# KohakuBlueleaf/UwUDiff

Hardware: AMD Instinct MI355X
Metric: train images/sec (whole node), DiT-S/2 256^2 latent (higher is better)
Workload: dtype bf16; 1 GPU; DiT-S/2 (L12 D384 h6), 4x32x32 synthetic latents + pooled-text cond 1280, eps-MSE, AdamW lr1e-6 wd0.01 cosine; random-init weights; per_gpu_batch=768, global_batch=768, parallelism=dp1

## Files before the change

include/uwu_hip.h:

```cpp
#ifndef UWU_HIP_H
#define UWU_HIP_H

#include <stddef.h>
#include <stdint.h>

#ifdef __cplusplus
extern "C" {
#endif

#define UWU_F32 0
#define UWU_BF16 1
#define UWU_I64 2

#define UWU_OK 0
#define UWU_EINVAL (-1)
#define UWU_ELAUNCH (-2)
#define UWU_ENOTIMPL (-3)

#define UWU_PT_EPSILON 0
#define UWU_PT_V 1
#define UWU_PT_SAMPLE 2
#define UWU_PT_RF 3

#define UWU_EPI_NONE 0
#define UWU_EPI_BIAS 1
#define UWU_EPI_BIAS_GELU 2
#define UWU_EPI_DGELU 3
#define UWU_EPI_BIAS_SILU 4
#define UWU_EPI_ACCUM 5

const char* uwu_last_error(void);
int uwu_version(void);
int uwu_env_refresh(void);
int uwu_memset_zero(void* p, uint64_t bytes, void* stream);


int uwu_schedule_gather(const int64_t* timesteps, const float* sigmas_desc, const float* all_snr,
                        const float* alphas_cumprod, int n_train, int B, int snr_mode, float gamma,
                        int debias, float* coef, void* stream);

int uwu_rf_time_to_sigma(const float* u01, float sigma_max, const float* log_sigmas_asc, int n_train,
                         int B, float* coef, float* timesteps, void* stream);

int uwu_qsample(const float* x, const float* noise, const float* coef, int B, int64_t n, float* noisy,
                void* noisy_bf16, void* stream);

int uwu_qsample_norm(const float* x, const float* noise, const float* coef, int B, int64_t n, float vae_mean,
                     float vae_std, float* x_norm, float* noisy, void* stream);

int uwu_philox_raw(uint32_t* out, int64_t n_counters, uint64_t seed, uint64_t offset, void* stream);
int uwu_philox_normal(float* out, int64_t n, uint64_t seed, uint64_t offset, void* stream);
int uwu_draw_timesteps(int64_t* timesteps, int n_train, int B, uint64_t seed, uint64_t offset, void* stream);
int uwu_draw_u01(float* u01, int B, uint64_t seed, uint64_t offset, void* stream);
int uwu_qsample_draw(const float* x, const float* coef, int B, int64_t n, int use_norm, float vae_mean, float vae_std,
                     float* x_norm, float* noise, float* noisy, uint64_t seed, uint64_t offset, void* stream);
int uwu_posterior_draw(const float* moments, int ldm, int B, int latent, int64_t HW, float* z, float* mean_out, float* logvar_out,
                       uint64_t seed, uint64_t offset, void* stream);

int uwu_ctx_place(const void* src, int dtype, const int64_t* mask, float* out, int B, int S, int F, int S_total,
                  int F_total, int s_off, int f_off, void* stream);

int uwu_loss_fwd_bwd(const float* x, const float* noise, const float* xt, const void* model_output,
                     int out_dtype, const float* coef, int pred_type, int target_type, int force_convert,
                     int B, int64_t n, float* losses, float* loss_mean, void* grad_out, float* pred,
                     float* target, void* stream);

int uwu_scale_inplace(void* y, int dtype, int64_t n, const float* scale, void* stream);
int uwu_scale_into(const void* x, void* y, int dtype, int64_t n, const float* scale, void* stream);
int uwu_cast_i64_to_f32(const int64_t* x, float* y, int64_t n, void* stream);

int uwu_aggregate_concat(const void* emb, const int* starts, void* out, int B, int max_n, int64_t unit_bytes,
                         int elem_size, uint64_t pad_bits, void* stream);
int uwu_aggregate_split(const void* cat, const int* starts, void* out, int B, int max_n, int64_t unit_bytes,
                        void* stream);
int uwu_aggregate_first(const void* emb, const int* starts, void* out, int B, int64_t unit_bytes, void* stream);

int uwu_sampler_step(const float* x, const float* eps_cond, const float* eps_uncond, const float* noise, float* out,
                     float* denoised, int64_t n, float cfg, float sigma, float sigma_down, float sigma_up,
                     float s_noise, void* stream);
int uwu_sampler_combine(const float* base, const float* eps_cond, const float* eps_uncond, const float* noise,
                        float* out, int64_t n, float cfg, float a, float b, float c, void* stream);
int uwu_scale_copy(const float* x, float* y, int64_t n, float scale, void* stream);

int uwu_cfg_input(const float* x, float* y, int B, int64_t n, float c_in, void* stream);
int uwu_sampler_combine_draw(const float* base, const float* eps_cond, const float* eps_uncond, float* out, int64_t n, float cfg,
                             float a, float b, float c, uint64_t seed, uint64_t offset, void* stream);
// ... 328 lines not shown
```

uwudiff_amd/csrc/api.cpp:

```cpp
#include <hip/hip_runtime.h>
#include <stdarg.h>
#include <stdio.h>

#include <atomic>

#include "../../include/uwu_hip.h"

static thread_local char g_err[512] = "";

void uwu_set_error(const char* fmt, ...) {
  va_list ap;
  va_start(ap, fmt);
  vsnprintf(g_err, sizeof(g_err), fmt, ap);
  va_end(ap);
}

extern "C" const char* uwu_last_error(void) { return g_err; }
extern "C" int uwu_version(void) { return 1; }

static int g_env_gen = 0;
int uwu_env_generation() { return g_env_gen; }
extern "C" int uwu_env_refresh(void) { return ++g_env_gen; }

std::atomic<const char*> g_uwu_gemm_last_kernel{""};
extern "C" const char* uwu_gemm_last_kernel(void) { return g_uwu_gemm_last_kernel.load(std::memory_order_relaxed); }

extern "C" int uwu_memset_zero(void* p, uint64_t bytes, void* stream) {
  if (!p || !bytes) {
    uwu_set_error("memset_zero: bad argument");
    return UWU_EINVAL;
  }
  if (hipMemsetAsync(p, 0, (size_t)bytes, (hipStream_t)stream) != hipSuccess) {
    uwu_set_error("memset_zero: hipMemsetAsync failed");
    return UWU_ELAUNCH;
  }
  return UWU_OK;
}

static const int kMaxDev = 64;
static int g_dev_cus[kMaxDev];
static size_t g_dev_lds[kMaxDev];
static bool g_dev_known[kMaxDev];
static int cur_dev() {
  int dev = 0;
  if (hipGetDevice(&dev) != hipSuccess || dev < 0 || dev >= kMaxDev) dev = 0;
  if (!g_dev_known[dev]) {
    hipDeviceProp_t prop;
    if (hipGetDeviceProperties(&prop, dev) == hipSuccess) {
      g_dev_cus[dev] = prop.multiProcessorCount;
      g_dev_lds[dev] = prop.sharedMemPerBlockOptin ? prop.sharedMemPerBlockOptin : prop.sharedMemPerBlock;
    } else {
      g_dev_cus[dev] = 0;
      g_dev_lds[dev] = 0;
    }
    g_dev_known[dev] = true;
  }
  return dev;
}
int uwu_dev_index() { return cur_dev(); }
int uwu_dev_cus() { return g_dev_cus[cur_dev()]; }
bool uwu_dev_lds_fits(size_t bytes) { return g_dev_lds[cur_dev()] >= bytes; }
bool uwu_func_lds(const void* fn, size_t bytes, unsigned char* done) {
  const int dev = cur_dev();
  if (done[dev] == 1) return true;
  if (done[dev] == 2) return false;
  const bool ok = g_dev_lds[dev] >= bytes && hipFuncSetAttribute(fn, hipFuncAttributeMaxDynamicSharedMemorySize, (int)bytes) == hipSuccess;
  done[dev] = ok ? 1 : 2;
  return ok;
}
```

uwudiff_amd/csrc/attention_p256.hip:

```cpp
#include "common.h"

namespace {

constexpr int P_RING = 3;
template <int DH>
struct PGeom {
  static constexpr bool TAIL = DH > 64;
  static constexpr int SLOT = 16384 + (TAIL ? 2048 + 256 : 0);
  static constexpr int OFF_TT = 16384, OFF_TL = 16384 + 2048;
  static constexpr int OFF_DS = P_RING * SLOT;
  static constexpr int KIMG = 32768 + (TAIL ? 4096 : 0);
  static constexpr int OFF_K = OFF_DS + 32768;
  static constexpr int OFF_LSE = OFF_K + 2 * KIMG;
  static constexpr int OFF_DELTA = OFF_LSE + (TAIL ? 0 : 2 * 1024);
  static constexpr int OFF_ZERO = OFF_DELTA + 2 * 256;
  static constexpr int LDS = OFF_ZERO + (TAIL ? 16 : 0);
};
static_assert(PGeom<64>::LDS == 150016 && PGeom<72>::LDS <= 163840, "LDS budget");
constexpr int P_LDS = PGeom<64>::LDS;

struct PArgs {
  const bf16_t *q, *k, *v, *o, *dO;
  bf16_t *dq, *dk, *dv;
  const float* lse;
  int B, H, ldq, ldk, ldv, ldo, nheads;
  float scale;
};

__device__ __forceinline__ int fsw(int row) {
  return (((row >> 2) ^ (row >> 4)) & 1) | ((((row >> 3) ^ (row >> 4)) & 1) << 1) | (((row >> 1) & 1) << 2);
}
__device__ __forceinline__ int Fsw(int row) {
  return (row & 1) | (((row >> 2) & 1) << 1) | (((row >> 3) & 1) << 2) | (((row >> 1) & 1) << 3);
}

typedef short s16x4 __attribute__((ext_vector_type(4)));
typedef unsigned su32x2 __attribute__((ext_vector_type(2)));

__device__ __forceinline__ void glds16(const void* gsrc, unsigned lds_dst ) {
  unsigned keep;
  asm volatile("s_mov_b32 %0, m0\n\ts_mov_b32 m0, %2\n\ts_nop 0\n\tglobal_load_lds_dwordx4 %1, off\n\ts_mov_b32 m0, %0"
               : "=&s"(keep)
               : "v"(gsrc), "s"(lds_dst)
               : "memory");
}
__device__ __forceinline__ void glds4(const void* gsrc, unsigned lds_dst ) {
  unsigned keep;
  asm volatile("s_mov_b32 %0, m0\n\ts_mov_b32 m0, %2\n\ts_nop 0\n\tglobal_load_lds_dword %1, off\n\ts_mov_b32 m0, %0"
               : "=&s"(keep)
               : "v"(gsrc), "s"(lds_dst)
               : "memory");
}
__device__ __forceinline__ void glds16_s(const void* sbase , unsigned voff, unsigned lds_dst ) {
  unsigned keep;
  asm volatile("s_mov_b32 %0, m0\n\ts_mov_b32 m0, %3\n\ts_nop 0\n\tglobal_load_lds_dwordx4 %1, %2\n\ts_mov_b32 m0, %0"
               : "=&s"(keep)
               : "v"(voff), "s"(sbase), "s"(lds_dst)
               : "memory");
}
__device__ __forceinline__ f32x16 mfma32(const uint4& a, const uint4& b, f32x16 c) {
  return __builtin_amdgcn_mfma_f32_32x32x16_bf16(*reinterpret_cast<const bf16x8*>(&a), *reinterpret_cast<const bf16x8*>(&b), c, 0,
                                                 0, 0);
}
__device__ __forceinline__ f32x4 mfma16(const uint4& a, const uint4& b, f32x4 c) {
  return __builtin_amdgcn_mfma_f32_16x16x32_bf16(*reinterpret_cast<const bf16x8*>(&a), *reinterpret_cast<const bf16x8*>(&b), c, 0,
                                                 0, 0);
}
__device__ __forceinline__ uint4 pack8(const f32x16& x, int s) {
  bf16x8 f;
#pragma unroll
  for (int j = 0; j < 8; ++j) f[j] = (bf16_t)x[8 * s + j];
  return *reinterpret_cast<uint4*>(&f);
}

extern __shared__ __attribute__((aligned(16))) char p_smem[];

__device__ __forceinline__ void lane_halves(float x, float& lo, float& hi) {
  float a = x, b = x;
  asm volatile("v_nop\n\tv_nop\n\tv_permlane32_swap_b32 %0, %1" : "+v"(a), "+v"(b));
  lo = a;
  hi = b;
}

__device__ __forceinline__ uint4 tr_pair(unsigned a0, unsigned a1) {
  const s16x4 lo = __builtin_amdgcn_ds_read_tr16_b64_v4i16(
      (__attribute__((address_space(3))) s16x4*)((__attribute__((address_space(3))) char*)p_smem + a0));
  const s16x4 hi = __builtin_amdgcn_ds_read_tr16_b64_v4i16(
      (__attribute__((address_space(3))) s16x4*)((__attribute__((address_space(3))) char*)p_smem + a1));
  uint4 r;
  r.x = ((unsigned)(unsigned short)lo[0]) | ((unsigned)(unsigned short)lo[1] << 16);
  r.y = ((unsigned)(unsigned short)lo[2]) | ((unsigned)(unsigned short)lo[3] << 16);
  r.z = ((unsigned)(unsigned short)hi[0]) | ((unsigned)(unsigned short)hi[1] << 16);
  r.w = ((unsigned)(unsigned short)hi[2]) | ((unsigned)(unsigned short)hi[3] << 16);
  return r;
}

template <int DH>
__global__ void __launch_bounds__(512, 2) attn_bwd_p256(const PArgs a) {
  using G = PGeom<DH>;
  constexpr bool TAIL = G::TAIL;
  constexpr int T = 256, NKS = TAIL ? 5 : 4, NDT = TAIL ? 3 : 2;
  constexpr int P_SLOT = G::SLOT, P_OFF_DS = G::OFF_DS, P_OFF_K = G::OFF_K, P_OFF_LSE = G::OFF_LSE, P_OFF_DELTA = G::OFF_DELTA;
  constexpr int KIMG = G::KIMG;
  char* const smem = p_smem;
  const int tid = threadIdx.x, lane = tid & 63;
  const int wave = __builtin_amdgcn_readfirstlane(tid >> 6);
  const int r = lane & 31, h = lane >> 5;
  const int fr = lane & 15, fq = lane >> 4;
  const unsigned smem_base = (unsigned)(size_t)((const __attribute__((address_space(3))) char*)p_smem);
  const float c = a.scale * 1.4426950408889634f;
  const float ninv_scale = -1.f / a.scale;
  const int nmy = (a.nheads - (int)blockIdx.x + (int)gridDim.x - 1) / (int)gridDim.x;
  const int total = 4 * nmy;
  const int k0 = wave * 32;

  const int drow = tid >> 3;
  const int dchunk = (tid & 7) ^ fsw(drow);
  unsigned B0, A0, K0, D0, TQ0, TA0, KT0;
  auto phase1_consts = [&](int ln) {
    const int r_ = ln & 31, h_ = ln >> 5;
    B0 = (unsigned)(r_ * 128 + ((h_ ^ fsw(r_)) << 4));
    const int rowL = 4 * h_ + ((ln & 15) >> 2), chunkL = 2 * ((ln >> 4) & 1) + ((ln & 3) >> 1);
    A0 = (unsigned)(rowL * 128 + ((chunkL ^ fsw(rowL)) << 4) + 8 * (ln & 1));
    TQ0 = (unsigned)((r_ >> 3) * 256 + (r_ & 7) * 16);
    TA0 = (unsigned)(rowL * 16 + 8 * (ln & 1));
  };
  auto phase2_consts = [&](int ln) {
    const int fr_ = ln & 15, fq_ = ln >> 4;
    const int rowK = 8 * fq_ + (fr_ >> 2);
    K0 = (unsigned)(rowK * 128 + ((((fr_ & 3) >> 1) ^ fsw(rowK)) << 4) + 8 * (fr_ & 1));
    D0 = (unsigned)(rowK * 128 + (((fr_ & 3) ^ Fsw(rowK)) << 3));
    KT0 = (unsigned)(rowK * 16 + 8 * (fr_ & 1));
  };
  auto opaque_lane = [&]() {
    int ln = lane;
    asm volatile("" : "+v"(ln));
    return ln;
  };
  auto my_tid = [&]() {
    int x = tid;
    if constexpr (TAIL) asm volatile("" : "+v"(x));
    return x;
  };
  if constexpr (!TAIL) {
    phase1_consts(lane);
    phase2_consts(lane);
  }

  auto head_ptrs = [&](int j, int& b, int& hd) {
    const int bh = (int)blockIdx.x + j * (int)gridDim.x;
    b = bh / a.H;
    hd = bh - b * a.H;
  };
  uint4 oreg;
  unsigned otail = 0;
  auto issue_tile = [&](int g) {
    int b, hd;
    head_ptrs(g >> 2, b, hd);
    const int tid = my_tid(), lane = tid & 63, drow = tid >> 3, dchunk = (tid & 7) ^ fsw(drow);
    const int row = 64 * (g & 3) + drow;
    const bf16_t* qs = a.q + ((int64_t)b * T + row) * a.ldq + hd * DH + 8 * dchunk;
    const bf16_t* gs = a.dO + ((int64_t)b * T + row) * a.ldo + hd * DH + 8 * dchunk;
    const unsigned dst = smem_base + (unsigned)((g % P_RING) * P_SLOT + wave * 1024);
    glds16(qs, dst);
    glds16(gs, dst + 8192);
    oreg = *reinterpret_cast<const uint4*>(a.o + ((int64_t)b * T + row) * a.ldo + hd * DH + 8 * dchunk);
    if constexpr (TAIL) {
      const unsigned slot = smem_base + (unsigned)((g % P_RING) * P_SLOT);
      if (lane < 16) {
        const int64_t trow = (int64_t)b * T + 64 * (g & 3) + 8 * wave + (lane & 7);
        const bf16_t* src = lane < 8 ? a.q + trow * a.ldq + hd * DH + 64 : a.dO + trow * a.ldo + hd * DH + 64;
        glds16(src, slot + (unsigned)(G::OFF_TT + wave * 256));
      }
      glds4(a.lse + ((int64_t)b * a.H + hd) * T + 64 * (g & 3) + lane, slot + (unsigned)G::OFF_TL);
      otail = *reinterpret_cast<const unsigned*>(a.o + ((int64_t)b * T + row) * a.ldo + hd * DH + 64 + 2 * (tid & 3));
    }
  };
  auto issue_head = [&](int j) {
    int b, hd;
    head_ptrs(j, b, hd);
    const int tid = my_tid(), lane = tid & 63, drow = tid >> 3, dchunk = (tid & 7) ^ fsw(drow);
    const unsigned dst = smem_base + (unsigned)(P_OFF_K + (j & 1) * KIMG + wave * 1024);
#pragma unroll
    for (int p = 0; p < 4; ++p)
      glds16(a.k + ((int64_t)b * T + 64 * p + drow) * a.ldk + hd * DH + 8 * dchunk, dst + p * 8192);
    if constexpr (TAIL) {
      if (lane < 32)
        glds16(a.k + ((int64_t)b * T + 32 * wave + lane) * a.ldk + hd * DH + 64,
               smem_base + (unsigned)(P_OFF_K + (j & 1) * KIMG + 32768 + wave * 512));
    } else {
      glds4(a.lse + ((int64_t)b * a.H + hd) * T + 64 * (wave & 3) + lane,
            smem_base + (unsigned)(P_OFF_LSE + (j & 1) * 1024 + (wave & 3) * 256));
    }
  };
  uint4 kf[NKS], vf[NKS];
  auto load_kv = [&](int j) {
    int b, hd;
    head_ptrs(j, b, hd);
    const int tid = my_tid(), r = tid & 31, h = (tid >> 5) & 1;
#pragma unroll
    for (int s = 0; s < 4; ++s) {
      kf[s] = *reinterpret_cast<const uint4*>(a.k + ((int64_t)b * T + k0 + r) * a.ldk + hd * DH + 16 * s + 8 * h);
      vf[s] = *reinterpret_cast<const uint4*>(a.v + ((int64_t)b * T + k0 + r) * a.ldv + hd * DH + 16 * s + 8 * h);
// ... 188 lines not shown
      const uint4 fa = tr_pair(Ki + ka + ko, Ki + (ka ^ 0x10u) + 512u + ko);
      const uint4 fb = tr_pair(Ki + kb + ko, Ki + (kb ^ 0x10u) + 512u + ko);
      const uint4 fd = tr_pair(Di + da + ko, Di + (da ^ 0x10u) + 512u + ko);
      acc0 = mfma16(fa, fd, acc0);
      acc1 = mfma16(fb, fd, acc1);
      if constexpr (TAIL) {
        const unsigned kt = Ki + 32768u + KT0 + 512u * kk;
        acc2 = mfma16(tr_pair(kt, kt + 64u), fd, acc2);
      }
    }
    int b, hd;
    head_ptrs(j, b, hd);
    const f32x4 v0 = acc0 * a.scale, v1 = acc1 * a.scale;
    const bf16x4 p0b = {(bf16_t)v0[0], (bf16_t)v0[1], (bf16_t)v0[2], (bf16_t)v0[3]};
    const bf16x4 p1b = {(bf16_t)v1[0], (bf16_t)v1[1], (bf16_t)v1[2], (bf16_t)v1[3]};
    const uint2 p0 = *reinterpret_cast<const uint2*>(&p0b), p1 = *reinterpret_cast<const uint2*>(&p1b);
    const su32x2 sx = __builtin_amdgcn_permlane16_swap(p0.x, p1.x, false, false);
    const su32x2 sy = __builtin_amdgcn_permlane16_swap(p0.y, p1.y, false, false);
    const bool odd = fq & 1;
    const int d = odd ? 16 * (db0 + 1) + 4 * (fq - 1) : 16 * db0 + 4 * fq;
    bf16_t* dst = a.dq + ((int64_t)b * T + 64 * t + 16 * qblk + fr) * a.ldq + hd * DH + d;
    *reinterpret_cast<uint4*>(dst) = uint4{sx[0], sy[0], sx[1], sy[1]};
    if constexpr (TAIL) {
      const f32x4 v2 = acc2 * a.scale;
      store4(a.dq + ((int64_t)b * T + 64 * t + 16 * qblk + fr) * a.ldq + hd * DH + 64 + 4 * (fq & 1), v2);
    }
  }
  asm volatile("s_waitcnt lgkmcnt(0)" ::: "memory");
  __builtin_amdgcn_s_barrier();
  store_dkdv(nmy - 1);
}

template <int DH>
struct FGeom {
  static constexpr bool TAIL = DH > 64;
  static constexpr int RING = TAIL ? 4 : 5;
  static constexpr int SLOT = 16384 + (TAIL ? 2048 : 0);
  static constexpr int OFF_TT = 16384;
  static constexpr int OST = 4096 + (TAIL ? 512 : 0);
  static constexpr int OFF_O = RING * SLOT;
  static constexpr int OFF_Q = OFF_O + 8 * OST;
  static constexpr int OFF_ZERO = OFF_Q + 32768 + (TAIL ? 4096 : 0);
  static constexpr int LDS = OFF_ZERO + (TAIL ? 16 : 0);
};
static_assert(FGeom<64>::LDS == 147456 && FGeom<72>::LDS <= 163840, "LDS budget");
constexpr int F_LDS = FGeom<64>::LDS;

struct FArgs {
  const bf16_t *q, *k, *v;
  bf16_t* out;
  float* lse;
  int B, H, ldq, ldk, ldv, ldo, nheads;
  float scale;
};

template <int N>
__device__ __forceinline__ void wait_vm_n() {
  asm volatile("s_waitcnt vmcnt(%0)" ::"n"(N) : "memory");
}
__device__ __forceinline__ void wait_vm(int n) {
  switch (n < 20 ? n : 20) {
    case 20: wait_vm_n<20>(); break;
    case 19: wait_vm_n<19>(); break;
    case 18: wait_vm_n<18>(); break;
    case 17: wait_vm_n<17>(); break;
    case 16: wait_vm_n<16>(); break;
    case 15: wait_vm_n<15>(); break;
    case 14: wait_vm_n<14>(); break;
    case 13: wait_vm_n<13>(); break;
    case 12: wait_vm_n<12>(); break;
    case 11: wait_vm_n<11>(); break;
    case 10: wait_vm_n<10>(); break;
    case 9: wait_vm_n<9>(); break;
    case 8: wait_vm_n<8>(); break;
    case 7: wait_vm_n<7>(); break;
    case 6: wait_vm_n<6>(); break;
    case 5: wait_vm_n<5>(); break;
    case 4: wait_vm_n<4>(); break;
    case 3: wait_vm_n<3>(); break;
    case 2: wait_vm_n<2>(); break;
    case 1: wait_vm_n<1>(); break;
    default: wait_vm_n<0>();
  }
}

template <int DH>
__global__ void __launch_bounds__(512, 2) attn_fwd_p256(const FArgs a) {
  using G = FGeom<DH>;
  constexpr bool TAIL = G::TAIL;
  constexpr int T = 256, NKS = TAIL ? 5 : 4, NDT = TAIL ? 3 : 2;
  constexpr int F_RING = G::RING, AHEAD = F_RING - 1, F_SLOT = G::SLOT, F_OFF_O = G::OFF_O, F_OFF_Q = G::OFF_Q;
  constexpr int TILE_OPS = TAIL ? 3 : 2, Q_OPS = TAIL ? 5 : 4, ST_OPS = TAIL ? 6 : 5;
  char* const smem = p_smem;
  const int tid = threadIdx.x, lane = tid & 63;
  const int wave = __builtin_amdgcn_readfirstlane(tid >> 6);
  const int r = lane & 31, h = lane >> 5;
  const unsigned smem_base = (unsigned)(size_t)((const __attribute__((address_space(3))) char*)p_smem);
  const float c = a.scale * 1.4426950408889634f;
  const int nmy = (a.nheads - (int)blockIdx.x + (int)gridDim.x - 1) / (int)gridDim.x;
  const int total = 4 * nmy;
  const int q0 = wave * 32;
  const int drow = tid >> 3;
  const int dchunk = (tid & 7) ^ fsw(drow);
  const unsigned B0 = (unsigned)(r * 128 + ((h ^ fsw(r)) << 4));
  const unsigned QR0 = (unsigned)(F_OFF_Q + (q0 + r) * 128 + ((h ^ fsw(q0 + r)) << 4));
  const int rowL = 4 * h + ((lane & 15) >> 2), chunkL = 2 * ((lane >> 4) & 1) + ((lane & 3) >> 1);
  const unsigned A0 = (unsigned)(rowL * 128 + ((chunkL ^ fsw(rowL)) << 4) + 8 * (lane & 1));
  const unsigned TQ0 = (unsigned)((r >> 3) * 256 + (r & 7) * 16);
  const unsigned TA0 = (unsigned)(rowL * 16 + 8 * (lane & 1));
  auto head_ptrs = [&](int j, int& b, int& hd) {
    const int bh = (int)blockIdx.x + j * (int)gridDim.x;
    b = bh / a.H;
    hd = bh - b * a.H;
  };
  const unsigned kvoff = (unsigned)((drow * a.ldk + 8 * dchunk) * 2), vvoff = (unsigned)((drow * a.ldv + 8 * dchunk) * 2);
  const unsigned qvoff = (unsigned)((drow * a.ldq + 8 * dchunk) * 2);
  const bf16_t *kb_n = nullptr, *vb_n = nullptr, *qb_n = nullptr;
  int b_c = 0, hd_c = 0;
  auto set_issue_head = [&](int j) {
    int b, hd;
    head_ptrs(j, b, hd);
    kb_n = a.k + (int64_t)b * T * a.ldk + hd * DH;
    vb_n = a.v + (int64_t)b * T * a.ldv + hd * DH;
    qb_n = a.q + (int64_t)b * T * a.ldq + hd * DH;
  };
  auto issue_tile = [&](int g) {
    const int t64 = 64 * (g & 3);
    const unsigned dst = smem_base + (unsigned)((g % F_RING) * F_SLOT + wave * 1024);
    glds16_s(kb_n, kvoff + (unsigned)(t64 * a.ldk * 2), dst);
    glds16_s(vb_n, vvoff + (unsigned)(t64 * a.ldv * 2), dst + 8192);
    if constexpr (TAIL) {
      if (lane < 16) {
        const int trow = t64 + 8 * wave + (lane & 7);
        const bf16_t* src = lane < 8 ? kb_n + (int64_t)trow * a.ldk + 64 : vb_n + (int64_t)trow * a.ldv + 64;
        glds16(src, smem_base + (unsigned)((g % F_RING) * F_SLOT + G::OFF_TT + wave * 256));
      }
    }
  };
  auto issue_q = [&]() {
#pragma unroll
    for (int p = 0; p < 4; ++p)
      glds16_s(qb_n, qvoff + (unsigned)(64 * p * a.ldq * 2), smem_base + (unsigned)(F_OFF_Q + p * 8192 + wave * 1024));
    if constexpr (TAIL) {
      if (lane < 32) glds16(qb_n + (int64_t)(32 * wave + lane) * a.ldq + 64, smem_base + (unsigned)(F_OFF_Q + 32768 + wave * 512));
    }
  };
  auto extras = [&](int i) { return ((i & 3) == 1 && (i >> 2) + 1 < nmy ? Q_OPS : 0) + ((i & 3) == 3 ? ST_OPS : 0); };
  auto younger = [&](int g) {
    int y = 0;
    const int gi = g - (F_RING - 1);
    if (gi < 0) {
      for (int x = g + 1; x < F_RING - 1; ++x) y += x < total ? TILE_OPS : 0;
    } else {
      y += extras(gi);
    }
    for (int i = gi < 0 ? 0 : gi + 1; i < g; ++i) y += (i + F_RING - 1 < total ? TILE_OPS : 0) + extras(i);
    return y;
  };
  if (total == 0) return;
  static_assert(AHEAD == 4 || AHEAD == 3, "the tile issued in iteration g belongs to the next head from t = 4 - AHEAD on");
  if constexpr (TAIL)
    if (tid < 4) reinterpret_cast<unsigned*>(smem + G::OFF_ZERO)[tid] = 0u;
  set_issue_head(0);
  head_ptrs(0, b_c, hd_c);
  issue_q();
#pragma unroll
  for (int g = 0; g < F_RING - 1; ++g) issue_tile(g);

  uint4 qf[NKS];
  f32x16 o[NDT];
  float m = -INFINITY, l = 0.f;
  for (int g = 0; g < total; ++g) {
    const int j = g >> 2, t = g & 3;
    int n_fly = younger(g);
    if (t == 0 && j > 0) {
      const int yq = (g - 2 + F_RING - 1 < total ? TILE_OPS : 0) + (g - 1 + F_RING - 1 < total ? TILE_OPS : 0) + ST_OPS;
      n_fly = yq < n_fly ? yq : n_fly;
    }
    wait_vm(n_fly);
    __builtin_amdgcn_s_barrier();
    if (t == 0) head_ptrs(j, b_c, hd_c);
    if (t == 4 - AHEAD && j + 1 < nmy) set_issue_head(j + 1);
    if (g + F_RING - 1 < total) issue_tile(g + F_RING - 1);
    if (t == 0) {
#pragma unroll
      for (int s = 0; s < 4; ++s) qf[s] = *reinterpret_cast<const uint4*>(smem + (QR0 ^ (unsigned)(s << 5)));
      if constexpr (TAIL)
        qf[4] = *reinterpret_cast<const uint4*>(smem + (h ? (unsigned)G::OFF_ZERO : (unsigned)(F_OFF_Q + 32768 + (q0 + r) * 16)));
#pragma unroll
      for (int dt = 0; dt < NDT; ++dt) o[dt] = f32x16{};
      m = -INFINITY;
      l = 0.f;
    }
    if (t == 1 && j + 1 < nmy) issue_q();
    const unsigned Ks = (unsigned)((g % F_RING) * F_SLOT), Vs = Ks + 8192;
// ... 39 lines not shown
    for (int dt = 0; dt < 2; ++dt)
#pragma unroll
      for (int i = 0; i < 16; ++i) o[dt][i] *= alpha;
    if constexpr (TAIL) {
#pragma unroll
      for (int i = 0; i < 4; ++i) o[2][i] *= alpha;
    }
#pragma unroll
    for (int kt = 0; kt < 2; ++kt)
#pragma unroll
      for (int s2 = 0; s2 < 2; ++s2) {
        const uint4 pf = pack8(s[kt], s2);
#pragma unroll
        for (int dt = 0; dt < 2; ++dt) {
          const unsigned x0 = (A0 ^ (unsigned)(0x30 * s2) ^ (unsigned)(0x40 * dt)) + 2048u * s2 + 4096u * kt;
          const uint4 vt = tr_pair(Vs + x0, Vs + (x0 ^ 0x20u) + 1024u);
          o[dt] = mfma32(vt, pf, o[dt]);
        }
        if constexpr (TAIL) {
          const unsigned x0 = Ks + (unsigned)G::OFF_TT + 128u + TA0 + 512u * s2 + 1024u * kt;
          o[2] = mfma32(tr_pair(x0, x0 + 256u), pf, o[2]);
        }
      }
    if (t == 3) {
      const int b = b_c, hd = hd_c;
      float lt;
      {
        float lo, hi;
        lane_halves(l, lo, hi);
        lt = lo + hi;
      }
      const float inv = 1.f / lt;
      char* mine = smem + F_OFF_O + wave * G::OST;
#pragma unroll
      for (int dt = 0; dt < 2; ++dt)
#pragma unroll
        for (int g4 = 0; g4 < 4; ++g4) {
          const int d0 = 32 * dt + 8 * g4 + 4 * h;
          store4(reinterpret_cast<bf16_t*>(mine + r * 128 + (((d0 >> 3) ^ (r & 7)) << 4) + 2 * (d0 & 7)),
                 f32x4{o[dt][4 * g4] * inv, o[dt][4 * g4 + 1] * inv, o[dt][4 * g4 + 2] * inv, o[dt][4 * g4 + 3] * inv});
        }
      bf16_t* ob = a.out + ((int64_t)b * T + q0) * a.ldo + hd * DH;
#pragma unroll
      for (int p = 0; p < 4; ++p) {
        const int row = 8 * p + (lane >> 3), ch = lane & 7;
        const uint4 x = *reinterpret_cast<const uint4*>(mine + row * 128 + ((ch ^ (row & 7)) << 4));
        *reinterpret_cast<uint4*>(ob + (int64_t)row * a.ldo + 8 * ch) = x;
      }
      if constexpr (TAIL) {
        store4(reinterpret_cast<bf16_t*>(mine + 4096 + r * 16 + 8 * h), f32x4{o[2][0] * inv, o[2][1] * inv, o[2][2] * inv, o[2][3] * inv});
        const uint4 xt = *reinterpret_cast<const uint4*>(mine + 4096 + r * 16);
        *reinterpret_cast<uint4*>(ob + (int64_t)r * a.ldo + 64) = xt;
      }
      a.lse[((int64_t)b * a.H + hd) * T + q0 + r] = m * a.scale + __logf(lt);
    }
  }
}

}

bool uwu_attn_p256_ok(int T, int Tk, int d, int ldq, int ldk, int ldv, int ldo) {
  static UwuEnv on("UWU_ATTN_P256");
  if (on.get().is('0') || T != 256 || Tk != 256 || ldq % 8 || ldk % 8 || ldv % 8 || ldo % 8 || uwu_dev_cus() <= 0) return false;
  if (d == 64) return uwu_dev_lds_fits(P_LDS);
  static UwuEnv on72("UWU_ATTN_P256_D72");
  return d == 72 && !on72.get().is('0') && uwu_dev_lds_fits(PGeom<72>::LDS);
}

int uwu_attn_p256_bwd(const void* q, const void* k, const void* v, const void* o, const void* dO, const float* lse, void* dq,
                      void* dk, void* dv, int B, int H, int d, int ldq, int ldk, int ldv, int ldo, float scale, hipStream_t st) {
  static unsigned char done[UWU_MAX_DEV];
  const int n_cu = uwu_dev_cus();
  if (d == 72) {
    static unsigned char done72[UWU_MAX_DEV];
    if (n_cu <= 0 || !uwu_func_lds(reinterpret_cast<const void*>(attn_bwd_p256<72>), PGeom<72>::LDS, done72)) {
      uwu_set_error("attention_bwd(p256, d = 72): the device cannot give a workgroup %d bytes of LDS", (int)PGeom<72>::LDS);
      return UWU_ELAUNCH;
    }
    PArgs a{};
    a.q = (const bf16_t*)q; a.k = (const bf16_t*)k; a.v = (const bf16_t*)v; a.o = (const bf16_t*)o; a.dO = (const bf16_t*)dO;
    a.dq = (bf16_t*)dq; a.dk = (bf16_t*)dk; a.dv = (bf16_t*)dv; a.lse = lse;
    a.B = B; a.H = H; a.ldq = ldq; a.ldk = ldk; a.ldv = ldv; a.ldo = ldo; a.nheads = B * H; a.scale = scale;
    const int grid = a.nheads < n_cu ? a.nheads : n_cu;
    hipLaunchKernelGGL(attn_bwd_p256<72>, dim3(grid), dim3(512), PGeom<72>::LDS, st, a);
    UWU_LAUNCH_CHECK("attention_bwd(p256, d = 72)");
    return UWU_OK;
  }
  if (n_cu <= 0 || !uwu_func_lds(reinterpret_cast<const void*>(attn_bwd_p256<64>), P_LDS, done)) {
    uwu_set_error("attention_bwd(p256): the device cannot give a workgroup %d bytes of LDS", (int)P_LDS);
    return UWU_ELAUNCH;
  }
  PArgs a{};
  a.q = (const bf16_t*)q; a.k = (const bf16_t*)k; a.v = (const bf16_t*)v; a.o = (const bf16_t*)o; a.dO = (const bf16_t*)dO;
  a.dq = (bf16_t*)dq; a.dk = (bf16_t*)dk; a.dv = (bf16_t*)dv; a.lse = lse;
  a.B = B; a.H = H; a.ldq = ldq; a.ldk = ldk; a.ldv = ldv; a.ldo = ldo; a.nheads = B * H; a.scale = scale;
  const int grid = a.nheads < n_cu ? a.nheads : n_cu;
  hipLaunchKernelGGL(attn_bwd_p256<64>, dim3(grid), dim3(512), P_LDS, st, a);
  UWU_LAUNCH_CHECK("attention_bwd(p256)");
  return UWU_OK;
}

bool uwu_attn_p256_fwd_ok(int nheads, int T, int Tk, int d, int ldq, int ldk, int ldv, int ldo) {
  static UwuEnv on("UWU_ATTN_P256F");
  if (on.get().is('0')) return false;
  if (!on.is('1') && nheads < 1024) return false;
  if (T != 256 || Tk != 256 || ldq % 8 || ldk % 8 || ldv % 8 || ldo % 8 || uwu_dev_cus() <= 0) return false;
  if (d == 64) return uwu_dev_lds_fits(F_LDS);
  static UwuEnv on72("UWU_ATTN_P256F_D72");
  return d == 72 && !on72.get().is('0') && uwu_dev_lds_fits(FGeom<72>::LDS);
}

int uwu_attn_p256_fwd(const void* q, const void* k, const void* v, void* o, float* lse, int B, int H, int d, int ldq, int ldk, int ldv,
                      int ldo, float scale, hipStream_t st) {
  static unsigned char done[2][UWU_MAX_DEV];
  const int n_cu = uwu_dev_cus();
  const int lds = d == 72 ? FGeom<72>::LDS : F_LDS;
  const void* fn = d == 72 ? reinterpret_cast<const void*>(attn_fwd_p256<72>) : reinterpret_cast<const void*>(attn_fwd_p256<64>);
  if (n_cu <= 0 || !uwu_func_lds(fn, lds, done[d == 72])) {
    uwu_set_error("attention_fwd(p256): the device cannot give a workgroup %d bytes of LDS", lds);
    return UWU_ELAUNCH;
  }
  FArgs a{};
  a.q = (const bf16_t*)q; a.k = (const bf16_t*)k; a.v = (const bf16_t*)v; a.out = (bf16_t*)o; a.lse = lse;
  a.B = B; a.H = H; a.ldq = ldq; a.ldk = ldk; a.ldv = ldv; a.ldo = ldo; a.nheads = B * H; a.scale = scale;
  const int grid = a.nheads < n_cu ? a.nheads : n_cu;
  if (d == 72) hipLaunchKernelGGL(attn_fwd_p256<72>, dim3(grid), dim3(512), lds, st, a);
  else hipLaunchKernelGGL(attn_fwd_p256<64>, dim3(grid), dim3(512), lds, st, a);
  UWU_LAUNCH_CHECK("attention_fwd(p256)");
  return UWU_OK;
}
```

uwudiff_amd/csrc/common.h:

```cpp
#pragma once
#include <hip/hip_runtime.h>
#include <stdint.h>
#include <stdio.h>
#include <stdlib.h>

#include "../../include/uwu_hip.h"

typedef __bf16 bf16_t;
typedef __bf16 bf16x2 __attribute__((ext_vector_type(2)));
typedef __bf16 bf16x4 __attribute__((ext_vector_type(4)));
typedef __bf16 bf16x8 __attribute__((ext_vector_type(8)));
typedef float f32x2 __attribute__((ext_vector_type(2)));
typedef float f32x4 __attribute__((ext_vector_type(4)));
typedef float f32x16 __attribute__((ext_vector_type(16)));

#define UWU_WAVE 64

void uwu_set_error(const char* fmt, ...);

#define UWU_CHECK_ARG(cond, ...)       \
  do {                                 \
    if (!(cond)) {                     \
      uwu_set_error(__VA_ARGS__);      \
      return UWU_EINVAL;               \
    }                                  \
  } while (0)

#define UWU_LAUNCH_CHECK(name)                                                  \
  do {                                                                          \
    hipError_t e_ = hipGetLastError();                                          \
    if (e_ != hipSuccess) {                                                     \
      uwu_set_error("%s: launch failed: %s", name, hipGetErrorString(e_));      \
      return UWU_ELAUNCH;                                                       \
    }                                                                           \
  } while (0)

#include "env.h"

int uwu_dev_index();
int uwu_dev_cus();
bool uwu_dev_lds_fits(size_t bytes);
constexpr int UWU_MAX_DEV = 64;
bool uwu_func_lds(const void* fn, size_t bytes, unsigned char* done );

int uwu_prof_begin(void* stream);
void uwu_prof_end(int slot, int tag, int kind, double flops, double bytes, void* stream);
struct UwuProfScope {
  int slot;
  void* st;
  explicit UwuProfScope(void* s) : slot(uwu_prof_begin(s)), st(s) {}
  void done(int tag, int kind, double flops, double bytes) {
    if (slot >= 0) uwu_prof_end(slot, tag, kind, flops, bytes, st);
  }
};

__device__ __forceinline__ float to_f32(float v) { return v; }
__device__ __forceinline__ float to_f32(bf16_t v) { return (float)v; }
template <typename T>
__device__ __forceinline__ T from_f32(float v);
template <>
__device__ __forceinline__ float from_f32<float>(float v) { return v; }
template <>
__device__ __forceinline__ bf16_t from_f32<bf16_t>(float v) { return (bf16_t)v; }

#define UWU_DPP_F(v, ctrl, rmask, ident) \
  __builtin_bit_cast(float, __builtin_amdgcn_update_dpp(__builtin_bit_cast(int, (float)(ident)), __builtin_bit_cast(int, v), ctrl, rmask, 0xF, false))
__device__ __forceinline__ float wave_sum(float v) {
  v += UWU_DPP_F(v, 0xB1, 0xF, 0.f);
  v += UWU_DPP_F(v, 0x4E, 0xF, 0.f);
  v += UWU_DPP_F(v, 0x141, 0xF, 0.f);
  v += UWU_DPP_F(v, 0x140, 0xF, 0.f);
  v += UWU_DPP_F(v, 0x142, 0xA, 0.f);
  v += UWU_DPP_F(v, 0x143, 0xC, 0.f);
  return __builtin_bit_cast(float, __builtin_amdgcn_readlane(__builtin_bit_cast(int, v), 63));
}
__device__ __forceinline__ float wave_max(float v) {
  v = fmaxf(v, UWU_DPP_F(v, 0xB1, 0xF, v));
  v = fmaxf(v, UWU_DPP_F(v, 0x4E, 0xF, v));
  v = fmaxf(v, UWU_DPP_F(v, 0x141, 0xF, v));
  v = fmaxf(v, UWU_DPP_F(v, 0x140, 0xF, v));
  v = fmaxf(v, UWU_DPP_F(v, 0x142, 0xA, v));
  v = fmaxf(v, UWU_DPP_F(v, 0x143, 0xC, v));
  return __builtin_bit_cast(float, __builtin_amdgcn_readlane(__builtin_bit_cast(int, v), 63));
}
__device__ __forceinline__ float row16_sum(float v) {
  v += __builtin_bit_cast(float, __builtin_amdgcn_update_dpp(0, __builtin_bit_cast(int, v), 0xB1, 0xF, 0xF, true));
  v += __builtin_bit_cast(float, __builtin_amdgcn_update_dpp(0, __builtin_bit_cast(int, v), 0x4E, 0xF, 0xF, true));
  v += __builtin_bit_cast(float, __builtin_amdgcn_update_dpp(0, __builtin_bit_cast(int, v), 0x141, 0xF, 0xF, true));
  v += __builtin_bit_cast(float, __builtin_amdgcn_update_dpp(0, __builtin_bit_cast(int, v), 0x140, 0xF, 0xF, true));
  return v;
// ... 94 lines not shown
```

uwudiff_amd/csrc/dit.cpp:

```cpp
#include <hip/hip_runtime.h>
#include <math.h>
#include <stddef.h>
#include <stdint.h>
#include <stdlib.h>

#include "../../include/uwu_hip.h"
#include "env.h"

void uwu_set_error(const char* fmt, ...);

namespace {

constexpr int WGRAD_BLOCKS = 512;

struct Layout {
  size_t es;
  int64_t M, D, D3, D4, Kp, Ko;
  size_t feat, t_pre, t_h, temb, yemb, c, sc, mod;
  size_t sc16, dmod16;
  size_t tok, xe;
  size_t layer0, layer_stride;
  bool ckpt;
  size_t keep, scratch0;
  size_t o_x0, o_m1, o_r1, o_h1, o_qkv, o_lse, o_ao, o_y1, o_x1, o_m2, o_r2, o_h2, o_u, o_f, o_y2;
  size_t o_rope;
  size_t o_h1t, o_aot, o_h2t, o_ft;
  size_t xF, mF, rF, hF, otok;
  size_t dx, dy, dh, dqkv, dao, du, delta, dotok, dmod, dsc, dc, dth, dtp;
  size_t w2t;
  size_t wsc, wsc_bytes;
  size_t x8, x8t, dy8, dy8t, w8, w8_layer;
  size_t total;
};

inline size_t al(size_t x) { return (x + 255) & ~(size_t)255; }

Layout make_layout(const uwu_dit_desc& d) {
  Layout L{};
  L.es = d.dtype == UWU_BF16 ? 2 : 4;
  L.M = (int64_t)d.B * d.T;
  L.D = d.D;
  L.D3 = 3 * (int64_t)d.D;
  L.D4 = (int64_t)d.mlp_ratio * d.D;
  L.Kp = (int64_t)d.in_ch * d.patch * d.patch;
  L.Ko = (int64_t)d.out_ch * d.patch * d.patch;
  size_t p = 0;
  auto take = [&](size_t bytes) { size_t o = p; p = al(p + bytes); return o; };
  const size_t f4 = 4;
  L.feat = take((size_t)d.B * d.freq_dim * f4);
  L.t_pre = take((size_t)d.B * d.D * f4);
  L.t_h = take((size_t)d.B * d.D * f4);
  L.temb = take((size_t)d.B * d.D * f4);
  L.yemb = take((size_t)d.B * d.D * f4);
  L.c = take((size_t)d.B * d.D * f4);
  L.sc = take((size_t)d.B * d.D * f4);
  L.mod = take((size_t)d.B * d.mod_total * f4);
  L.sc16 = take((size_t)d.B * d.D * 2);
  L.dmod16 = take((size_t)d.B * d.mod_total * 2);
  L.tok = take(L.M * L.Kp * L.es);
  L.xe = take(L.M * L.D * L.es);
// ... 58 lines not shown
                           uwu_gemm_fp8_scratch_bytes((int)L.D3, d.D, (int)L.M), uwu_gemm_fp8_scratch_bytes(d.D, d.D, (int)L.M)})
      if (t > L.wsc_bytes) L.wsc_bytes = t;
  }
  L.wsc_bytes = (L.wsc_bytes + 255) & ~(size_t)255;
  L.wsc = take(L.wsc_bytes * (L.M <= 16384 ? 4 : 1));
  if (d.fp8) {
    L.x8 = take(L.M * L.D4);
    L.x8t = 0;
    L.dy8 = take(L.M * L.D4);
    L.dy8t = take(L.M * L.D4);
    L.w8_layer = al((size_t)24 * d.D * d.D);
    L.w8 = take((size_t)d.L * L.w8_layer);
  }
  L.total = p;
  return L;
}

int check_desc(const uwu_dit_desc* d) {
  if (!d) { uwu_set_error("dit: null descriptor"); return UWU_EINVAL; }
  if (d->B <= 0 || d->T <= 0 || d->D <= 0 || d->H <= 0 || d->L <= 0 || d->D % d->H || d->D % 8 ||
      d->img % d->patch || (d->img / d->patch) * (d->img / d->patch) != d->T || d->mlp_ratio <= 0 ||
      d->freq_dim <= 0 || d->freq_dim % 8) {
    uwu_set_error("dit: inconsistent shape B=%d T=%d D=%d H=%d L=%d img=%d patch=%d", d->B, d->T, d->D, d->H, d->L,
                  d->img, d->patch);
    return UWU_EINVAL;
  }
  if (d->dtype != UWU_F32 && d->dtype != UWU_BF16) { uwu_set_error("dit: bad dtype"); return UWU_EINVAL; }
  if (d->mod_total != d->L * 6 * d->D + 2 * d->D) { uwu_set_error("dit: mod_total mismatch"); return UWU_EINVAL; }
  if ((d->in_ch * d->patch * d->patch) % 8 || (d->out_ch * d->patch * d->patch) % 8 || (d->cond_dim % 8)) {
    uwu_set_error("dit: C*p*p and cond_dim must be multiples of 8");
    return UWU_EINVAL;
  }
  if (!d->w || !d->w32 || !d->pos || !d->ws) { uwu_set_error("dit: null buffer"); return UWU_EINVAL; }
  if (d->rope && (d->dtype != UWU_BF16 || d->D / d->H != 64 || d->T % 64 || d->T > 256 || !d->pos_xy)) {
    uwu_set_error("dit: the fused axial-RoPE attention needs bf16, head dim 64, T a multiple of 64 up to 256 and pos_xy");
    return UWU_EINVAL;
  }
  if (d->fp8) {
    if (d->fp8 < 0 || d->fp8 > 2 || d->dtype != UWU_BF16 || d->D % 128 || d->mlp_ratio != 4 || ((int64_t)d->B * d->T) % 128 ||
        !d->f8_scale || !d->f8_amax || !d->f8_fmt) {
      uwu_set_error("dit: fp8 mode needs bf16 activations, D %% 128 == 0, B*T %% 128 == 0, mlp_ratio 4 and the scale / amax / fmt arrays");
      return UWU_EINVAL;
    }
  }
  return UWU_OK;
}

#define RUN(expr)              \
  do {                         \
    int rc_ = (expr);          \
    if (rc_ != UWU_OK) return rc_; \
  } while (0)

int lin_fwd(const void* X, const void* W, const float* bias, void* Y, void* Y2, int M, int N, int K, int dt, int cdt,
            int epi, void* st) {
  return uwu_gemm(X, W, Y, Y2, bias, nullptr, M, N, K, K, K, N, 0, 0, 0, dt, cdt, epi, 1, st);
}
int lin_fwd32(const float* X, const float* W, const float* bias, float* Y, float* Y2, int M, int N, int K, int epi, void* st) {
  if (M <= 16 && N <= 4096 && uwu_skinny_linear_ok(M, N, K)) return uwu_skinny_linear_fwd(X, W, bias, Y, Y2, M, N, K, epi, st);
  return lin_fwd(X, W, bias, Y, Y2, M, N, K, UWU_F32, UWU_F32, epi, st);
}
int lin_dgrad(const void* dY, const void* W, void* dX, const void* aux, int M, int N, int K, int dt, void* st,
              float* colsum = nullptr) {
  return uwu_gemm(dY, W, dX, colsum, nullptr, aux, M, K, N, N, K, K, K, 0, 1, dt, dt,
                  aux ? UWU_EPI_DGELU : UWU_EPI_NONE, 1, st);
}
static bool mod_bf16(const uwu_dit_desc& d) {
  return d.dtype == UWU_BF16 && d.B >= 64 && d.mod_total % 8 == 0;
}
int lin_dgrad_splitk(const void* dY, const void* W, float* dX, int M, int N, int K, void* st) {
  if (hipMemsetAsync(dX, 0, (size_t)M * K * sizeof(float), (hipStream_t)st) != hipSuccess) {
    uwu_set_error("dgrad_splitk: memset failed");
    return UWU_ELAUNCH;
  }
  const int tiles = ((M + 127) / 128) * ((K + 127) / 128);
  const int ktiles = (N + 31) / 32;
  int split = (512 + tiles - 1) / tiles;
  if (split > ktiles) split = ktiles;
  return uwu_gemm(dY, W, dX, nullptr, nullptr, nullptr, M, K, N, N, K, K, 0, 0, 1, UWU_F32, UWU_F32, UWU_EPI_ACCUM, split,
                  st);
}
int lin_wgrad(const void* dY, const void* X, float* dW, int M, int N, int K, int dt, void* st, void* scratch = nullptr,
              size_t scratch_bytes = 0, float* db = nullptr) {
  if (dt == UWU_BF16 && scratch && uwu_gemm_wgrad_scratch_bytes(N, K, M) <= scratch_bytes)
    return uwu_gemm_wgrad(dY, X, dW, db, N, K, M, N, K, K, dt, WGRAD_BLOCKS, scratch, scratch_bytes, st);
  if (db) {
    const int rc = uwu_colsum(dY, dt, M, N, N, db, 1, st);
    if (rc != UWU_OK) return rc;
  }
  const int tiles = ((N + 127) / 128) * ((K + 127) / 128);
  const int bk = dt == UWU_BF16 ? 64 : 32;
  const int ktiles = (M + bk - 1) / bk;
  const int target = tiles >= 16 ? 768 : 256;
  int split = (target + tiles - 1) / tiles;
  if (split > ktiles) split = ktiles;
  if (split < 1) split = 1;
  return uwu_gemm(dY, X, dW, nullptr, nullptr, nullptr, N, K, M, N, K, K, 0, 1, 1, dt, UWU_F32, UWU_EPI_ACCUM, split, st);
}

bool wgrad_pair_ok(int M, int Na, int Ka, int Nb, int Kb, size_t scratch_bytes) {
  const size_t need = uwu_gemm_wgrad_pair_scratch_bytes(Na, Ka, Nb, Kb, M);
  return need && need <= scratch_bytes;
}
int lin_wgrad_pair(const void* dYa, const void* Xa, float* dWa, float* dba, int Na, int Ka, const void* dYb, const void* Xb,
                   float* dWb, float* dbb, int Nb, int Kb, int M, void* st, void* scratch, size_t scratch_bytes) {
  return uwu_gemm_wgrad_pair(dYa, Xa, dWa, dba, Na, Ka, Na, Ka, Ka, dYb, Xb, dWb, dbb, Nb, Kb, Nb, Kb, Kb, M, UWU_BF16,
// ... 115 lines not shown
  if (f.on && hipStreamWaitEvent(f.main, f.ev[4 + slot], 0) != hipSuccess) {
    uwu_set_error("dit_backward: stream join failed");
    return UWU_ELAUNCH;
  }
  return UWU_OK;
}

struct Ptrs {
  char* ws;
  const Layout& L;
  template <typename T = void>
  T* at(size_t off) const { return reinterpret_cast<T*>(ws + off); }
  template <typename T = void>
  T* lay(int l, size_t sub) const {
    if (L.ckpt && sub >= L.keep) return reinterpret_cast<T*>(ws + L.scratch0 + sub);
    return reinterpret_cast<T*>(ws + L.layer0 + (size_t)l * L.layer_stride + sub);
  }
};

struct LayerW {
  const void *qkv_w, *o_w, *fc1_w, *fc2_w;
  const float *qkv_b, *o_b, *fc1_b, *fc2_b;
  int64_t off_qkv_w, off_qkv_b, off_o_w, off_o_b, off_fc1_w, off_fc1_b, off_fc2_w, off_fc2_b;
};

inline int64_t pad64(int64_t n) { return (n + 63) & ~(int64_t)63; }

LayerW layer_weights(const uwu_dit_desc& d, int l) {
  LayerW w{};
  const int64_t D = d.D, D4 = (int64_t)d.mlp_ratio * d.D;
  int64_t o = d.off_layer0 + (int64_t)l * d.layer_stride;
  w.off_qkv_w = o; o += pad64(3 * D * D);
  w.off_qkv_b = o; o += pad64(3 * D);
  w.off_o_w = o; o += pad64(D * D);
  w.off_o_b = o; o += pad64(D);
  w.off_fc1_w = o; o += pad64(D4 * D);
  w.off_fc1_b = o; o += pad64(D4);
  w.off_fc2_w = o; o += pad64(D * D4);
  w.off_fc2_b = o; o += pad64(D);
  const size_t es = d.dtype == UWU_BF16 ? 2 : 4;
  const char* wb = static_cast<const char*>(d.w);
  w.qkv_w = wb + w.off_qkv_w * es;
  w.o_w = wb + w.off_o_w * es;
  w.fc1_w = wb + w.off_fc1_w * es;
  w.fc2_w = wb + w.off_fc2_w * es;
  w.qkv_b = d.w32 + w.off_qkv_b;
  w.o_b = d.w32 + w.off_o_b;
  w.fc1_b = d.w32 + w.off_fc1_b;
  w.fc2_b = d.w32 + w.off_fc2_b;
  return w;
}


int block_forward(const uwu_dit_desc& d, const Layout& L, const Ptrs& P, const F8& f8, int l, bool recompute, void* st) {
  const int dt = d.dtype, B = d.B, T = d.T, D = d.D, M = (int)L.M, D3 = (int)L.D3, D4 = (int)L.D4;
  const size_t es = L.es;
  const float* w32 = d.w32;
  const int ML = d.mod_total;
  const float* mod = P.at<float>(L.mod);
  const float scale = 1.f / sqrtf((float)(D / d.H));
  const LayerW w = layer_weights(d, l);
  const float* m = mod + (int64_t)l * 6 * D;
  void* x0 = P.lay(l, L.o_x0);
  int h1q = 0, h2q = 0;
  if (d.fp8) {
    if (l == 0 || recompute) {
      h1q = ln_fwd_f8(d, f8, x0, nullptr, nullptr, m + 0, m + D, ML, x0, P.lay(l, L.o_h1), P.lay(l, L.o_h1t), f8.role(l, 0),
                      P.lay<float>(l, L.o_m1), P.lay<float>(l, L.o_r1), st);
    } else {
      const float* mp = mod + (int64_t)(l - 1) * 6 * D;
      h1q = ln_fwd_f8(d, f8, P.lay(l - 1, L.o_x1), P.lay(l - 1, L.o_y2), mp + 5 * D, m + 0, m + D, ML, x0, P.lay(l, L.o_h1),
                      P.lay(l, L.o_h1t), f8.role(l, 0), P.lay<float>(l, L.o_m1), P.lay<float>(l, L.o_r1), st);
    }
    if (h1q < 0) return h1q;
  } else
  if (l == 0 || recompute) {
    RUN(uwu_add_ln_modulate_fwd(x0, nullptr, nullptr, m + 0, m + D, ML, x0, P.lay(l, L.o_h1),
                                P.lay<float>(l, L.o_m1), P.lay<float>(l, L.o_r1), B, T, D, d.ln_eps, 0, dt, st));
  } else {
    const float* mp = mod + (int64_t)(l - 1) * 6 * D;
    RUN(uwu_add_ln_modulate_fwd(P.lay(l - 1, L.o_x1), P.lay(l - 1, L.o_y2), mp + 5 * D, m + 0, m + D, ML, x0,
                                P.lay(l, L.o_h1), P.lay<float>(l, L.o_m1), P.lay<float>(l, L.o_r1), B, T, D,
                                d.ln_eps, 0, dt, st));
  }
  if (d.fp8) RUN(f8_fwd(f8, h1q ? nullptr : P.lay(l, L.o_h1), P.lay(l, L.o_h1t), f8.w(l, 0, false), w.qkv_b, P.lay(l, L.o_qkv), nullptr, M, D3, D, f8.role(l, 0), f8.role(l, 8), UWU_EPI_BIAS));
  else RUN(lin_fwd(P.lay(l, L.o_h1), w.qkv_w, w.qkv_b, P.lay(l, L.o_qkv), nullptr, M, D3, D, dt, dt, UWU_EPI_BIAS, st));
  char* qkv = P.lay<char>(l, L.o_qkv);
  if (d.rope) {
    const int64_t fo = (int64_t)l * d.H * (D / d.H / 4);
    RUN(uwu_axial_rope_table(d.pos_xy, w32 + d.off_rope_h + fo, w32 + d.off_rope_w + fo, P.lay<float>(l, L.o_rope), T, d.H,
                             D / d.H, D, st));
    RUN(uwu_attention_rope_fwd(qkv, qkv + (size_t)D * es, qkv + (size_t)2 * D * es, P.lay<float>(l, L.o_rope), P.lay(l, L.o_ao),
                               P.lay<float>(l, L.o_lse), B, T, d.H, D / d.H, D3, D3, D3, D, D, scale, dt, st));
  } else
  RUN(uwu_attention_fwd(qkv, qkv + (size_t)D * es, qkv + (size_t)2 * D * es, P.lay(l, L.o_ao), P.lay<float>(l, L.o_lse),
                        B, T, T, d.H, D / d.H, D3, D3, D3, D, scale, dt, st));
  if (d.fp8) RUN(f8_fwd(f8, P.lay(l, L.o_ao), P.lay(l, L.o_aot), f8.w(l, 1, false), w.o_b, P.lay(l, L.o_y1), nullptr, M, D, D, f8.role(l, 1), f8.role(l, 9), UWU_EPI_BIAS));
  else RUN(lin_fwd(P.lay(l, L.o_ao), w.o_w, w.o_b, P.lay(l, L.o_y1), nullptr, M, D, D, dt, dt, UWU_EPI_BIAS, st));
  if (d.fp8) {
    h2q = ln_fwd_f8(d, f8, x0, P.lay(l, L.o_y1), m + 2 * D, m + 3 * D, m + 4 * D, ML, P.lay(l, L.o_x1), P.lay(l, L.o_h2),
                    P.lay(l, L.o_h2t), f8.role(l, 2), P.lay<float>(l, L.o_m2), P.lay<float>(l, L.o_r2), st);
    if (h2q < 0) return h2q;
  } else
  RUN(uwu_add_ln_modulate_fwd(x0, P.lay(l, L.o_y1), m + 2 * D, m + 3 * D, m + 4 * D, ML, P.lay(l, L.o_x1),
                              P.lay(l, L.o_h2), P.lay<float>(l, L.o_m2), P.lay<float>(l, L.o_r2), B, T, D, d.ln_eps,
                              0, dt, st));
  if (d.fp8) {
    if (f8_emit(d)) {
      const int r2 = f8.role(l, 2), r3 = f8.role(l, 3);
      if (!h2q) RUN(f8.quant(P.lay(l, L.o_h2), UWU_BF16, M, D, r2, f8.x8, P.lay(l, L.o_h2t), nullptr, false));
      RUN(uwu_gemm_fp8_emit(f8.x8, f8.w(l, 2, false), P.lay(l, L.o_u), nullptr, w.fc1_b, nullptr, M, D4, D, D, D, D4, 0, UWU_FP8_E4M3,
                            UWU_EPI_BIAS_GELU, f8.scale + r2, f8.scale + f8.role(l, 10), f8.dy8, D4, P.lay(l, L.o_ft), M, f8.scale + r3,
                            f8.amax + r3, st));
      RUN(uwu_gemm_fp8(f8.dy8, f8.w(l, 3, false), P.lay(l, L.o_y2), nullptr, w.fc2_b, nullptr, M, D, D4, D4, D4, D, 0, UWU_FP8_E4M3,
                       UWU_EPI_BIAS, f8.scale + r3, f8.scale + f8.role(l, 11), nullptr, 0, st));
      return UWU_OK;
    }
    RUN(f8_fwd(f8, h2q ? nullptr : P.lay(l, L.o_h2), P.lay(l, L.o_h2t), f8.w(l, 2, false), w.fc1_b, P.lay(l, L.o_u), P.lay(l, L.o_f), M, D4, D, f8.role(l, 2), f8.role(l, 10), UWU_EPI_BIAS_GELU));
    RUN(f8_fwd(f8, P.lay(l, L.o_f), P.lay(l, L.o_ft), f8.w(l, 3, false), w.fc2_b, P.lay(l, L.o_y2), nullptr, M, D, D4, f8.role(l, 3), f8.role(l, 11), UWU_EPI_BIAS));
  } else {
    RUN(lin_fwd(P.lay(l, L.o_h2), w.fc1_w, w.fc1_b, P.lay(l, L.o_u), P.lay(l, L.o_f), M, D4, D, dt, dt,
                UWU_EPI_BIAS_GELU, st));
    RUN(lin_fwd(P.lay(l, L.o_f), w.fc2_w, w.fc2_b, P.lay(l, L.o_y2), nullptr, M, D, D4, dt, dt, UWU_EPI_BIAS, st));
  }
  return UWU_OK;
}

}

extern "C" size_t uwu_dit_workspace_bytes(const uwu_dit_desc* d) {
  if (!d) return 0;
  return make_layout(*d).total;
}

extern "C" int64_t uwu_dit_layer_param_stride(int D, int mlp_ratio) {
  const int64_t d = D, d4 = (int64_t)mlp_ratio * D;
  return pad64(3 * d * d) + pad64(3 * d) + pad64(d * d) + pad64(d) + pad64(d4 * d) + pad64(d4) + pad64(d * d4) + pad64(d);
}

extern "C" int uwu_dit_forward(const uwu_dit_desc* dp, const float* noisy, const float* t, const float* cond,
                               float* out, void* st) {
  RUN(check_desc(dp));
  const uwu_dit_desc& d = *dp;
  if (!noisy || !t || !out) { uwu_set_error("dit_forward: null tensor"); return UWU_EINVAL; }
  if ((d.cond_dim > 0) != (cond != nullptr)) { uwu_set_error("dit_forward: cond / cond_dim mismatch"); return UWU_EINVAL; }
  const Layout L = make_layout(d);
  if (d.ws_bytes < L.total) { uwu_set_error("dit_forward: workspace too small (%zu < %zu)", d.ws_bytes, L.total); return UWU_EINVAL; }
  if (d.layer_stride != uwu_dit_layer_param_stride(d.D, d.mlp_ratio)) { uwu_set_error("dit: layer_stride mismatch"); return UWU_EINVAL; }
  Ptrs P{static_cast<char*>(d.ws), L};
  const int dt = d.dtype, B = d.B, T = d.T, D = d.D, M = (int)L.M, D3 = (int)L.D3, D4 = (int)L.D4;
  const size_t es = L.es;
  const char* wb = static_cast<const char*>(d.w);
  const float* w32 = d.w32;
  const int ML = d.mod_total;

  RUN(uwu_timestep_embedding(t, B, d.freq_dim, 10000.f, P.at(L.feat), UWU_F32, st));
  RUN(lin_fwd32(P.at<float>(L.feat), w32 + d.off_t_w1, w32 + d.off_t_b1, P.at<float>(L.t_pre), P.at<float>(L.t_h), B, D,
                d.freq_dim, UWU_EPI_BIAS_SILU, st));
  RUN(lin_fwd32(P.at<float>(L.t_h), w32 + d.off_t_w2, w32 + d.off_t_b2, P.at<float>(L.temb), nullptr, B, D, D, UWU_EPI_BIAS, st));
  const void* cptr = P.at(L.temb);
  if (cond) {
    RUN(lin_fwd32(cond, w32 + d.off_y_w, w32 + d.off_y_b, P.at<float>(L.yemb), nullptr, B, D, d.cond_dim, UWU_EPI_BIAS, st));
    RUN(uwu_add(P.at(L.temb), P.at(L.yemb), P.at(L.c), (int64_t)B * D, UWU_F32, st));
    cptr = P.at(L.c);
  }
  RUN(uwu_silu_fwd(cptr, P.at(L.sc), (int64_t)B * D, UWU_F32, st));
  if (mod_bf16(d)) {
    RUN(uwu_cast_f32_to_bf16(P.at<float>(L.sc), P.at(L.sc16), (int64_t)B * D, st));
    RUN(lin_fwd(P.at(L.sc16), wb + d.off_mod_w * es, w32 + d.off_mod_b, P.at(L.mod), nullptr, B, ML, D, UWU_BF16, UWU_F32, UWU_EPI_BIAS, st));
  } else {
    RUN(lin_fwd32(P.at<float>(L.sc), w32 + d.off_mod_w, w32 + d.off_mod_b, P.at<float>(L.mod), nullptr, B, ML, D, UWU_EPI_BIAS, st));
  }
  const float* mod = P.at<float>(L.mod);

  const F8 f8{d.fp8, d.f8_scale, d.f8_amax, d.f8_fmt, P.at<char>(L.x8), nullptr, P.at<char>(L.dy8),
              P.at<char>(L.dy8t), P.at<char>(L.wsc), P.at<char>(L.w8), L.wsc_bytes, L.w8_layer, d.D, st};
  if (d.fp8) {
    const F8 fw{2, d.f8_scale, d.f8_amax, d.f8_fmt, nullptr, nullptr, nullptr, nullptr, nullptr, f8.w8, 0, L.w8_layer, d.D, st};
    const int rows[4] = {D3, D, D4, D}, cols[4] = {D, D, D, D4};
    for (int l = 0; l < d.L; ++l) {
      const LayerW w = layer_weights(d, l);
      const void* ws4[4] = {w.qkv_w, w.o_w, w.fc1_w, w.fc2_w};
      for (int i = 0; i < 4; ++i)
        RUN(uwu_fp8_amax(ws4[i], UWU_BF16, (int64_t)rows[i] * cols[i], d.f8_amax + fw.role(l, 8 + i), st));
    }
    RUN(uwu_fp8_update_scales(d.f8_amax, d.f8_scale, d.f8_fmt, 12 * d.L, 1.f, st));
    for (int l = 0; l < d.L; ++l) {
      const LayerW w = layer_weights(d, l);
      const void* ws4[4] = {w.qkv_w, w.o_w, w.fc1_w, w.fc2_w};
      for (int i = 0; i < 4; ++i)
        RUN(fw.quant(ws4[i], UWU_BF16, rows[i], cols[i], fw.role(l, 8 + i), fw.w(l, i, false), fw.w(l, i, true), nullptr, true));
    }
  }

  RUN(uwu_patchify(noisy, P.at(L.tok), B, d.in_ch, d.img, d.img, d.patch, dt, st));
  RUN(lin_fwd(P.at(L.tok), wb + d.off_patch_w * es, w32 + d.off_patch_b, P.lay(0, L.o_x0), nullptr, M, D, (int)L.Kp, dt,
              dt, UWU_EPI_BIAS, st));
  RUN(uwu_add_pos(P.lay(0, L.o_x0), d.pos, B, T, D, dt, st));

  for (int l = 0; l < d.L; ++l) RUN(block_forward(d, L, P, f8, l, false, st));
  {
    const int l = d.L - 1;
    const float* mp = mod + (int64_t)l * 6 * D;
    const float* mf = mod + (int64_t)d.L * 6 * D;
    RUN(uwu_add_ln_modulate_fwd(P.lay(l, L.o_x1), P.lay(l, L.o_y2), mp + 5 * D, mf + 0, mf + D, ML, P.at(L.xF),
                                P.at(L.hF), P.at<float>(L.mF), P.at<float>(L.rF), B, T, D, d.ln_eps, 0, dt, st));
    RUN(lin_fwd(P.at(L.hF), wb + d.off_final_w * es, w32 + d.off_final_b, P.at(L.otok), nullptr, M, (int)L.Ko, D, dt, dt,
                UWU_EPI_BIAS, st));
    RUN(uwu_unpatchify(P.at(L.otok), dt, out, B, d.out_ch, d.img, d.img, d.patch, st));
  }
  return UWU_OK;
}

extern "C" int uwu_dit_backward(const uwu_dit_desc* dp, const float* dout, void* st) {
  RUN(check_desc(dp));
  const uwu_dit_desc& d = *dp;
  if (!dout || !d.g32) { uwu_set_error("dit_backward: null tensor"); return UWU_EINVAL; }
  const Layout L = make_layout(d);
  if (d.ws_bytes < L.total) { uwu_set_error("dit_backward: workspace too small"); return UWU_EINVAL; }
  Ptrs P{static_cast<char*>(d.ws), L};
  const int dt = d.dtype, B = d.B, T = d.T, D = d.D, M = (int)L.M, D3 = (int)L.D3, D4 = (int)L.D4;
  const size_t es = L.es;
  const char* wb = static_cast<const char*>(d.w);
  const float* w32 = d.w32;
  float* g = d.g32;
  const int ML = d.mod_total;
  const float* mod = P.at<float>(L.mod);
  float* dmod = P.at<float>(L.dmod);
  if (hipMemsetAsync(dmod, 0, (size_t)B * ML * sizeof(float), (hipStream_t)st) != hipSuccess) {
    uwu_set_error("dit_backward: memset failed");
    return UWU_ELAUNCH;
  }
  const float scale = 1.f / sqrtf((float)(D / d.H));
  const F8 f8{d.fp8, d.f8_scale, d.f8_amax, d.f8_fmt, P.at<char>(L.x8), nullptr, P.at<char>(L.dy8),
              P.at<char>(L.dy8t), P.at<char>(L.wsc), P.at<char>(L.w8), L.wsc_bytes, L.w8_layer, d.D, st};
  Fork fk{static_cast<hipStream_t>(st), {}, {}, false};
  fk.on = d.side_stream && d.side_stream != st && !d.fp8 && dt == UWU_BF16 && M <= 16384 && !L.ckpt &&
          fork_resources(fk, static_cast<hipStream_t>(d.side_stream));
  char* const wsc = P.at<char>(L.wsc);
  bool side_used[4] = {false, false, false, false};
  const bool pairs = !fk.on && !d.fp8 && dt == UWU_BF16 && M > 16384 && !L.ckpt;
  const bool pair_fc = pairs && wgrad_pair_ok(M, D4, D, D, D4, L.wsc_bytes);
  const bool pair_attn = pairs && wgrad_pair_ok(M, D3, D, D, D, L.wsc_bytes);

  RUN(uwu_patchify(dout, P.at(L.dotok), B, d.out_ch, d.img, d.img, d.patch, dt, st));
  RUN(lin_wgrad(P.at(L.dotok), P.at(L.hF), g + d.off_final_w, M, (int)L.Ko, D, dt, st));
  RUN(uwu_colsum(P.at(L.dotok), dt, M, (int)L.Ko, (int)L.Ko, g + d.off_final_b, 1, st));
  RUN(lin_dgrad(P.at(L.dotok), wb + d.off_final_w * es, P.at(L.dh), nullptr, M, (int)L.Ko, D, dt, st));
  {
    const int l = d.L - 1;
    const float* mp = mod + (int64_t)l * 6 * D;
    const float* mf = mod + (int64_t)d.L * 6 * D;
    float* dmp = dmod + (int64_t)l * 6 * D;
    float* dmf = dmod + (int64_t)d.L * 6 * D;
    RUN(uwu_add_ln_modulate_bwd(P.at(L.dh), P.at(L.xF), P.at<float>(L.mF), P.at<float>(L.rF), mf + D, nullptr,
                                P.lay(l, L.o_y2), mp + 5 * D, ML, P.at(L.dx), P.at(L.dy), dmf + 0, dmf + D, dmp + 5 * D,
                                B, T, D, 0, dt, st));
  }
  for (int l = d.L - 1; l >= 0; --l) {
    const LayerW w = layer_weights(d, l);
    const float* m = mod + (int64_t)l * 6 * D;
    float* dm = dmod + (int64_t)l * 6 * D;
    if (d.fp8) {
      if (f8_emit(d)) {
        RUN(f8_bwd(f8, P.at(L.dy), P.lay(l, L.o_ft), f8.w(l, 3, true), g + w.off_fc2_w, g + w.off_fc2_b, nullptr, P.lay(l, L.o_u),
                   g + w.off_fc1_b, M, D, D4, f8.role(l, 7), f8.role(l, 3), f8.role(l, 11), nullptr, nullptr, f8.role(l, 6), f8.x8, f8.dy8t));
        RUN(f8_bwd(f8, nullptr, P.lay(l, L.o_h2t), f8.w(l, 2, true), g + w.off_fc1_w, nullptr, P.at(L.dh), nullptr, nullptr, M, D4, D,
                   f8.role(l, 6), f8.role(l, 2), f8.role(l, 10), f8.x8, f8.dy8t));
      } else {
      RUN(f8_bwd(f8, P.at(L.dy), P.lay(l, L.o_ft), f8.w(l, 3, true), g + w.off_fc2_w, g + w.off_fc2_b, P.at(L.du), P.lay(l, L.o_u),
                 g + w.off_fc1_b, M, D, D4, f8.role(l, 7), f8.role(l, 3), f8.role(l, 11)));
      RUN(f8_bwd(f8, P.at(L.du), P.lay(l, L.o_h2t), f8.w(l, 2, true), g + w.off_fc1_w, nullptr, P.at(L.dh), nullptr, nullptr, M, D4, D,
                 f8.role(l, 6), f8.role(l, 2), f8.role(l, 10)));
      }
    } else {
    if (!pair_fc) {
    RUN(on_side(fk, 0, [&](void* s2, int k) {
      return lin_wgrad(P.at(L.dy), P.lay(l, L.o_f), g + w.off_fc2_w, M, D, D4, dt, s2, wsc + (size_t)k * L.wsc_bytes, L.wsc_bytes, g + w.off_fc2_b);
    }));
    side_used[0] = true;
    }
    if (side_used[1]) RUN(join_side(fk, 1));
    if (dt == UWU_BF16 && D == 384 && M % 256 == 0 && M >= 256 * 256 && D4 % 64 == 0 && D4 >= 1024 && D4 <= 2048) {
      RUN(uwu_transpose_bf16(w.fc2_w, P.at(L.w2t), D, D4, D4, D, st));
      RUN(uwu_gemm(P.at(L.dy), P.at(L.w2t), P.at(L.du), nullptr, nullptr, P.lay(l, L.o_u), M, D4, D, D, D, D4, D4, 0, 0, dt, dt,
                   UWU_EPI_DGELU, 1, st));
    } else {
      RUN(lin_dgrad(P.at(L.dy), w.fc2_w, P.at(L.du), P.lay(l, L.o_u), M, D, D4, dt, st, nullptr));
    }
    if (pair_fc) {
      RUN(lin_wgrad_pair(P.at(L.du), P.lay(l, L.o_h2), g + w.off_fc1_w, g + w.off_fc1_b, D4, D, P.at(L.dy), P.lay(l, L.o_f),
                         g + w.off_fc2_w, g + w.off_fc2_b, D, D4, M, st, wsc, L.wsc_bytes));
    } else {
    RUN(on_side(fk, 1, [&](void* s2, int k) {
      return lin_wgrad(P.at(L.du), P.lay(l, L.o_h2), g + w.off_fc1_w, M, D4, D, dt, s2, wsc + (size_t)k * L.wsc_bytes, L.wsc_bytes, g + w.off_fc1_b);
    }));
    side_used[1] = true;
    }
    RUN(lin_dgrad(P.at(L.du), w.fc1_w, P.at(L.dh), nullptr, M, D4, D, dt, st));
    RUN(join_side(fk, 0));
    }
    RUN(uwu_add_ln_modulate_bwd(P.at(L.dh), P.lay(l, L.o_x1), P.lay<float>(l, L.o_m2), P.lay<float>(l, L.o_r2), m + 4 * D,
                                P.at(L.dx), P.lay(l, L.o_y1), m + 2 * D, ML, P.at(L.dx), P.at(L.dy), dm + 3 * D,
                                dm + 4 * D, dm + 2 * D, B, T, D, 0, dt, st));
    if (d.fp8) {
      RUN(f8_bwd(f8, P.at(L.dy), P.lay(l, L.o_aot), f8.w(l, 1, true), g + w.off_o_w, g + w.off_o_b, P.at(L.dao), nullptr, nullptr, M, D, D,
                 f8.role(l, 5), f8.role(l, 1), f8.role(l, 9)));
    } else {
    if (!pair_attn) {
    RUN(on_side(fk, 2, [&](void* s2, int k) {
      return lin_wgrad(P.at(L.dy), P.lay(l, L.o_ao), g + w.off_o_w, M, D, D, dt, s2, wsc + (size_t)k * L.wsc_bytes, L.wsc_bytes, g + w.off_o_b);
    }));
    side_used[2] = true;
    }
    RUN(lin_dgrad(P.at(L.dy), w.o_w, P.at(L.dao), nullptr, M, D, D, dt, st));
    if (side_used[3]) RUN(join_side(fk, 3));
    }
    char* qkv = P.lay<char>(l, L.o_qkv);
    char* dqkv = P.at<char>(L.dqkv);
    if (d.rope) {
      const int64_t fo = (int64_t)l * d.H * (D / d.H / 4);
      RUN(uwu_attention_rope_bwd(qkv, qkv + (size_t)D * es, qkv + (size_t)2 * D * es, P.lay<float>(l, L.o_rope), P.lay(l, L.o_ao),
                                 P.at(L.dao), P.lay<float>(l, L.o_lse), dqkv, dqkv + (size_t)D * es, dqkv + (size_t)2 * D * es,
                                 B, T, d.H, D / d.H, D3, D3, D3, D, D, scale, dt, st));
      for (int qk = 0; qk < 2; ++qk)
        RUN(uwu_axial_rope_bwd_shared(qkv + (size_t)qk * D * es, dqkv + (size_t)qk * D * es, d.pos_xy, T,
                                      w32 + d.off_rope_h + fo, w32 + d.off_rope_w + fo, dqkv + (size_t)qk * D * es,
                                      g + d.off_rope_h + fo, g + d.off_rope_w + fo, (int64_t)M, d.H, D / d.H, D3, dt, st));
    } else
    RUN(uwu_attention_bwd(qkv, qkv + (size_t)D * es, qkv + (size_t)2 * D * es, P.lay(l, L.o_ao), P.at(L.dao),
                          P.lay<float>(l, L.o_lse), P.at<float>(L.delta), dqkv, dqkv + (size_t)D * es,
                          dqkv + (size_t)2 * D * es, B, T, T, d.H, D / d.H, D3, D3, D3, D, scale, dt, st));
    if (d.fp8) {
      RUN(f8_bwd(f8, dqkv, P.lay(l, L.o_h1t), f8.w(l, 0, true), g + w.off_qkv_w, g + w.off_qkv_b, P.at(L.dh), nullptr, nullptr, M, D3, D,
                 f8.role(l, 4), f8.role(l, 0), f8.role(l, 8)));
    } else if (pair_attn) {
      RUN(lin_wgrad_pair(dqkv, P.lay(l, L.o_h1), g + w.off_qkv_w, g + w.off_qkv_b, D3, D, P.at(L.dy), P.lay(l, L.o_ao),
                         g + w.off_o_w, g + w.off_o_b, D, D, M, st, wsc, L.wsc_bytes));
    } else {
    RUN(on_side(fk, 3, [&](void* s2, int k) {
      return lin_wgrad(dqkv, P.lay(l, L.o_h1), g + w.off_qkv_w, M, D3, D, dt, s2, wsc + (size_t)k * L.wsc_bytes, L.wsc_bytes, g + w.off_qkv_b);
    }));
    side_used[3] = true;
    }
    if (fk.on && d.layer_done && d.layer_done[l])
      for (int k = 0; k < 3; ++k)
        if (fk.side[k] != fk.side[3] && hipStreamWaitEvent(fk.side[3], fk.ev[4 + k], 0) != hipSuccess) {
          uwu_set_error("dit_backward: stream join failed");
          return UWU_ELAUNCH;
        }
    if (d.layer_done && d.layer_done[l] &&
        hipEventRecord(static_cast<hipEvent_t>(d.layer_done[l]), fk.on ? fk.side[3] : static_cast<hipStream_t>(st)) != hipSuccess) {
      uwu_set_error("dit_backward: hipEventRecord(layer_done[%d]) failed", l);
      return UWU_ELAUNCH;
    }
    if (!d.fp8) RUN(lin_dgrad(dqkv, w.qkv_w, P.at(L.dh), nullptr, M, D3, D, dt, st));
    if (!d.fp8) RUN(join_side(fk, 2));
    if (L.ckpt && l > 0) RUN(block_forward(d, L, P, f8, l - 1, true, st));
    if (l > 0) {
      const float* mp = mod + (int64_t)(l - 1) * 6 * D;
      float* dmp = dmod + (int64_t)(l - 1) * 6 * D;
      RUN(uwu_add_ln_modulate_bwd(P.at(L.dh), P.lay(l, L.o_x0), P.lay<float>(l, L.o_m1), P.lay<float>(l, L.o_r1), m + D,
                                  P.at(L.dx), P.lay(l - 1, L.o_y2), mp + 5 * D, ML, P.at(L.dx), P.at(L.dy), dm + 0,
                                  dm + D, dmp + 5 * D, B, T, D, 0, dt, st));
    } else {
      RUN(uwu_add_ln_modulate_bwd(P.at(L.dh), P.lay(l, L.o_x0), P.lay<float>(l, L.o_m1), P.lay<float>(l, L.o_r1), m + D,
                                  P.at(L.dx), nullptr, nullptr, ML, P.at(L.dx), nullptr, dm + 0, dm + D, nullptr, B, T, D, 0, dt, st));
    }
  }
  if (fk.on)
    for (int k = 0; k < 4; ++k) RUN(join_side(fk, k));
  RUN(lin_wgrad(P.at(L.dx), P.at(L.tok), g + d.off_patch_w, M, D, (int)L.Kp, dt, st));
  RUN(uwu_colsum(P.at(L.dx), dt, M, D, D, g + d.off_patch_b, 1, st));

  if (mod_bf16(d)) {
    RUN(uwu_cast_f32_to_bf16(dmod, P.at(L.dmod16), (int64_t)B * ML, st));
    RUN(lin_wgrad(P.at(L.dmod16), P.at(L.sc16), g + d.off_mod_w, B, ML, D, UWU_BF16, st));
    RUN(uwu_colsum(dmod, UWU_F32, B, ML, ML, g + d.off_mod_b, 1, st));
    if (hipMemsetAsync(P.at(L.dsc), 0, (size_t)B * D * sizeof(float), (hipStream_t)st) != hipSuccess) {
      uwu_set_error("dit_backward: memset failed");
      return UWU_ELAUNCH;
    }
    {
      const int tiles = ((B + 127) / 128) * ((D + 127) / 128), ktiles = (ML + 63) / 64;
      int split = (512 + tiles - 1) / tiles;
      if (split > ktiles) split = ktiles;
      RUN(uwu_gemm(P.at(L.dmod16), wb + d.off_mod_w * es, P.at(L.dsc), nullptr, nullptr, nullptr, B, D, ML, ML, D, D, 0, 0, 1, UWU_BF16,
                   UWU_F32, UWU_EPI_ACCUM, split, st));
    }
  } else {
    RUN(lin_wgrad32(dmod, P.at<float>(L.sc), g + d.off_mod_w, g + d.off_mod_b, B, ML, D, st));
    RUN(lin_dgrad_splitk(dmod, w32 + d.off_mod_w, P.at<float>(L.dsc), B, ML, D, st));
  }
  const void* cptr = d.cond_dim > 0 ? P.at(L.c) : P.at(L.temb);
  RUN(uwu_silu_bwd(cptr, P.at(L.dsc), P.at(L.dc), (int64_t)B * D, UWU_F32, st));
  if (d.cond_dim > 0) {
  }
  RUN(lin_wgrad32(P.at<float>(L.dc), P.at<float>(L.t_h), g + d.off_t_w2, g + d.off_t_b2, B, D, D, st));
  if (B <= 16 && uwu_skinny_linear_ok(B, D, D) && D <= 512) RUN(uwu_skinny_linear_dgrad(P.at<float>(L.dc), w32 + d.off_t_w2, P.at<float>(L.dth), B, D, D, st));
  else RUN(lin_dgrad(P.at(L.dc), w32 + d.off_t_w2, P.at(L.dth), nullptr, B, D, D, UWU_F32, st));
  RUN(uwu_silu_bwd(P.at(L.t_pre), P.at(L.dth), P.at(L.dtp), (int64_t)B * D, UWU_F32, st));
  RUN(lin_wgrad32(P.at<float>(L.dtp), P.at<float>(L.feat), g + d.off_t_w1, g + d.off_t_b1, B, D, d.freq_dim, st));
  return UWU_OK;
}

extern "C" int uwu_dit_backward_cond(const uwu_dit_desc* dp, const float* cond, void* st) {
  RUN(check_desc(dp));
  const uwu_dit_desc& d = *dp;
  if (d.cond_dim <= 0) return UWU_OK;
  if (!cond || !d.g32) { uwu_set_error("dit_backward_cond: null tensor"); return UWU_EINVAL; }
  const Layout L = make_layout(d);
  Ptrs P{static_cast<char*>(d.ws), L};
  return lin_wgrad32(P.at<float>(L.dc), cond, d.g32 + d.off_y_w, d.g32 + d.off_y_b, d.B, d.D, d.cond_dim, st);
}
```

uwudiff_amd/csrc/gemm.hip:

```cpp
#include "gemm_shared.h"

namespace {

template <typename T, typename TC, bool TA, bool TB, bool ACC, bool GL = false, int EPI = -1>
__global__ void __launch_bounds__(256, 2) gemm_kernel(const GemmArgs g) {
  extern __shared__ __attribute__((aligned(16))) char smem[];
  constexpr int BK = GT<T>::BK;
  const int tid = threadIdx.x, lane = tid & 63, wave = tid >> 6;
  const int wm = wave >> 1, wn = wave & 1;

  const int nblk = g.tiles_m * g.tiles_n;
  int tile;
  {
    const int bid = blockIdx.x, xcd = bid & 7, loc = bid >> 3;
    const int q = nblk >> 3, rm = nblk & 7;
    tile = (xcd < rm ? xcd * (q + 1) : rm * (q + 1) + (xcd - rm) * q) + loc;
  }
  const int tm = tile / g.tiles_n, tn = tile - tm * g.tiles_n;
  const int m0 = tm * BM, n0 = tn * BN;

  const int ktiles = (g.K + BK - 1) / BK;
  const int kt_begin = blockIdx.z * g.k_tiles_per_split;
  int kt_end = kt_begin + g.k_tiles_per_split;
  if (kt_end > ktiles) kt_end = ktiles;
// ... 364 lines not shown
    for (int kk = 0; kk < 2; ++kk) {
      uint4 bf[4], af[8];
      if constexpr (!TB) {
#pragma unroll
        for (int j = 0; j < 4; ++j) bf[j] = lds_read128_asm(lb + swz((wn & 1) * 64 + 16 * j + fr, 4 * kk + fq));
      } else {
        const unsigned sub = smem_base + (unsigned)((s & 1) * STAGE + 2 * TILE_BYTES + (2 * kk + (wn >> 1)) * R_BSUB);
#pragma unroll
        for (int j = 0; j < 4; ++j) {
          const uint2 lo = t_read_tr<0>(sub + (b_t0 ^ (unsigned)(j << 5)));
          const uint2 hi = t_read_tr<0>(sub + (b_t1 ^ (unsigned)(j << 5)));
          bf[j] = uint4{lo.x, lo.y, hi.x, hi.y};
        }
      }
#pragma unroll
      for (int i = 0; i < 4; ++i) af[i] = lds_read128_asm(la + swz(16 * i + fr, 4 * kk + fq));
      asm volatile("s_waitcnt lgkmcnt(0)" ::: "memory");
#pragma unroll
      for (int i = 4; i < 8; ++i) af[i] = lds_read128_asm(la + swz(16 * i + fr, 4 * kk + fq));
      __builtin_amdgcn_sched_barrier(0);
#pragma unroll
      for (int i = 0; i < 4; ++i)
#pragma unroll
        for (int j = 0; j < 4; ++j) mma_frag<T>(bf[j], af[i], acc[i][j]);
      asm volatile("s_waitcnt lgkmcnt(0)" ::: "memory");
      __builtin_amdgcn_sched_barrier(0);
#pragma unroll
      for (int i = 4; i < 8; ++i)
#pragma unroll
        for (int j = 0; j < 4; ++j) mma_frag<T>(bf[j], af[i], acc[i][j]);
    }
  }
  EpiPre<T, 8, 4> pre;
  epi_prefetch<T, 8, 4, EPI>(pre, g, m0 + wm * 128, n0 + wn * 64, fr, fq);
  epilogue_tile<T, TC, 8, 4, EPI>(acc, pre, g, m0 + wm * 128, n0 + wn * 64, fr, fq,
                                  reinterpret_cast<float*>(smem) + (wn >> 1) * 256, wm, wn & 1, wm == 0 ? (tid & 127) : 128);
}

template <typename TC, int EPI, bool TB>
__global__ void __launch_bounds__(512, 2) gemm_wide_kernel(const GemmArgs g) {
  extern __shared__ __attribute__((aligned(16))) char smem[];
  typedef bf16_t T;
  constexpr int FI = 6, FJ = 6, BMR = 192, BNC = 384;
  constexpr int A_BYTES = BMR * ROW_BYTES, STAGE = (BMR + BNC) * ROW_BYTES;
  const int tid = threadIdx.x, lane = tid & 63, wave = tid >> 6;
  const int wm = wave >> 2, wn = wave & 3;
  const int fr = lane & 15, fq = lane >> 4;
  const int nblk = g.tiles_m * g.tiles_n;
  int tile;
  {
    const int bid = blockIdx.x, xcd = bid & 7, loc = bid >> 3;
    const int q = nblk >> 3, rm = nblk & 7;
    tile = (xcd < rm ? xcd * (q + 1) : rm * (q + 1) + (xcd - rm) * q) + loc;
  }
  const int tm = tile / g.tiles_n, tn = tile - tm * g.tiles_n;
  const int m0 = tm * BMR, n0 = tn * BNC;
  const int nk = g.K >> 6;
  const T* A = static_cast<const T*>(g.A);
  const T* B = static_cast<const T*>(g.B);

  const T* pa[3];
  const T* pb[6];
#pragma unroll
  for (int q = 0; q < 3; ++q) {
    const int row = 8 * (wave + 8 * q) + (lane >> 3);
    const int c = ((lane & 7) ^ (row >> 1) ^ (row >> 4)) & 7;
    int grow = m0 + row;
    if (grow >= g.M) grow = g.M - 1;
    pa[q] = A + (int64_t)grow * g.lda + 8 * c;
  }
#pragma unroll
  for (int q = 0; q < 6; ++q) {
    if constexpr (!TB) {
      const int row = 8 * (wave + 8 * q) + (lane >> 3);
      const int c = ((lane & 7) ^ (row >> 1) ^ (row >> 4)) & 7;
      int grow = n0 + row;
      if (grow >= g.N) grow = g.N - 1;
      pb[q] = B + (int64_t)grow * g.ldb + 8 * c;
    } else {
      const int kh = q / 3, nh = q - 3 * kh;
      const int drow = lane >> 4;
      const int dchunk = (lane & 15) ^ (((drow & 3) << 2) | (wave & 3));
      int x = n0 + 128 * nh + 8 * dchunk;
      if (x > g.N - 8) x = g.N - 8;
      pb[q] = B + (int64_t)(32 * kh + 4 * wave + drow) * g.ldb + x;
    }
  }
  const bool a_once = g.tiles_n == 1;
  auto issue = [&](int s) {
    char* st = smem + (s & 1) * STAGE;
    if (a_once) {
#pragma unroll
      for (int q = 0; q < 3; ++q)
        __builtin_amdgcn_global_load_lds((const __attribute__((address_space(1))) void*)(pa[q] + 64 * s),
                                         (__attribute__((address_space(3))) void*)(st + (wave + 8 * q) * 1024), 16, 0, 2);
    } else {
#pragma unroll
      for (int q = 0; q < 3; ++q)
        __builtin_amdgcn_global_load_lds((const __attribute__((address_space(1))) void*)(pa[q] + 64 * s),
                                         (__attribute__((address_space(3))) void*)(st + (wave + 8 * q) * 1024), 16, 0, 0);
    }
#pragma unroll
    for (int q = 0; q < 6; ++q) {
      if constexpr (!TB)
        __builtin_amdgcn_global_load_lds((const __attribute__((address_space(1))) void*)(pb[q] + 64 * s),
                                         (__attribute__((address_space(3))) void*)(st + A_BYTES + (wave + 8 * q) * 1024),
// ... 434 lines not shown
    RETURN_IF(uwu_conv3x3_args(g, B, H, W, C, 2));
    g.cHo = Ho; g.cWo = Wo;
    g.A = x; g.B = w; g.C = y; g.bias = bias;
    g.M = B * Ho * Wo; g.N = Cout; g.K = 9 * C; g.lda = C; g.ldb = 9 * C; g.ldc = Cout;
    g.epi = bias ? UWU_EPI_BIAS : UWU_EPI_NONE;
    g.wide = (Cout % 8 == 0) ? 1 : 0;
    if (bias) return launch_r3<bf16_t, UWU_EPI_BIAS, false, 8, 3>(g, st);
    return launch_r3<bf16_t, UWU_EPI_NONE, false, 8, 3>(g, st);
  }
  const size_t need = (size_t)B * Ho * Wo * 9 * C * (dtype == UWU_BF16 ? 2 : 4);
  UWU_CHECK_ARG(ws && ws_bytes >= need && ((uintptr_t)ws & 15) == 0,
                "conv3x3_s2br_fwd: this shape needs a 16-byte aligned workspace of %zu bytes (uwu_conv3x3_s2br_ws_bytes)", need);
  RETURN_IF(uwu_im2col3x3_s2br(x, ws, B, H, W, C, dtype, st));
  return uwu_gemm(ws, w, y, nullptr, bias, nullptr, B * Ho * Wo, Cout, 9 * C, 9 * C, 9 * C, Cout, 0, 0, 0, dtype, dtype,
                  bias ? UWU_EPI_BIAS : UWU_EPI_NONE, 1, stream);
}

extern "C" int uwu_gemm(const void* A, const void* B, void* C, void* C2, const float* bias, const void* aux, int M,
                        int N, int K, int lda, int ldb, int ldc, int ldaux, int transA, int transB, int dtype,
                        int c_dtype, int epilogue, int split_k, void* stream) {
  UWU_CHECK_ARG(A && B && C, "gemm: null operand");
  UWU_CHECK_ARG(M > 0 && N > 0 && K > 0, "gemm: bad shape M=%d N=%d K=%d", M, N, K);
  UWU_CHECK_ARG(dtype == UWU_F32 || dtype == UWU_BF16, "gemm: bad dtype %d", dtype);
  UWU_CHECK_ARG(c_dtype == UWU_F32 || c_dtype == dtype, "gemm: c_dtype must be fp32 or the operand dtype");
  const int epc = dtype == UWU_BF16 ? 8 : 4;
  const int bk = dtype == UWU_BF16 ? 64 : 32;
  UWU_CHECK_ARG((((uintptr_t)A | (uintptr_t)B) & 15) == 0, "gemm: A/B must be 16-byte aligned");
  UWU_CHECK_ARG(lda % epc == 0 && ldb % epc == 0, "gemm: lda/ldb must be multiples of %d", epc);
  UWU_CHECK_ARG(transA ? (M % epc == 0) : (K % epc == 0), "gemm: A contiguous extent must be a multiple of %d", epc);
  UWU_CHECK_ARG(transB ? (N % epc == 0) : (K % epc == 0), "gemm: B contiguous extent must be a multiple of %d", epc);
  UWU_CHECK_ARG(lda >= (transA ? M : K) && ldb >= (transB ? N : K), "gemm: leading dimension too small");
  UWU_CHECK_ARG(epilogue >= UWU_EPI_NONE && epilogue <= UWU_EPI_ACCUM, "gemm: bad epilogue %d", epilogue);
  const bool acc = epilogue == UWU_EPI_ACCUM;
  if (!acc) {
    UWU_CHECK_ARG(split_k <= 1, "gemm: split_k needs UWU_EPI_ACCUM");
    UWU_CHECK_ARG(N % 4 == 0 && ldc % 4 == 0 && ldc >= N, "gemm: N and ldc must be multiples of 4");
    const int cal = c_dtype == UWU_BF16 ? 7 : 15;
    UWU_CHECK_ARG(((uintptr_t)C & cal) == 0, "gemm: C misaligned");
    if (epilogue == UWU_EPI_BIAS || epilogue == UWU_EPI_BIAS_GELU || epilogue == UWU_EPI_BIAS_SILU)
      UWU_CHECK_ARG(bias && ((uintptr_t)bias & 15) == 0, "gemm: bias missing/misaligned");
    if (epilogue == UWU_EPI_BIAS_GELU || epilogue == UWU_EPI_BIAS_SILU)
      UWU_CHECK_ARG(C2 && ((uintptr_t)C2 & cal) == 0, "gemm: C2 missing/misaligned");
    if (epilogue == UWU_EPI_DGELU)
      UWU_CHECK_ARG(aux && ldaux % 4 == 0 && ldaux >= N && ((uintptr_t)aux & (dtype == UWU_BF16 ? 7 : 15)) == 0,
                    "gemm: aux missing/misaligned");
  } else {
    UWU_CHECK_ARG(c_dtype == UWU_F32 && ldc >= N, "gemm: ACCUM needs fp32 C");
  }
  GemmArgs g{};
  g.A = A; g.B = B; g.C = C; g.C2 = C2; g.bias = bias; g.aux = aux;
  g.M = M; g.N = N; g.K = K; g.lda = lda; g.ldb = ldb; g.ldc = ldc; g.ldaux = ldaux; g.epi = epilogue;
  g.tiles_m = (M + BM - 1) / BM;
  g.tiles_n = (N + BN - 1) / BN;
  g.wide = (!acc && c_dtype == UWU_BF16 && N % 8 == 0 && ldc % 8 == 0 && ((uintptr_t)C & 15) == 0 &&
            (C2 == nullptr || epilogue == UWU_EPI_DGELU || ((uintptr_t)C2 & 15) == 0)) ? 1 : 0;
  g.aux16 = (epilogue == UWU_EPI_DGELU && dtype == UWU_BF16 && N % 8 == 0 && ldaux % 8 == 0 && ((uintptr_t)aux & 15) == 0) ? 1 : 0;

  const int ktiles = (K + bk - 1) / bk;
  int split = split_k < 1 ? 1 : split_k;
  if (split > ktiles) split = ktiles;
  g.k_tiles_per_split = (ktiles + split - 1) / split;
  split = (ktiles + g.k_tiles_per_split - 1) / g.k_tiles_per_split;
  hipStream_t st = (hipStream_t)stream;
  if (dtype == UWU_BF16) {
    if (c_dtype == UWU_BF16) return dispatch_trans<bf16_t, bf16_t>(g, transA, transB, acc, split, st);
    return dispatch_trans<bf16_t, float>(g, transA, transB, acc, split, st);
  }
  return dispatch_trans<float, float>(g, transA, transB, acc, split, st);
}
```

uwudiff_amd/csrc/gemm_as.hip:

```cpp
#include "gemm_shared.h"

namespace {

constexpr int AS_K = 384, AS_BN = 64, AS_STAGE = AS_BN * AS_K * 2;
constexpr int AS_NST = 3;
constexpr int AS_LDS = AS_NST * AS_STAGE + 8192;
template <typename TC, int EPI>
__global__ void __launch_bounds__(512, 2) gemm_as_kernel(const GemmArgs g) {
  extern __shared__ __attribute__((aligned(16))) char smem[];
  typedef bf16_t T;
  constexpr int FI = 2, FJ = 4, KS = AS_K / 32;
  const int tid = threadIdx.x, lane = tid & 63;
  const int wave = __builtin_amdgcn_readfirstlane(tid >> 6);
  const int fr = lane & 15, fq = lane >> 4;
  const int m0 = blockIdx.x * 256 + wave * 32;
  const T* A = static_cast<const T*>(g.A);
  const T* B = static_cast<const T*>(g.B);
  float* bias_lds = reinterpret_cast<float*>(smem + AS_NST * AS_STAGE);
  if (EPI == UWU_EPI_BIAS || EPI == UWU_EPI_BIAS_GELU)
    for (int n = tid; n < g.N; n += 512) bias_lds[n] = g.bias[n];

  uint4 af[FI][KS];
#pragma unroll
  for (int i = 0; i < FI; ++i)
#pragma unroll
    for (int s = 0; s < KS; ++s)
      af[i][s] = *reinterpret_cast<const uint4*>(A + (int64_t)(m0 + 16 * i + fr) * g.lda + 32 * s + 8 * fq);

  const int drow = 8 * wave + (lane >> 3);
  const int dc = ((lane & 7) ^ (drow >> 1) ^ (drow >> 4)) & 7;
  const T* bsrc = B + (int64_t)drow * g.ldb + 8 * dc;
  const unsigned smem_base = (unsigned)(size_t)((const __attribute__((address_space(3))) char*)smem);
  auto issue = [&](int c) {
    const T* p = bsrc + (int64_t)c * AS_BN * g.ldb;
#pragma unroll
    for (int q = 0; q < AS_K / 64; ++q)
      glds16_asm(p + 64 * q, smem_base + (unsigned)((c % AS_NST) * AS_STAGE + q * 8192 + wave * 1024));
  };
  const int nchunks = g.N / AS_BN;
  static_assert(EPI == UWU_EPI_BIAS_GELU || EPI == UWU_EPI_BIAS || EPI == UWU_EPI_DGELU, "the interleaved epilogues");
  constexpr int NS = EPI == UWU_EPI_BIAS ? 4 : 8;
  TC* const C = static_cast<TC*>(g.C);
  TC* const C2 = static_cast<TC*>(g.C2);
  const bool odd = fq & 1;
  auto pack = [](const f32x4& v) {
    bf16x4 b = {(bf16_t)v[0], (bf16_t)v[1], (bf16_t)v[2], (bf16_t)v[3]};
    return *reinterpret_cast<uint2*>(&b);
  };
  uint4 auxr[4];
  const T* const auxp = static_cast<const T*>(g.aux);
  auto aux_load = [&](int n0, int u) {
    const int i = u >> 1, jp = u & 1;
    const int m = m0 + 16 * i + fr, n = n0 + 32 * jp + (odd ? 16 + 4 * (fq - 1) : 4 * fq);
    auxr[u] = *reinterpret_cast<const uint4*>(auxp + (int64_t)m * g.ldaux + n);
  };
  auto epi_unit = [&](const f32x4 (&pa)[FI][FJ], int n0, int i, int jp) {
    f32x4 v0 = pa[i][2 * jp], v1 = pa[i][2 * jp + 1];
    typedef unsigned su32x2 __attribute__((ext_vector_type(2)));
    typedef unsigned su32x4 __attribute__((ext_vector_type(4)));
    if constexpr (EPI == UWU_EPI_DGELU) {
      const uint4 a = auxr[2 * i + jp];
      const su32x2 sx = __builtin_amdgcn_permlane16_swap(a.x, a.z, false, false);
      const su32x2 sy = __builtin_amdgcn_permlane16_swap(a.y, a.w, false, false);
      const uint2 r0 = {sx[0], sy[0]}, r1 = {sx[1], sy[1]};
      const bf16x4 u0 = *reinterpret_cast<const bf16x4*>(&r0), u1 = *reinterpret_cast<const bf16x4*>(&r1);
      v0 = v0 * dgelu_tanh_f4(f32x4{(float)u0[0], (float)u0[1], (float)u0[2], (float)u0[3]});
      v1 = v1 * dgelu_tanh_f4(f32x4{(float)u1[0], (float)u1[1], (float)u1[2], (float)u1[3]});
    } else {
      const float* bl = bias_lds + n0 + 32 * jp + 4 * fq;
      v0 = v0 + *reinterpret_cast<const f32x4*>(bl);
      v1 = v1 + *reinterpret_cast<const f32x4*>(bl + 16);
    }
    const int m = m0 + 16 * i + fr;
    const int n = n0 + 32 * jp + (odd ? 16 + 4 * (fq - 1) : 4 * fq);
    auto exchange_store = [&](TC* dst, const f32x4& x0, const f32x4& x1, bool stream_out) {
      const uint2 p0 = pack(x0), p1 = pack(x1);
      const su32x2 sx = __builtin_amdgcn_permlane16_swap(p0.x, p1.x, false, false);
      const su32x2 sy = __builtin_amdgcn_permlane16_swap(p0.y, p1.y, false, false);
      const su32x4 o = su32x4{sx[0], sy[0], sx[1], sy[1]};
      su32x4* ptr = reinterpret_cast<su32x4*>(dst + (int64_t)m * g.ldc + n);
      if (stream_out) __builtin_nontemporal_store(o, ptr);
      else *ptr = o;
    };
    if constexpr (EPI == UWU_EPI_BIAS_GELU) {
      exchange_store(C, v0, v1, true);
      exchange_store(C2, gelu_tanh_f4(v0), gelu_tanh_f4(v1), false);
    } else {
      exchange_store(C, v0, v1, false);
    }
  };
  f32x4 prev[FI][FJ];
#pragma unroll
  for (int i = 0; i < FI; ++i)
#pragma unroll
    for (int j = 0; j < FJ; ++j) prev[i][j] = f32x4{0.f, 0.f, 0.f, 0.f};
  issue(0);
  issue(1);
  for (int c = 0; c < nchunks; ++c) {
    if (c == 0) asm volatile("s_waitcnt vmcnt(6) lgkmcnt(0)" ::: "memory");
    else if (c <= 2 || c + 1 >= nchunks) asm volatile("s_waitcnt vmcnt(0)" ::: "memory");
    else asm volatile("s_waitcnt vmcnt(%0)" ::"n"(2 * NS + 6) : "memory");
    __builtin_amdgcn_s_barrier();
    if (c + 2 < nchunks) issue(c + 2);
    const char* lb = smem + (c % AS_NST) * AS_STAGE;
    f32x4 acc[FI][FJ];
#pragma unroll
    for (int i = 0; i < FI; ++i)
#pragma unroll
      for (int j = 0; j < FJ; ++j) acc[i][j] = f32x4{0.f, 0.f, 0.f, 0.f};
    constexpr int NBF = EPI == UWU_EPI_DGELU ? 1 : 2;
    uint4 bf[NBF][FJ];
    auto frags = [&](uint4 (&dst)[FJ], int s) {
#pragma unroll
      for (int j = 0; j < FJ; ++j)
        dst[j] = *reinterpret_cast<const uint4*>(lb + (s >> 1) * 8192 + swz(16 * j + fr, 4 * (s & 1) + fq));
    };
    if constexpr (NBF == 2) frags(bf[0], 0);
#pragma unroll
    for (int s = 0; s < KS; ++s) {
      if constexpr (NBF == 2) {
        if (s + 1 < KS) frags(bf[(s + 1) & 1], s + 1);
      } else {
        frags(bf[0], s);
      }
#pragma unroll
      for (int i = 0; i < FI; ++i)
#pragma unroll
        for (int j = 0; j < FJ; ++j) mma_frag<T>(bf[s & (NBF - 1)][j], af[i][s], acc[i][j]);
      if (s % 3 == 1) {
        if (c > 0) epi_unit(prev, (c - 1) * AS_BN, (s / 3) >> 1, (s / 3) & 1);
        if constexpr (EPI == UWU_EPI_DGELU) aux_load(c * AS_BN, s / 3);
      }
    }
#pragma unroll
    for (int i = 0; i < FI; ++i)
#pragma unroll
      for (int j = 0; j < FJ; ++j) prev[i][j] = acc[i][j];
  }
#pragma unroll
  for (int u = 0; u < 4; ++u) epi_unit(prev, (nchunks - 1) * AS_BN, u >> 1, u & 1);
}

}

bool uwu_gemm_use_as(const GemmArgs& g, int out_bytes) {
  static UwuEnv on("UWU_GEMM_AS");
  if (on.get().is('0')) return false;
  return g.K == AS_K && g.M % 256 == 0 && g.M >= 256 * 256 && g.N % AS_BN == 0 && g.N <= 2048 && g.N >= 1024 && out_bytes == 2 &&
         g.lda % 8 == 0 &&
         g.ldb % 8 == 0 && g.ldc % 8 == 0 && (((uintptr_t)g.A | (uintptr_t)g.B | (uintptr_t)g.C | (uintptr_t)g.C2) & 15) == 0;
}
bool uwu_gemm_use_as_bias() {
  static UwuEnv on("UWU_GEMM_AS_BIAS");
  return !on.get().is('0');
}


template <typename TC, int EPI>
int uwu_launch_gemm_as(GemmArgs g, hipStream_t st) {
  g.wide = 1;
  return gemm_launch<gemm_as_kernel<TC, EPI>>("gemm_as", AS_LDS, dim3(g.M / 256), 512, st, gemm_prof(g, false, sizeof(TC)), g);
}

template int uwu_launch_gemm_as<bf16_t, UWU_EPI_BIAS>(GemmArgs, hipStream_t);
template int uwu_launch_gemm_as<bf16_t, UWU_EPI_BIAS_GELU>(GemmArgs, hipStream_t);
template int uwu_launch_gemm_as<bf16_t, UWU_EPI_DGELU>(GemmArgs, hipStream_t);
```

uwudiff_amd/csrc/gemm_p8n.hip:

```cpp
#include "gemm_shared.h"

namespace {

constexpr int N8_HT = 128 * ROW_BYTES;
template <int FI> struct N8 {
  static constexpr int AROWS = 32 * FI, AB = AROWS * ROW_BYTES, PAR = 3 * N8_HT + AB, RING = 2 * PAR;
  static constexpr int BIAS = RING, LDS = BIAS + 8 * 512;
  static constexpr int APIECES = AROWS / 64;
  static constexpr int VM = 2 * 4 + APIECES;
};

template <typename TC, int EPI, bool TB, int FI>
__global__ void __launch_bounds__(512, 2) gemm_p8n_kernel(const GemmArgs g) {
  typedef N8<FI> G;
  extern __shared__ __attribute__((aligned(16))) char smem[];
  typedef bf16_t T;
  const int tid = threadIdx.x, lane = tid & 63;
  const int wave = __builtin_amdgcn_readfirstlane(tid >> 6);
  const int grp = wave >> 2, wc = wave & 3;
  const int fr = lane & 15, fq = lane >> 4;
  const int nblk = g.tiles_m * g.tiles_n;
  const int nk = g.K >> 6;
  auto tile_of = [&](int L) __attribute__((always_inline)) {
    const int xcd = L & 7, loc = L >> 3;
    const int q = nblk >> 3, rm = nblk & 7;
    return (xcd < rm ? xcd * (q + 1) : rm * (q + 1) + (xcd - rm) * q) + loc;
  };

  constexpr int NOA = FI == 6 ? 1 : G::APIECES;
  unsigned oa[NOA], ob;
  const char* abase;
  const char* bbase;
  auto setup = [&](int tile, int& m0, int& n0) __attribute__((always_inline)) {
    const int tm = tile / g.tiles_n, tn = tile - tm * g.tiles_n;
    m0 = tm * G::AROWS;
    n0 = tn * 384;
    abase = reinterpret_cast<const char*>(static_cast<const T*>(g.A) + (int64_t)m0 * g.lda);
    bbase = reinterpret_cast<const char*>(static_cast<const T*>(g.B) + (TB ? (int64_t)n0 : (int64_t)n0 * g.ldb));
    int lane_ = lane;
    asm volatile("" : "+v"(lane_));
#pragma unroll
    for (int q = 0; q < NOA; ++q) {
      const int row = 8 * (wave + 8 * q) + (lane_ >> 3);
      const int c = ((lane_ & 7) ^ (row >> 1)) & 7;
      int ga = row;
      if (ga >= g.M - m0) ga = g.M - m0 - 1;
      oa[q] = (unsigned)(ga * g.lda + 8 * c) * 2u;
    }
    if constexpr (!TB) {
      const int row = 8 * wave + (lane >> 3);
      ob = (unsigned)(row * g.ldb + 8 * (((lane & 7) ^ (row >> 1)) & 7)) * 2u;
    } else {
      const int drow = lane >> 4;
      const int dchunk = (lane & 15) ^ (((drow & 3) << 2) | (wave & 3));
      ob = (unsigned)((4 * wave + drow) * g.ldb + 8 * dchunk) * 2u;
    }
  };
  auto boff = [&](int y, int q) __attribute__((always_inline)) {
    return TB ? (int64_t)64 * q * g.ldb + 256 * y : ((int64_t)128 * y + 64 * q) * g.ldb * 2;
  };
  const int64_t bstep = TB ? (int64_t)128 * g.ldb : 128;
  auto issue = [&](auto ec, auto pc, int kt) __attribute__((always_inline)) {
    constexpr int e = decltype(ec)::value, par = decltype(pc)::value;
    constexpr int y = e == 0 ? 0 : e - 1;
    char* slot = smem + par * G::PAR + (e == 1 ? 3 : y) * N8_HT;
    if constexpr (e == 1) {
#pragma unroll
      for (int q = 0; q < G::APIECES; ++q)
        __builtin_amdgcn_global_load_lds((const __attribute__((address_space(1))) void*)(abase + (int64_t)kt * 128 +
                                                                                      (NOA == 1 ? (int64_t)128 * q * g.lda + oa[0] : (int64_t)oa[q % NOA])),
                                         (__attribute__((address_space(3))) void*)(slot + (wave + 8 * q) * 1024), 16, 0, 0);
    } else {
#pragma unroll
      for (int q = 0; q < 2; ++q) {
        char* dst = TB ? slot + q * R_BSUB + wave * 1024 : slot + (wave + 8 * q) * 1024;
        __builtin_amdgcn_global_load_lds((const __attribute__((address_space(1))) void*)(bbase + kt * bstep + boff(y, q) + ob),
                                         (__attribute__((address_space(3))) void*)dst, 16, 0, 0);
      }
    }
// ... 238 lines not shown
```

uwudiff_amd/csrc/gemm_shared.h:

```cpp
#pragma once
#include <stdlib.h>

#include <atomic>
#include <type_traits>

#include "common.h"

#define RETURN_IF(...)             \
  do {                             \
    const int rc_ = (__VA_ARGS__); \
    if (rc_ != UWU_OK) return rc_; \
  } while (0)

extern std::atomic<const char*> g_uwu_gemm_last_kernel;

struct GemmArgs {
  const void* A;
  const void* B;
  void* C;
  void* C2;
  const float* bias;
  const void* aux;
  int M, N, K, lda, ldb, ldc, ldaux, epi, tiles_m, tiles_n, k_tiles_per_split, wide;
  int xs, nloc, part_m;
  int aux16;
  int cH, cW, cC, cHo, cWo, cS;
  const void* zero;
  void* q8;
  void* q8t;
  const float* q_scale;
  float* q_amax;
  int ldq, ldqt;
};

namespace {

constexpr int BM = 128, BN = 128;
constexpr int ROW_BYTES = 128;
constexpr int TILE_BYTES = 128 * ROW_BYTES;

template <typename T> struct GT;
template <> struct GT<bf16_t> { static constexpr int EPC = 8; static constexpr int BK = 64; };
template <> struct GT<float> { static constexpr int EPC = 4; static constexpr int BK = 32; };

__device__ __forceinline__ int swz(int row, int chunk) {
  return row * ROW_BYTES + (((chunk ^ (row >> 1) ^ (row >> 4)) & 7) << 4);
}

typedef unsigned gu32x4 __attribute__((ext_vector_type(4)));
__device__ __forceinline__ uint4 lds_read128_asm(const char* p) {
  gu32x4 v;
  const unsigned a = (unsigned)(size_t)((const __attribute__((address_space(3))) char*)p);
  asm volatile("ds_read_b128 %0, %1" : "=v"(v) : "v"(a) : "memory");
  return uint4{v[0], v[1], v[2], v[3]};
}

template <typename T, bool TRANS>
struct Stager {
  uint4 r[4];

  __device__ __forceinline__ void load(const T* __restrict__ base, int ld, int row0, int k0, int nrows, int K,
                                       int tid) {
    constexpr int EPC = GT<T>::EPC;
    if constexpr (!TRANS) {
      const int c = tid & 7, rr = tid >> 3;
      const int kk = k0 + c * EPC;
#pragma unroll
      for (int p = 0; p < 4; ++p) {
        const int grow = row0 + rr + 32 * p;
        if (grow < nrows && kk < K)
          r[p] = *reinterpret_cast<const uint4*>(base + (int64_t)grow * ld + kk);
        else
          r[p] = uint4{0, 0, 0, 0};
      }
    } else if constexpr (sizeof(T) == 2) {
      const int xg = tid & 15, kg = tid >> 4;
      const int x = row0 + 8 * xg;
#pragma unroll
      for (int kr = 0; kr < 4; ++kr) {
        const int k = k0 + 4 * kg + kr;
        if (k < K && x < nrows)
          r[kr] = *reinterpret_cast<const uint4*>(base + (int64_t)k * ld + x);
        else
          r[kr] = uint4{0, 0, 0, 0};
      }
// ... 365 lines not shown
```

uwudiff_amd/csrc/norm.hip:

```cpp
#include "common.h"

namespace {
__device__ __forceinline__ f32x8 load8_nt(const float* p) { return load8(p); }
__device__ __forceinline__ f32x8 load8_nt(const bf16_t* p) {
  typedef unsigned nu32x4 __attribute__((ext_vector_type(4)));
  nu32x4 raw = __builtin_nontemporal_load(reinterpret_cast<const nu32x4*>(p));
  bf16x8 v = *reinterpret_cast<bf16x8*>(&raw);
  f32x8 r;
#pragma unroll
  for (int i = 0; i < 8; ++i) r[i] = (float)v[i];
  return r;
}
__device__ __forceinline__ void store8_nt(float* p, f32x8 v) { store8(p, v); }
__device__ __forceinline__ void store8_nt(bf16_t* p, f32x8 v) {
  typedef unsigned nu32x4 __attribute__((ext_vector_type(4)));
  bf16x8 o;
#pragma unroll
  for (int i = 0; i < 8; ++i) o[i] = (bf16_t)v[i];
  __builtin_nontemporal_store(*reinterpret_cast<nu32x4*>(&o), reinterpret_cast<nu32x4*>(p));
}

template <typename T> struct Raw8;
template <> struct Raw8<float> { typedef f32x8 type; };
template <> struct Raw8<bf16_t> { typedef bf16x8 type; };
__device__ __forceinline__ f32x8 raw8_nt(const float* p) { return load8(p); }
__device__ __forceinline__ bf16x8 raw8_nt(const bf16_t* p) {
  typedef unsigned nu32x4 __attribute__((ext_vector_type(4)));
  nu32x4 raw = __builtin_nontemporal_load(reinterpret_cast<const nu32x4*>(p));
  return *reinterpret_cast<bf16x8*>(&raw);
}
__device__ __forceinline__ f32x8 raw8(const float* p) { return load8(p); }
__device__ __forceinline__ bf16x8 raw8(const bf16_t* p) { return *reinterpret_cast<const bf16x8*>(p); }
__device__ __forceinline__ f32x8 unpack8(f32x8 v) { return v; }
__device__ __forceinline__ f32x8 unpack8(bf16x8 v) {
  f32x8 r;
#pragma unroll
  for (int i = 0; i < 8; ++i) r[i] = (float)v[i];
  return r;
}

constexpr int MAX_D = 4096;

template <typename T, int MAX_IT>
__global__ void __launch_bounds__(256) add_ln_mod_fwd_kernel(const T* __restrict__ x_in, const T* __restrict__ y,
                                                             const float* __restrict__ gate,
                                                             const float* __restrict__ shift,
                                                             const float* __restrict__ scale, int mod_ld,
                                                             T* __restrict__ x_out, T* __restrict__ h,
                                                             float* __restrict__ mean_o, float* __restrict__ rstd_o,
                                                             int M, int T_tok, int D, float eps, int affine) {
  const int lane = threadIdx.x & 63, wave = threadIdx.x >> 6;
  const int nit = (D + 511) >> 9;
  for (int row = blockIdx.x * 4 + wave; row < M; row += gridDim.x * 4) {
    const int b = row / T_tok;
    const int64_t off = (int64_t)row * D;
    f32x8 v[MAX_IT];
    float s = 0.f;
#pragma unroll
    for (int it = 0; it < MAX_IT; ++it) {
      const int d = it * 512 + lane * 8;
      if (it < nit && d < D) {
        f32x8 xv = load8_nt(x_in + off + d);
        if (y) {
          f32x8 yv = load8_nt(y + off + d), gv = load8(gate + (int64_t)b * mod_ld + d);
          xv = xv + gv * yv;
          if constexpr (sizeof(T) == 2) {
#pragma unroll
            for (int e = 0; e < 8; ++e) xv[e] = (float)(bf16_t)xv[e];
          }
          store8_nt(x_out + off + d, xv);
        }
        v[it] = xv;
        _Pragma("unroll") for (int e = 0; e < 8; ++e) s += xv[e];
      } else {
        v[it] = f32x8{0.f, 0.f, 0.f, 0.f, 0.f, 0.f, 0.f, 0.f};
      }
    }
    const float mean = wave_sum(s) / (float)D;
    float q = 0.f;
#pragma unroll
    for (int it = 0; it < MAX_IT; ++it) {
      const int d = it * 512 + lane * 8;
      if (it < nit && d < D) {
#pragma unroll
        for (int e = 0; e < 8; ++e) {
          float c = v[it][e] - mean;
          q += c * c;
        }
      }
    }
    const float var = wave_sum(q) / (float)D;
    const float rstd = 1.f / sqrtf(var + eps);
    if (lane == 0) {
      mean_o[row] = mean;
      rstd_o[row] = rstd;
    }
#pragma unroll
    for (int it = 0; it < MAX_IT; ++it) {
      const int d = it * 512 + lane * 8;
      if (it < nit && d < D) {
        f32x8 o;
#pragma unroll
        for (int e = 0; e < 8; ++e) o[e] = (v[it][e] - mean) * rstd;
        if (scale) {
          f32x8 sc = load8(scale + (int64_t)b * mod_ld + d), sh = load8(shift + (int64_t)b * mod_ld + d);
#pragma unroll
          for (int e = 0; e < 8; ++e) o[e] = o[e] * (affine ? sc[e] : 1.f + sc[e]) + sh[e];
        }
        store8(h + off + d, o);
      }
    }
  }
}

template <typename T, int NCH>
__global__ void __launch_bounds__(256) add_ln_mod_fwd16_kernel(const T* __restrict__ x_in, const T* __restrict__ y,
                                                               const float* __restrict__ gate,
                                                               const float* __restrict__ shift,
                                                               const float* __restrict__ scale, int mod_ld,
                                                               T* __restrict__ x_out, T* __restrict__ h,
                                                               float* __restrict__ mean_o, float* __restrict__ rstd_o,
                                                               int M, int T_tok, float eps, int affine) {
  constexpr int D = 128 * NCH;
  const int lane = threadIdx.x & 63, wave = threadIdx.x >> 6;
  const int sub = lane >> 4, l16 = lane & 15;
  for (int row0 = (blockIdx.x * 4 + wave) * 4; row0 < M; row0 += gridDim.x * 16) {
    const int row = row0 + sub;
    const bool ok = row < M;
    const int rc = ok ? row : M - 1;
    const int b = rc / T_tok;
    const int64_t off = (int64_t)rc * D + 8 * l16;
    const float* gb = gate + (int64_t)b * mod_ld + 8 * l16;
    f32x8 v[NCH];
    float s = 0.f;
#pragma unroll
    for (int cidx = 0; cidx < NCH; ++cidx) {
      f32x8 xv = load8_nt(x_in + off + 128 * cidx);
      if (y) {
        const f32x8 yv = load8_nt(y + off + 128 * cidx), gv = load8(gb + 128 * cidx);
        xv = xv + gv * yv;
        if constexpr (sizeof(T) == 2) {
#pragma unroll
          for (int e = 0; e < 8; ++e) xv[e] = (float)(bf16_t)xv[e];
        }
        if (ok) store8_nt(x_out + off + 128 * cidx, xv);
      }
      v[cidx] = xv;
#pragma unroll
      for (int e = 0; e < 8; ++e) s += xv[e];
    }
    const float mean = row16_sum(s) * (1.f / (float)D);
    float q = 0.f;
#pragma unroll
    for (int cidx = 0; cidx < NCH; ++cidx)
#pragma unroll
      for (int e = 0; e < 8; ++e) {
        const float c = v[cidx][e] - mean;
        q += c * c;
      }
    const float var = row16_sum(q) * (1.f / (float)D);
    const float rstd = 1.f / sqrtf(var + eps);
    if (l16 == 0 && ok) {
      mean_o[row] = mean;
      rstd_o[row] = rstd;
    }
#pragma unroll
    for (int cidx = 0; cidx < NCH; ++cidx) {
      f32x8 o;
#pragma unroll
      for (int e = 0; e < 8; ++e) o[e] = (v[cidx][e] - mean) * rstd;
      if (scale) {
        const f32x8 sc = load8(scale + (int64_t)b * mod_ld + 8 * l16 + 128 * cidx), sh = load8(shift + (int64_t)b * mod_ld + 8 * l16 + 128 * cidx);
#pragma unroll
        for (int e = 0; e < 8; ++e) o[e] = o[e] * (affine ? sc[e] : 1.f + sc[e]) + sh[e];
      }
      if (ok) store8(h + off + 128 * cidx, o);
    }
  }
}
// ... 86 lines not shown
      const int d = it * 512 + lane * 8;
      if (it < nit && d < D) {
        f32x8 o;
        const f32x8 sc = load8(scale + (int64_t)b * mod_ld + d), sh = load8(shift + (int64_t)b * mod_ld + d);
        const f32x8 xv = unpack8(v[it]);
#pragma unroll
        for (int e = 0; e < 8; ++e) {
          o[e] = (xv[e] - mean) * rstd * (1.f + sc[e]) + sh[e];
          mx = fmaxf(mx, fabsf(o[e]));
        }
        const unsigned lo = q8_pack4(o[0], o[1], o[2], o[3], qs), hi = q8_pack4(o[4], o[5], o[6], o[7], qs);
        *reinterpret_cast<uint2*>(q8 + (int64_t)row * ldq + d) = uint2{lo, hi};
        *reinterpret_cast<uint2*>(img + (8 * wave + r) * pitch + d) = uint2{lo, hi};
      }
    }
  }
  mx = wave_max(mx);
  if (lane == 0) red[wave] = mx;
  __syncthreads();
  if (q_amax && threadIdx.x == 0) {
    float a = red[0];
#pragma unroll
    for (int w = 1; w < NW; ++w) a = fmaxf(a, red[w]);
    const unsigned cur = __hip_atomic_load(reinterpret_cast<unsigned*>(q_amax), __ATOMIC_RELAXED, __HIP_MEMORY_SCOPE_AGENT);
    if (__float_as_uint(a) > cur) atomicMax(reinterpret_cast<unsigned*>(q_amax), __float_as_uint(a));
  }
  constexpr int RB = NW / 2;
  const int nq = D >> 2;
  for (int idx = threadIdx.x; idx < RB * nq; idx += 64 * NW) {
    const int cq = idx / RB, rb = idx - cq * RB;
    const unsigned* src = reinterpret_cast<const unsigned*>(img + (16 * rb) * pitch) + cq;
    unsigned w[16];
#pragma unroll
    for (int i = 0; i < 16; ++i) w[i] = src[i * (pitch >> 2)];
#pragma unroll
    for (int e = 0; e < 4; ++e) {
      const unsigned sel = 0x0c0c0400u + (unsigned)e * 0x0101u;
      uint4 o;
      o.x = __builtin_amdgcn_perm(w[1], w[0], sel) | (__builtin_amdgcn_perm(w[3], w[2], sel) << 16);
      o.y = __builtin_amdgcn_perm(w[5], w[4], sel) | (__builtin_amdgcn_perm(w[7], w[6], sel) << 16);
      o.z = __builtin_amdgcn_perm(w[9], w[8], sel) | (__builtin_amdgcn_perm(w[11], w[10], sel) << 16);
      o.w = __builtin_amdgcn_perm(w[13], w[12], sel) | (__builtin_amdgcn_perm(w[15], w[14], sel) << 16);
      *reinterpret_cast<uint4*>(q8t + (int64_t)(4 * cq + e) * ldqt + row0 + 16 * rb) = o;
    }
  }
}

template <typename T, int MAX_IT, int NW = 4>
__global__ void __launch_bounds__(64 * NW) add_ln_mod_bwd_kernel(
    const T* __restrict__ dh, const T* __restrict__ x, const float* __restrict__ mean_i,
    const float* __restrict__ rstd_i, const float* __restrict__ scale, const T* __restrict__ dx_in,
    const T* __restrict__ y, const float* __restrict__ gate, int mod_ld, T* __restrict__ dx_out, T* __restrict__ dy,
    float* __restrict__ dshift, float* __restrict__ dscale, float* __restrict__ dgate, int M, int T_tok, int D,
    int rows_per_block, int affine) {
  extern __shared__ __attribute__((aligned(16))) float red[];
  const int lane = threadIdx.x & 63, wave = threadIdx.x >> 6;
  const int nit = (D + 511) >> 9;
  const int row0 = blockIdx.x * rows_per_block;
  const int b = row0 / T_tok;
  f32x8 a_sh[MAX_IT], a_sc[MAX_IT], a_g[MAX_IT];
#pragma unroll
  for (int it = 0; it < MAX_IT; ++it) a_sh[it] = a_sc[it] = a_g[it] = f32x8{0.f, 0.f, 0.f, 0.f, 0.f, 0.f, 0.f, 0.f};

  for (int r = wave; r < rows_per_block; r += NW) {
    const int row = row0 + r;
    if (row >= M) break;
    const int64_t off = (int64_t)row * D;
    const float mean = mean_i[row], rstd = rstd_i[row];
    if constexpr (MAX_IT == 1) {
      f32x8 xh[MAX_IT], g[MAX_IT];
      float s1 = 0.f, s2 = 0.f;
  #pragma unroll
      for (int it = 0; it < MAX_IT; ++it) {
        const int d = it * 512 + lane * 8;
        if (it < nit && d < D) {
          f32x8 xv = load8_nt(x + off + d), dv = load8(dh + off + d);
          f32x8 sc = scale ? load8(scale + (int64_t)b * mod_ld + d)
                           : (affine ? f32x8{1.f, 1.f, 1.f, 1.f, 1.f, 1.f, 1.f, 1.f} : f32x8{0.f, 0.f, 0.f, 0.f, 0.f, 0.f, 0.f, 0.f});
  #pragma unroll
          for (int e = 0; e < 8; ++e) {
            float xhat = (xv[e] - mean) * rstd;
            float gg = dv[e] * (affine ? sc[e] : 1.f + sc[e]);
            xh[it][e] = xhat;
            g[it][e] = gg;
            s1 += gg;
            s2 += gg * xhat;
            a_sh[it][e] += dv[e];
            a_sc[it][e] += dv[e] * xhat;
          }
        }
      }
      s1 = wave_sum(s1) / (float)D;
      s2 = wave_sum(s2) / (float)D;
  #pragma unroll
      for (int it = 0; it < MAX_IT; ++it) {
        const int d = it * 512 + lane * 8;
        if (it < nit && d < D) {
          f32x8 dx;
  #pragma unroll
          for (int e = 0; e < 8; ++e) dx[e] = rstd * (g[it][e] - s1 - xh[it][e] * s2);
          if (dx_in) dx = dx + load8_nt(dx_in + off + d);
          store8_nt(dx_out + off + d, dx);
          if (y) {
            f32x8 yv = load8_nt(y + off + d), gv = load8(gate + (int64_t)b * mod_ld + d);
            store8(dy + off + d, gv * dx);
  #pragma unroll
            for (int e = 0; e < 8; ++e) a_g[it][e] += dx[e] * yv[e];
          }
        }
      }
    } else {
// ... 203 lines not shown
  UWU_CHECK_ARG(x_in && q8 && q8t && q_scale && mean && rstd && shift && scale, "add_ln_modulate_fwd_q8: null pointer");
  UWU_CHECK_ARG(B > 0 && T > 0 && D > 0 && D % 8 == 0 && D <= 1536, "add_ln_modulate_fwd_q8: D=%d unsupported", D);
  UWU_CHECK_ARG(((int64_t)B * T) % 64 == 0, "add_ln_modulate_fwd_q8: B*T must be a multiple of 64");
  UWU_CHECK_ARG((y == nullptr) || (gate && x_out), "add_ln_modulate_fwd_q8: y needs gate and x_out");
  UWU_CHECK_ARG(mod_ld % 4 == 0, "add_ln_modulate_fwd_q8: mod_ld must be a multiple of 4");
  UWU_CHECK_ARG((((uintptr_t)x_in | (uintptr_t)y | (uintptr_t)x_out | (uintptr_t)q8t) & 15) == 0 && ((uintptr_t)q8 & 7) == 0,
                "add_ln_modulate_fwd_q8: misaligned tensor");
  const int M = B * T;
  UWU_CHECK_ARG(ldq >= D && ldq % 8 == 0 && ldqt >= M && ldqt % 16 == 0, "add_ln_modulate_fwd_q8: bad leading dimension");
  hipStream_t st = (hipStream_t)stream;
  const int nw = (size_t)64 * (D + 8) * 2 <= 150 * 1024 ? 8 : 4;
  UWU_CHECK_ARG(M % (8 * nw) == 0, "add_ln_modulate_fwd_q8: B*T must be a multiple of %d", 8 * nw);
  const size_t lds = (size_t)8 * nw * (D + 8);
  UwuProfScope prof(stream);
#define Q8_LAUNCH(NIT, NW)                                                                                                 \
  {                                                                                                                        \
    static unsigned char done[UWU_MAX_DEV];                                                                                \
    if (!uwu_func_lds(reinterpret_cast<const void*>(add_ln_mod_fwd_q8_kernel<NIT, NW>), 8 * NW * (1536 + 8), done)) {    \
      uwu_set_error("add_ln_modulate_fwd_q8: the device cannot give a workgroup %d bytes of LDS", 8 * NW * (1536 + 8));   \
      return UWU_ELAUNCH;                                                                                                  \
    }                                                                                                                      \
    hipLaunchKernelGGL((add_ln_mod_fwd_q8_kernel<NIT, NW>), dim3(M / (8 * NW)), dim3(64 * NW), lds, st,                   \
                       (const bf16_t*)x_in, (const bf16_t*)y, gate, shift, scale, mod_ld, (bf16_t*)x_out,                 \
                       (unsigned char*)q8, ldq, (unsigned char*)q8t, ldqt, q_scale, q_amax, mean, rstd, M, T, D, eps);     \
  }
#define Q8_CASE(NIT)                \
  case NIT:                         \
    if (nw == 8) Q8_LAUNCH(NIT, 8)  \
    else Q8_LAUNCH(NIT, 4)          \
    break;
  switch ((D + 511) / 512) { Q8_CASE(1) Q8_CASE(2) Q8_CASE(3) }
#undef Q8_CASE
#undef Q8_LAUNCH
  const double md = (double)M * D;
  prof.done(UWU_PROF_LN_FWD, 0, 8.0 * md, md * (2.0 * (1 + (y ? 2 : 0)) + 2.0));
  UWU_LAUNCH_CHECK("add_ln_modulate_fwd_q8");
  return UWU_OK;
}

extern "C" int uwu_add_ln_modulate_fwd(const void* x_in, const void* y, const float* gate, const float* shift,
                                       const float* scale, int mod_ld, void* x_out, void* h, float* mean, float* rstd,
                                       int B, int T, int D, float eps, int affine, int dtype, void* stream) {
  UWU_CHECK_ARG(x_in && h && mean && rstd, "add_ln_modulate_fwd: null pointer");
  UWU_CHECK_ARG(B > 0 && T > 0 && D > 0 && D % 8 == 0 && D <= MAX_D, "add_ln_modulate_fwd: D=%d unsupported", D);
  UWU_CHECK_ARG((y == nullptr) || (gate && x_out), "add_ln_modulate_fwd: y needs gate and x_out");
  UWU_CHECK_ARG((scale == nullptr) == (shift == nullptr), "add_ln_modulate_fwd: scale/shift go together");
  UWU_CHECK_ARG(!scale || mod_ld % 4 == 0, "add_ln_modulate_fwd: mod_ld must be a multiple of 4");
  UWU_CHECK_ARG((((uintptr_t)x_in | (uintptr_t)h) & 15) == 0, "add_ln_modulate_fwd: tensors must be 16-byte aligned");
  const int M = B * T;
  int grid = (M + 3) / 4;
  if (grid > 8192) grid = 8192;
  hipStream_t st = (hipStream_t)stream;
  UWU_CHECK_ARG(dtype == UWU_F32 || dtype == UWU_BF16, "add_ln_modulate_fwd: bad dtype");
  UwuProfScope prof(stream);
  static UwuEnv r16("UWU_LN_ROW16");
  const bool al16 = (((uintptr_t)x_in | (uintptr_t)h | (uintptr_t)y | (uintptr_t)x_out) & 15) == 0 && (mod_ld % 4 == 0);
  if (!r16.get().is('0') && D % 128 == 0 && D <= (r16.get().is('1') ? 1536 : 768) && al16 && M >= 4096) {
    int g16 = (M + 15) / 16;
    if (g16 > 4096) g16 = 4096;
#define F16_CASE(NCH)                                                                                                          \
  case NCH:                                                                                                                    \
    if (dtype == UWU_F32)                                                                                                      \
      hipLaunchKernelGGL((add_ln_mod_fwd16_kernel<float, NCH>), dim3(g16), dim3(256), 0, st, (const float*)x_in, (const float*)y, \
                         gate, shift, scale, mod_ld, (float*)x_out, (float*)h, mean, rstd, M, T, eps, affine);                   \
    else                                                                                                                       \
      hipLaunchKernelGGL((add_ln_mod_fwd16_kernel<bf16_t, NCH>), dim3(g16), dim3(256), 0, st, (const bf16_t*)x_in,            \
                         (const bf16_t*)y, gate, shift, scale, mod_ld, (bf16_t*)x_out, (bf16_t*)h, mean, rstd, M, T, eps,       \
                         affine);                                                                                               \
    break;
    switch (D / 128) {
      F16_CASE(1) F16_CASE(2) F16_CASE(3) F16_CASE(4) F16_CASE(5) F16_CASE(6) F16_CASE(7) F16_CASE(8) F16_CASE(9) F16_CASE(10)
      F16_CASE(11) F16_CASE(12)
    }
#undef F16_CASE
    const double e = dtype == UWU_BF16 ? 2.0 : 4.0, md = (double)M * D;
    prof.done(UWU_PROF_LN_FWD, dtype == UWU_BF16 ? 0 : 1, 8.0 * md, md * e * (2 + (y ? 1 : 0) + (x_out && x_out != x_in ? 1 : 0)));
    UWU_LAUNCH_CHECK("add_ln_modulate_fwd");
    return UWU_OK;
  }
#define FWD_CASE(NIT)                                                                                              \
  case NIT:                                                                                                        \
    if (dtype == UWU_F32)                                                                                          \
      hipLaunchKernelGGL((add_ln_mod_fwd_kernel<float, NIT>), dim3(grid), dim3(256), 0, st, (const float*)x_in,    \
                         (const float*)y, gate, shift, scale, mod_ld, (float*)x_out, (float*)h, mean, rstd, M, T, D, \
                         eps, affine);                                                                                     \
    else                                                                                                           \
      hipLaunchKernelGGL((add_ln_mod_fwd_kernel<bf16_t, NIT>), dim3(grid), dim3(256), 0, st, (const bf16_t*)x_in,  \
                         (const bf16_t*)y, gate, shift, scale, mod_ld, (bf16_t*)x_out, (bf16_t*)h, mean, rstd, M,  \
                         T, D, eps, affine);                                                                               \
    break;
  switch ((D + 511) / 512) {
    FWD_CASE(1) FWD_CASE(2) FWD_CASE(3) FWD_CASE(4) FWD_CASE(5) FWD_CASE(6) FWD_CASE(7) FWD_CASE(8)
  }
#undef FWD_CASE
  {
    const double e = dtype == UWU_BF16 ? 2.0 : 4.0, md = (double)M * D;
    prof.done(UWU_PROF_LN_FWD, dtype == UWU_BF16 ? 0 : 1, 8.0 * md, md * e * (2 + (y ? 1 : 0) + (x_out && x_out != x_in ? 1 : 0)));
  }
  UWU_LAUNCH_CHECK("add_ln_modulate_fwd");
  return UWU_OK;
}

extern "C" int uwu_add_ln_modulate_bwd(const void* dh, const void* x, const float* mean, const float* rstd,
                                       const float* scale, const void* dx_in, const void* y, const float* gate,
                                       int mod_ld, void* dx_out, void* dy, float* dshift, float* dscale, float* dgate,
                                       int B, int T, int D, int affine, int dtype, void* stream) {
  UWU_CHECK_ARG(dh && x && mean && rstd && dx_out, "add_ln_modulate_bwd: null pointer");
  UWU_CHECK_ARG(B > 0 && T > 0 && D > 0 && D % 8 == 0 && D <= MAX_D, "add_ln_modulate_bwd: D=%d unsupported", D);
  UWU_CHECK_ARG((((uintptr_t)dh | (uintptr_t)x | (uintptr_t)dx_out) & 15) == 0, "add_ln_modulate_bwd: tensors must be 16-byte aligned");
  UWU_CHECK_ARG((y == nullptr) || (gate && dy), "add_ln_modulate_bwd: y needs gate and dy");
  UWU_CHECK_ARG(!(scale || y) || mod_ld % 4 == 0, "add_ln_modulate_bwd: mod_ld must be a multiple of 4");
  const int M = B * T;
  hipStream_t st = (hipStream_t)stream;
  UWU_CHECK_ARG(dtype == UWU_F32 || dtype == UWU_BF16, "add_ln_modulate_bwd: bad dtype");
  if (affine && mod_ld == 0 && scale && !y && dshift && dscale && D <= 2048 && (dx_in == nullptr || ((uintptr_t)dx_in & 15) == 0)) {
    const int rpb = M >= 16384 ? 64 : (M >= 4096 ? 32 : 16);
    const int grid = (M + rpb - 1) / rpb;
    const size_t lds2 = (size_t)8 * 2 * D * sizeof(float);
    if (lds2 > 64 * 1024) {
      static unsigned char done[2][4][UWU_MAX_DEV];
      for (int nit = 1; nit <= 4; ++nit) {
        const void* kf = nullptr;
        if (dtype == UWU_F32)
          kf = nit == 1 ? (const void*)ln_affine_bwd_kernel<float, 1> : nit == 2 ? (const void*)ln_affine_bwd_kernel<float, 2>
               : nit == 3 ? (const void*)ln_affine_bwd_kernel<float, 3> : (const void*)ln_affine_bwd_kernel<float, 4>;
        else
          kf = nit == 1 ? (const void*)ln_affine_bwd_kernel<bf16_t, 1> : nit == 2 ? (const void*)ln_affine_bwd_kernel<bf16_t, 2>
               : nit == 3 ? (const void*)ln_affine_bwd_kernel<bf16_t, 3> : (const void*)ln_affine_bwd_kernel<bf16_t, 4>;
        if (!uwu_func_lds(kf, 160 * 1024, done[dtype == UWU_F32][nit - 1])) {
          uwu_set_error("ln_affine_bwd: the device cannot give a workgroup %d bytes of LDS", 160 * 1024);
          return UWU_ELAUNCH;
        }
      }
    }
    UwuProfScope prof(stream);
#define AFF_CASE(NIT)                                                                                                   \
  case NIT:                                                                                                             \
    if (dtype == UWU_F32)                                                                                               \
      hipLaunchKernelGGL((ln_affine_bwd_kernel<float, NIT>), dim3(grid), dim3(512), lds2, st, (const float*)dh,         \
                         (const float*)x, mean, rstd, scale, (const float*)dx_in, (float*)dx_out, dshift, dscale, M, D, \
                         rpb);                                                                                          \
    else                                                                                                                \
      hipLaunchKernelGGL((ln_affine_bwd_kernel<bf16_t, NIT>), dim3(grid), dim3(512), lds2, st, (const bf16_t*)dh,       \
                         (const bf16_t*)x, mean, rstd, scale, (const bf16_t*)dx_in, (bf16_t*)dx_out, dshift, dscale, M, \
                         D, rpb);                                                                                       \
    break;
    switch ((D + 511) / 512) {
      AFF_CASE(1) AFF_CASE(2) AFF_CASE(3) AFF_CASE(4)
    }
#undef AFF_CASE
    const double e = dtype == UWU_BF16 ? 2.0 : 4.0, md = (double)M * D;
    prof.done(UWU_PROF_LN_BWD, dtype == UWU_BF16 ? 0 : 1, 16.0 * md, md * e * (3 + (dx_in ? 1 : 0)));
    UWU_LAUNCH_CHECK("ln_affine_bwd");
    return UWU_OK;
  }
  int rows = 32;
  while (rows > 1 && T % rows) rows >>= 1;
  const bool small = M / rows < 1024 && T % 16 == 0 && D <= 640;
  if (small) rows = 16;
  while (!small && rows > 4 && M / rows < 1024) rows >>= 1;
  const size_t lds = (size_t)(small ? 8 : (D > 1024 ? 1 : 4)) * 3 * D * sizeof(float);
  if (small) {
    UwuProfScope prof(stream);
#define SMALL_CASE(NIT)                                                                                                \
  case NIT:                                                                                                            \
    hipLaunchKernelGGL((add_ln_mod_bwd_kernel<bf16_t, NIT, 8>), dim3(M / rows), dim3(512), lds, st, (const bf16_t*)dh, \
                       (const bf16_t*)x, mean, rstd, scale, (const bf16_t*)dx_in, (const bf16_t*)y, gate, mod_ld,      \
                       (bf16_t*)dx_out, (bf16_t*)dy, dshift, dscale, dgate, M, T, D, rows, affine);                    \
    break;
    if (dtype == UWU_BF16) {
      switch ((D + 511) / 512) { SMALL_CASE(1) SMALL_CASE(2) }
#undef SMALL_CASE
      const double md = (double)M * D;
      prof.done(UWU_PROF_LN_BWD, 0, 16.0 * md, md * 2.0 * (3 + (dx_in ? 1 : 0) + (y ? 2 : 0)));
      UWU_LAUNCH_CHECK("add_ln_modulate_bwd");
      return UWU_OK;
    }
  }
  UWU_CHECK_ARG(lds <= 160 * 1024, "add_ln_modulate_bwd: D=%d needs %zu B of LDS (> 160 KB)", D, lds);
  UwuProfScope prof(stream);
#define BWD_CASE(NIT)                                                                                               \
  case NIT:                                                                                                         \
    if (lds > 64 * 1024) {                      \
      static unsigned char done[2][UWU_MAX_DEV];                                                                    \
      const void* kf = dtype == UWU_F32 ? reinterpret_cast<const void*>(add_ln_mod_bwd_kernel<float, NIT>)          \
                                        : reinterpret_cast<const void*>(add_ln_mod_bwd_kernel<bf16_t, NIT>);        \
      if (!uwu_func_lds(kf, 160 * 1024, done[dtype == UWU_F32])) {                                                  \
        uwu_set_error("add_ln_modulate_bwd: the device cannot give a workgroup %d bytes of LDS", 160 * 1024);       \
        return UWU_ELAUNCH;                                                                                         \
      }                                                                                                             \
    }                                                                                                               \
    if (dtype == UWU_F32)                                                                                           \
      hipLaunchKernelGGL((add_ln_mod_bwd_kernel<float, NIT>), dim3(M / rows), dim3(256), lds, st, (const float*)dh, \
                         (const float*)x, mean, rstd, scale, (const float*)dx_in, (const float*)y, gate, mod_ld,    \
                         (float*)dx_out, (float*)dy, dshift, dscale, dgate, M, T, D, rows, affine);                         \
    else                                                                                                            \
      hipLaunchKernelGGL((add_ln_mod_bwd_kernel<bf16_t, NIT>), dim3(M / rows), dim3(256), lds, st,                  \
                         (const bf16_t*)dh, (const bf16_t*)x, mean, rstd, scale, (const bf16_t*)dx_in,              \
                         (const bf16_t*)y, gate, mod_ld, (bf16_t*)dx_out, (bf16_t*)dy, dshift, dscale, dgate, M, T,   \
                         D, rows, affine);                                                                                  \
    break;
  switch ((D + 511) / 512) {
    BWD_CASE(1) BWD_CASE(2) BWD_CASE(3) BWD_CASE(4) BWD_CASE(5) BWD_CASE(6)
    default:
      UWU_CHECK_ARG(false, "add_ln_modulate_bwd: D=%d > 3072 not instantiated", D);
  }
#undef BWD_CASE
  {
    const double e = dtype == UWU_BF16 ? 2.0 : 4.0, md = (double)M * D;
    prof.done(UWU_PROF_LN_BWD, dtype == UWU_BF16 ? 0 : 1, 16.0 * md, md * e * (3 + (dx_in ? 1 : 0) + (y ? 2 : 0)));
  }
  UWU_LAUNCH_CHECK("add_ln_modulate_bwd");
  return UWU_OK;
}

static int colsum_impl(const void* X, int dtype, int batch, int M, int N, int ldx, float* out, int accumulate,
                       void* stream);
extern "C" int uwu_colsum(const void* X, int dtype, int M, int N, int ldx, float* out, int accumulate, void* stream) {
  return colsum_impl(X, dtype, 1, M, N, ldx, out, accumulate, stream);
}
extern "C" int uwu_colsum_batched(const void* X, int dtype, int batch, int M, int N, int ldx, float* out,
                                  int accumulate, void* stream) {
  return colsum_impl(X, dtype, batch, M, N, ldx, out, accumulate, stream);
}
static int colsum_impl(const void* X, int dtype, int batch, int M, int N, int ldx, float* out, int accumulate,
                       void* stream) {
  UWU_CHECK_ARG(X && out && batch > 0 && M > 0 && N > 0 && N % 4 == 0 && ldx % 4 == 0 && ldx >= N,
                "colsum: bad args (N=%d ldx=%d)", N, ldx);
  hipStream_t st = (hipStream_t)stream;
  if (!accumulate) {
    if (hipMemsetAsync(out, 0, (size_t)batch * N * sizeof(float), st) != hipSuccess) {
      uwu_set_error("colsum: memset failed");
      return UWU_ELAUNCH;
    }
  }
  int splits = (M + 255) / 256;
  const int strips = (N + 63) / 64;
  int want = 1024 / (strips * batch);
  if (want < 1) want = 1;
  if (splits > want) splits = want;
  const int rows = (M + splits - 1) / splits;
  splits = (M + rows - 1) / rows;
  if (dtype == UWU_F32)
    hipLaunchKernelGGL((colsum_kernel<float>), dim3(strips, splits, batch), dim3(256), 0, st, (const float*)X, M, N, ldx,
                       out, rows);
  else if (dtype == UWU_BF16)
    hipLaunchKernelGGL((colsum_kernel<bf16_t>), dim3(strips, splits, batch), dim3(256), 0, st, (const bf16_t*)X, M, N,
                       ldx, out, rows);
  else
    UWU_CHECK_ARG(false, "colsum: bad dtype");
  UWU_LAUNCH_CHECK("colsum");
  return UWU_OK;
}
// ... 1 lines not shown
```

uwudiff_amd/lib.py:

```python
import ctypes
import os
from ctypes import c_char_p, c_double, c_float, c_int, c_int32, c_int64, c_size_t, c_void_p

import torch

_HERE = os.path.dirname(os.path.abspath(__file__))
LIB_PATH = os.path.join(_HERE, "libuwu_hip.so")

F32, BF16, I64 = 0, 1, 2
PT = {"epsilon": 0, "v_prediction": 1, "sample": 2, "rectified_flow": 3}
EPI_NONE, EPI_BIAS, EPI_BIAS_GELU, EPI_DGELU, EPI_BIAS_SILU, EPI_ACCUM = 0, 1, 2, 3, 4, 5
ACT = {"quick_gelu": 0, "gelu": 1}
GATE = {"gated-gelu": 0}
FILTER = {"bilinear": 0, "bicubic": 1, "lanczos": 2}


class UwuError(RuntimeError):
    pass


class DitDesc(ctypes.Structure):
    _fields_ = (
        [(n, c_int32) for n in ("B", "T", "D", "H", "L", "mlp_ratio", "in_ch", "out_ch", "patch", "img", "dtype",
                                "cond_dim", "freq_dim")]
        + [("ln_eps", c_float), ("mod_total", c_int32)]
        + [("w", c_void_p), ("w32", c_void_p), ("g32", c_void_p)]
        + [(n, c_int64) for n in ("off_patch_w", "off_patch_b", "off_t_w1", "off_t_b1", "off_t_w2", "off_t_b2",
                                  "off_y_w", "off_y_b", "off_mod_w", "off_mod_b", "off_final_w", "off_final_b",
                                  "off_layer0", "layer_stride")]
        + [("pos", c_void_p), ("ws", c_void_p), ("ws_bytes", c_size_t), ("layer_done", c_void_p)]
        + [("side_stream", c_void_p)]
        + [("rope", c_int32), ("off_rope_h", c_int64), ("off_rope_w", c_int64), ("pos_xy", c_void_p)]
        + [("fp8", c_int32), ("f8_scale", c_void_p), ("f8_amax", c_void_p), ("f8_fmt", c_void_p)]
        + [("checkpoint", c_int32)]
    )


P = c_void_p
_SIGS = {
    "uwu_last_error": (c_char_p, []),
    "uwu_version": (c_int, []),
    "uwu_env_refresh": (c_int, []),
    "uwu_memset_zero": (c_int, [P, ctypes.c_uint64, P]),
    "uwu_schedule_gather": (c_int, [P, P, P, P, c_int, c_int, c_int, c_float, c_int, P, P]),
    "uwu_rf_time_to_sigma": (c_int, [P, c_float, P, c_int, c_int, P, P, P]),
    "uwu_qsample": (c_int, [P, P, P, c_int, c_int64, P, P, P]),
    "uwu_philox_raw": (c_int, [P, c_int64, ctypes.c_uint64, ctypes.c_uint64, P]),
    "uwu_philox_normal": (c_int, [P, c_int64, ctypes.c_uint64, ctypes.c_uint64, P]),
    "uwu_draw_timesteps": (c_int, [P, c_int, c_int, ctypes.c_uint64, ctypes.c_uint64, P]),
    "uwu_draw_u01": (c_int, [P, c_int, ctypes.c_uint64, ctypes.c_uint64, P]),
    "uwu_qsample_draw": (c_int, [P, P, c_int, c_int64, c_int, c_float, c_float, P, P, P, ctypes.c_uint64, ctypes.c_uint64, P]),
    "uwu_posterior_draw": (c_int, [P, c_int, c_int, c_int, c_int64, P, P, P, ctypes.c_uint64, ctypes.c_uint64, P]),
    "uwu_qsample_norm": (c_int, [P, P, P, c_int, c_int64, c_float, c_float, P, P, P]),
    "uwu_ctx_place": (c_int, [P, c_int, P, P] + [c_int] * 7 + [P]),
    "uwu_loss_fwd_bwd": (c_int, [P, P, P, P, c_int, P, c_int, c_int, c_int, c_int, c_int64, P, P, P, P, P, P]),
    "uwu_scale_inplace": (c_int, [P, c_int, c_int64, P, P]),
    "uwu_scale_into": (c_int, [P, P, c_int, c_int64, P, P]),
    "uwu_cast_i64_to_f32": (c_int, [P, P, c_int64, P]),
    "uwu_sampler_step": (c_int, [P, P, P, P, P, P, c_int64, c_float, c_float, c_float, c_float, c_float, P]),
    "uwu_aggregate_concat": (c_int, [P, P, P, c_int, c_int, c_int64, c_int, ctypes.c_uint64, P]),
    "uwu_aggregate_split": (c_int, [P, P, P, c_int, c_int, c_int64, P]),
    "uwu_aggregate_first": (c_int, [P, P, P, c_int, c_int64, P]),
    "uwu_sampler_combine": (c_int, [P, P, P, P, P, c_int64, c_float, c_float, c_float, c_float, P]),
    "uwu_scale_copy": (c_int, [P, P, c_int64, c_float, P]),
    "uwu_cfg_input": (c_int, [P, P, c_int, c_int64, c_float, P]),
    "uwu_sampler_combine_draw": (c_int, [P, P, P, P, c_int64, c_float, c_float, c_float, c_float, ctypes.c_uint64, ctypes.c_uint64, P]),
    "uwu_latent_finish_ws_bytes": (ctypes.c_size_t, [c_int, c_int64]),
    "uwu_latent_finish": (c_int, [P, P, c_int, c_int64, c_int, c_float, c_float, P, ctypes.c_size_t, P]),
    "uwu_image_u8": (c_int, [P, c_int, P, c_int, c_int, c_int, P]),
    "uwu_resample_ksize": (c_int, [c_int, c_int, c_int]),
    "uwu_resample_coeffs": (c_int, [c_int, c_int, c_int, c_int, c_int, P, P]),
    "uwu_image_resize_crop_ws_bytes": (ctypes.c_size_t, [c_int, P, c_int, c_int, c_int]),
    "uwu_image_resize_crop": (c_int, [P, c_int64, P, P, P, c_int64, P, P] + [c_int] * 6 + [P, ctypes.c_size_t, P]),
    "uwu_grad_sqnorm_clip": (c_int, [P, c_int64, c_float, c_float, P, P, P]),
    "uwu_adamw_step": (c_int, [P, P, P, P, P, c_int64, c_float, c_float, c_float, c_float, c_float, c_int, c_float,
                               P, c_int, P]),
    "uwu_lion_step": (c_int, [P, P, P, P, c_int64, c_double, c_double, c_double, c_double, c_float, P, c_int, P]),
    "uwu_adamw_fp16_step": (c_int, [P, P, P, P, P, c_int64, c_double, c_double, c_double, c_double, c_int, c_float, P,
                                    c_int, P]),
    "uwu_param_decay": (c_int, [P, P, c_int64, c_double, P]),
    "uwu_adamw8_step": (c_int, [P] * 9 + [c_int64] * 3 + [c_double] * 5 + [c_int, c_float, P, c_int, P]),
    "uwu_lion8_step": (c_int, [P] * 6 + [c_int64] * 3 + [c_double] * 4 + [c_float, P, c_int, P]),
    "uwu_prodigy_stats_blocks": (c_int, [c_int64]),
    "uwu_prodigy_stats": (c_int, [P] * 6 + [c_int64, P, P, c_int64, c_int64] + [c_double] * 5 + [c_int, c_double, c_int, c_int,
                                  c_float, P, c_int, P]),
    "uwu_prodigy_finalize": (c_int, [P, P, c_int64] + [c_double] * 7 + [c_int, P]),
    "uwu_prodigy_apply": (c_int, [P, P, P, P, c_int64, P, c_double, c_double, c_int, P]),
    "uwu_ema_update": (c_int, [P, P, c_int64, c_float, c_float, P]),
    "uwu_ema_swap": (c_int, [P, P, P, c_int64, c_int, P]),
    "uwu_cast_f32_to_bf16": (c_int, [P, P, c_int64, P]),
    "uwu_cast_bf16_to_f32": (c_int, [P, P, c_int64, P]),
    "uwu_adapter_merge": (c_int, [P, P, P, P, c_int, c_int64, P, P, P]),
    "uwu_adapter_grad": (c_int, [P, c_int64, c_int64, c_int, P, P, c_int64, c_int64, c_int64, c_int, c_int, c_int, c_float,
                                 P, c_int64, P]),
    "uwu_adapter_dora_norms": (c_int, [P, P, P, P, P, c_int, c_int64, P, P]),
# ... 162 lines not shown
```

uwudiff_amd/ops.py:

```python
import ctypes

import torch

from . import lib as L


def gemm(a, b, *, trans_a=False, trans_b=False, bias=None, aux=None, epilogue=L.EPI_NONE, out=None, out2=None,
         c_dtype=None, split_k=1, M=None, N=None, K=None):
    assert a.dim() == 2 and b.dim() == 2 and a.dtype == b.dtype
    if M is None:
        M, K_ = (a.shape[1], a.shape[0]) if trans_a else a.shape
        N, Kb = (b.shape[1], b.shape[0]) if trans_b else b.shape
        assert K_ == Kb, (a.shape, b.shape, trans_a, trans_b)
        K = K_
    c_dtype = c_dtype or a.dtype
    if out is None:
        out = (torch.zeros if epilogue == L.EPI_ACCUM else torch.empty)(M, N, device=a.device, dtype=c_dtype)
    if epilogue in (L.EPI_BIAS_GELU, L.EPI_BIAS_SILU) and out2 is None:
        out2 = torch.empty(M, N, device=a.device, dtype=c_dtype)
    L.call("uwu_gemm", L.ptr(a), L.ptr(b), L.ptr(out), L.ptr(out2), L.ptr(bias), L.ptr(aux), M, N, K, a.stride(0),
           b.stride(0), out.stride(0), aux.stride(0) if aux is not None else 0, int(trans_a), int(trans_b), L.dt(a),
           L.dt(out), epilogue, split_k, L.stream())
    return (out, out2) if out2 is not None else out


def add_ln_modulate_fwd(x_in, B, T, *, y=None, gate=None, shift=None, scale=None, mod_ld=0, eps=1e-6, affine=False):
    M, D = x_in.shape
    x_out = torch.empty_like(x_in) if y is not None else x_in
    h = torch.empty_like(x_in)
    mean = torch.empty(M, device=x_in.device, dtype=torch.float32)
    rstd = torch.empty_like(mean)
    L.call("uwu_add_ln_modulate_fwd", L.ptr(x_in), L.ptr(y), _p(gate), _p(shift), _p(scale), mod_ld, L.ptr(x_out),
           L.ptr(h), L.ptr(mean), L.ptr(rstd), B, T, D, eps, int(affine), L.dt(x_in), L.stream())
    return x_out, h, mean, rstd


def add_ln_modulate_fwd_q8(x_in, B, T, q_scale, *, shift, scale, mod_ld, y=None, gate=None, eps=1e-6, amax=None):
    M, D = x_in.shape
    x_out = torch.empty_like(x_in) if y is not None else x_in
    q8 = torch.empty(M, D, device=x_in.device, dtype=torch.uint8)
    q8t = torch.empty(D, M, device=x_in.device, dtype=torch.uint8)
    mean = torch.empty(M, device=x_in.device, dtype=torch.float32)
    rstd = torch.empty_like(mean)
    L.call("uwu_add_ln_modulate_fwd_q8", L.ptr(x_in), L.ptr(y), _p(gate), _p(shift), _p(scale), mod_ld, L.ptr(x_out), L.ptr(q8), D,
           L.ptr(q8t), M, L.ptr(q_scale), L.ptr(amax), L.ptr(mean), L.ptr(rstd), B, T, D, eps, L.stream())
    return x_out, q8, q8t, mean, rstd


def add_ln_modulate_bwd(dh, x, mean, rstd, B, T, *, scale=None, dx_in=None, y=None, gate=None, mod_ld=0,
                        dshift=None, dscale=None, dgate=None, affine=False):
    M, D = x.shape
    dx = torch.empty_like(x)
    dy = torch.empty_like(x) if y is not None else None
    L.call("uwu_add_ln_modulate_bwd", L.ptr(dh), L.ptr(x), L.ptr(mean), L.ptr(rstd), _p(scale), L.ptr(dx_in),
           L.ptr(y), _p(gate), mod_ld, L.ptr(dx), L.ptr(dy), _p(dshift), _p(dscale), _p(dgate), B, T, D, int(affine),
           L.dt(x), L.stream())
    return dx, dy
# ... 619 lines not shown
```

Measured before the change: 17740 images/s.

## Alternate kernel tile walk direction and use nontemporal loads for L2 reuse

Adds a per-thread stream plan that, for large bf16 non-fp8 runs, flips the block traversal order (reverse walk) on alternating kernels in the DiT forward/backward chain. Consecutive kernels then start on the data the previous kernel touched last, so more of it should still be in L2/MALL. The forward attention kernel additionally uses nontemporal K/V/Q loads and LSE stores under the policy so those streams do not evict reusable data. This adds template variants and a thread-local flag, and risks worse access patterns for kernels whose order affects coalescing or load balance.

```diff
diff --git a/include/uwu_hip.h b/include/uwu_hip.h
--- a/include/uwu_hip.h
+++ b/include/uwu_hip.h
@@ -32,6 +32,11 @@
 const char* uwu_last_error(void);
 int uwu_version(void);
 int uwu_env_refresh(void);
+
+#define UWU_SP_POLICY 1
+#define UWU_SP_REVERSE 2
+int uwu_stream_plan(int flags);
+int uwu_stream_walk_index(int i, int n, int reverse);
 int uwu_memset_zero(void* p, uint64_t bytes, void* stream);
 
 
diff --git a/uwudiff_amd/csrc/api.cpp b/uwudiff_amd/csrc/api.cpp
--- a/uwudiff_amd/csrc/api.cpp
+++ b/uwudiff_amd/csrc/api.cpp
@@ -5,6 +5,7 @@
 #include <atomic>
 
 #include "../../include/uwu_hip.h"
+#include "stream.h"
 
 static thread_local char g_err[512] = "";
 
@@ -21,6 +22,15 @@
 static int g_env_gen = 0;
 int uwu_env_generation() { return g_env_gen; }
 extern "C" int uwu_env_refresh(void) { return ++g_env_gen; }
+
+static thread_local int g_stream_flags = 0;
+int uwu_stream_flags() { return g_stream_flags; }
+extern "C" int uwu_stream_plan(int flags) {
+  const int prev = g_stream_flags;
+  g_stream_flags = flags & (UWU_SP_POLICY | UWU_SP_REVERSE);
+  return prev;
+}
+extern "C" int uwu_stream_walk_index(int i, int n, int reverse) { return uwu_walk_index(i, n, reverse); }
 
 std::atomic<const char*> g_uwu_gemm_last_kernel{""};
 extern "C" const char* uwu_gemm_last_kernel(void) { return g_uwu_gemm_last_kernel.load(std::memory_order_relaxed); }
diff --git a/uwudiff_amd/csrc/attention_p256.hip b/uwudiff_amd/csrc/attention_p256.hip
--- a/uwudiff_amd/csrc/attention_p256.hip
+++ b/uwudiff_amd/csrc/attention_p256.hip
@@ -25,6 +25,7 @@
   const float* lse;
   int B, H, ldq, ldk, ldv, ldo, nheads;
   float scale;
+  int rev;
 };
 
 __device__ __forceinline__ int fsw(int row) {
@@ -51,12 +52,19 @@
                : "v"(gsrc), "s"(lds_dst)
                : "memory");
 }
+template <bool NT = false>
 __device__ __forceinline__ void glds16_s(const void* sbase , unsigned voff, unsigned lds_dst ) {
   unsigned keep;
-  asm volatile("s_mov_b32 %0, m0\n\ts_mov_b32 m0, %3\n\ts_nop 0\n\tglobal_load_lds_dwordx4 %1, %2\n\ts_mov_b32 m0, %0"
-               : "=&s"(keep)
-               : "v"(voff), "s"(sbase), "s"(lds_dst)
-               : "memory");
+  if constexpr (NT)
+    asm volatile("s_mov_b32 %0, m0\n\ts_mov_b32 m0, %3\n\ts_nop 0\n\tglobal_load_lds_dwordx4 %1, %2 nt\n\ts_mov_b32 m0, %0"
+                 : "=&s"(keep)
+                 : "v"(voff), "s"(sbase), "s"(lds_dst)
+                 : "memory");
+  else
+    asm volatile("s_mov_b32 %0, m0\n\ts_mov_b32 m0, %3\n\ts_nop 0\n\tglobal_load_lds_dwordx4 %1, %2\n\ts_mov_b32 m0, %0"
+                 : "=&s"(keep)
+                 : "v"(voff), "s"(sbase), "s"(lds_dst)
+                 : "memory");
 }
 __device__ __forceinline__ f32x16 mfma32(const uint4& a, const uint4& b, f32x16 c) {
   return __builtin_amdgcn_mfma_f32_32x32x16_bf16(*reinterpret_cast<const bf16x8*>(&a), *reinterpret_cast<const bf16x8*>(&b), c, 0,
@@ -148,7 +156,7 @@
   }
 
   auto head_ptrs = [&](int j, int& b, int& hd) {
-    const int bh = (int)blockIdx.x + j * (int)gridDim.x;
+    const int bh = uwu_walk_index((int)blockIdx.x + j * (int)gridDim.x, a.nheads, a.rev);
     b = bh / a.H;
     hd = bh - b * a.H;
   };
@@ -443,6 +451,7 @@
   float* lse;
   int B, H, ldq, ldk, ldv, ldo, nheads;
   float scale;
+  int rev;
 };
 
 template <int N>
@@ -475,7 +484,7 @@
   }
 }
 
-template <int DH>
+template <int DH, bool FAR = false>
 __global__ void __launch_bounds__(512, 2) attn_fwd_p256(const FArgs a) {
   using G = FGeom<DH>;
   constexpr bool TAIL = G::TAIL;
@@ -500,7 +509,7 @@
   const unsigned TQ0 = (unsigned)((r >> 3) * 256 + (r & 7) * 16);
   const unsigned TA0 = (unsigned)(rowL * 16 + 8 * (lane & 1));
   auto head_ptrs = [&](int j, int& b, int& hd) {
-    const int bh = (int)blockIdx.x + j * (int)gridDim.x;
+    const int bh = uwu_walk_index((int)blockIdx.x + j * (int)gridDim.x, a.nheads, a.rev);
     b = bh / a.H;
     hd = bh - b * a.H;
   };
@@ -518,8 +527,8 @@
   auto issue_tile = [&](int g) {
     const int t64 = 64 * (g & 3);
     const unsigned dst = smem_base + (unsigned)((g % F_RING) * F_SLOT + wave * 1024);
-    glds16_s(kb_n, kvoff + (unsigned)(t64 * a.ldk * 2), dst);
-    glds16_s(vb_n, vvoff + (unsigned)(t64 * a.ldv * 2), dst + 8192);
+    glds16_s<FAR>(kb_n, kvoff + (unsigned)(t64 * a.ldk * 2), dst);
+    glds16_s<FAR>(vb_n, vvoff + (unsigned)(t64 * a.ldv * 2), dst + 8192);
     if constexpr (TAIL) {
       if (lane < 16) {
         const int trow = t64 + 8 * wave + (lane & 7);
@@ -531,7 +540,7 @@
   auto issue_q = [&]() {
 #pragma unroll
     for (int p = 0; p < 4; ++p)
-      glds16_s(qb_n, qvoff + (unsigned)(64 * p * a.ldq * 2), smem_base + (unsigned)(F_OFF_Q + p * 8192 + wave * 1024));
+      glds16_s<FAR>(qb_n, qvoff + (unsigned)(64 * p * a.ldq * 2), smem_base + (unsigned)(F_OFF_Q + p * 8192 + wave * 1024));
     if constexpr (TAIL) {
       if (lane < 32) glds16(qb_n + (int64_t)(32 * wave + lane) * a.ldq + 64, smem_base + (unsigned)(F_OFF_Q + 32768 + wave * 512));
     }
@@ -677,7 +686,9 @@
         const uint4 xt = *reinterpret_cast<const uint4*>(mine + 4096 + r * 16);
         *reinterpret_cast<uint4*>(ob + (int64_t)r * a.ldo + 64) = xt;
       }
-      a.lse[((int64_t)b * a.H + hd) * T + q0 + r] = m * a.scale + __logf(lt);
+      float* const lp = a.lse + ((int64_t)b * a.H + hd) * T + q0 + r;
+      if constexpr (FAR) __builtin_nontemporal_store(m * a.scale + __logf(lt), lp);
+      else *lp = m * a.scale + __logf(lt);
     }
   }
 }
@@ -706,6 +717,7 @@
     a.q = (const bf16_t*)q; a.k = (const bf16_t*)k; a.v = (const bf16_t*)v; a.o = (const bf16_t*)o; a.dO = (const bf16_t*)dO;
     a.dq = (bf16_t*)dq; a.dk = (bf16_t*)dk; a.dv = (bf16_t*)dv; a.lse = lse;
     a.B = B; a.H = H; a.ldq = ldq; a.ldk = ldk; a.ldv = ldv; a.ldo = ldo; a.nheads = B * H; a.scale = scale;
+    a.rev = uwu_stream_flags() & UWU_SP_REVERSE;
     const int grid = a.nheads < n_cu ? a.nheads : n_cu;
     hipLaunchKernelGGL(attn_bwd_p256<72>, dim3(grid), dim3(512), PGeom<72>::LDS, st, a);
     UWU_LAUNCH_CHECK("attention_bwd(p256, d = 72)");
@@ -719,6 +731,7 @@
   a.q = (const bf16_t*)q; a.k = (const bf16_t*)k; a.v = (const bf16_t*)v; a.o = (const bf16_t*)o; a.dO = (const bf16_t*)dO;
   a.dq = (bf16_t*)dq; a.dk = (bf16_t*)dk; a.dv = (bf16_t*)dv; a.lse = lse;
   a.B = B; a.H = H; a.ldq = ldq; a.ldk = ldk; a.ldv = ldv; a.ldo = ldo; a.nheads = B * H; a.scale = scale;
+  a.rev = uwu_stream_flags() & UWU_SP_REVERSE;
   const int grid = a.nheads < n_cu ? a.nheads : n_cu;
   hipLaunchKernelGGL(attn_bwd_p256<64>, dim3(grid), dim3(512), P_LDS, st, a);
   UWU_LAUNCH_CHECK("attention_bwd(p256)");
@@ -737,19 +750,24 @@
 
 int uwu_attn_p256_fwd(const void* q, const void* k, const void* v, void* o, float* lse, int B, int H, int d, int ldq, int ldk, int ldv,
                       int ldo, float scale, hipStream_t st) {
-  static unsigned char done[2][UWU_MAX_DEV];
+  static unsigned char done[3][UWU_MAX_DEV];
   const int n_cu = uwu_dev_cus();
   const int lds = d == 72 ? FGeom<72>::LDS : F_LDS;
-  const void* fn = d == 72 ? reinterpret_cast<const void*>(attn_fwd_p256<72>) : reinterpret_cast<const void*>(attn_fwd_p256<64>);
-  if (n_cu <= 0 || !uwu_func_lds(fn, lds, done[d == 72])) {
+  const int sp = uwu_stream_flags();
+  const bool far = d == 64 && (sp & UWU_SP_POLICY);
+  const void* fn = d == 72 ? reinterpret_cast<const void*>(attn_fwd_p256<72>)
+                           : far ? reinterpret_cast<const void*>(attn_fwd_p256<64, true>) : reinterpret_cast<const void*>(attn_fwd_p256<64>);
+  if (n_cu <= 0 || !uwu_func_lds(fn, lds, done[d == 72 ? 1 : far ? 2 : 0])) {
     uwu_set_error("attention_fwd(p256): the device cannot give a workgroup %d bytes of LDS", lds);
     return UWU_ELAUNCH;
   }
   FArgs a{};
   a.q = (const bf16_t*)q; a.k = (const bf16_t*)k; a.v = (const bf16_t*)v; a.out = (bf16_t*)o; a.lse = lse;
   a.B = B; a.H = H; a.ldq = ldq; a.ldk = ldk; a.ldv = ldv; a.ldo = ldo; a.nheads = B * H; a.scale = scale;
+  a.rev = sp & UWU_SP_REVERSE;
   const int grid = a.nheads < n_cu ? a.nheads : n_cu;
   if (d == 72) hipLaunchKernelGGL(attn_fwd_p256<72>, dim3(grid), dim3(512), lds, st, a);
+  else if (far) hipLaunchKernelGGL((attn_fwd_p256<64, true>), dim3(grid), dim3(512), lds, st, a);
   else hipLaunchKernelGGL(attn_fwd_p256<64>, dim3(grid), dim3(512), lds, st, a);
   UWU_LAUNCH_CHECK("attention_fwd(p256)");
   return UWU_OK;
diff --git a/uwudiff_amd/csrc/common.h b/uwudiff_amd/csrc/common.h
--- a/uwudiff_amd/csrc/common.h
+++ b/uwudiff_amd/csrc/common.h
@@ -36,6 +36,7 @@
   } while (0)
 
 #include "env.h"
+#include "stream.h"
 
 int uwu_dev_index();
 int uwu_dev_cus();
diff --git a/uwudiff_amd/csrc/dit.cpp b/uwudiff_amd/csrc/dit.cpp
--- a/uwudiff_amd/csrc/dit.cpp
+++ b/uwudiff_amd/csrc/dit.cpp
@@ -6,6 +6,7 @@
 
 #include "../../include/uwu_hip.h"
 #include "env.h"
+#include "stream.h"
 
 void uwu_set_error(const char* fmt, ...);
 
@@ -170,6 +171,32 @@
     if (rc_ != UWU_OK) return rc_; \
   } while (0)
 
+struct StreamPlan {
+  bool policy = false, alternate = false;
+  int dir = 0, saved = 0;
+  StreamPlan(const uwu_dit_desc& d, int64_t M, bool ckpt) {
+    static UwuEnv pol("UWU_STREAM_POLICY"), rev("UWU_STREAM_REVERSE");
+    policy = !pol.get().is('0') && d.dtype == UWU_BF16 && !d.fp8 && M > 16384 && !ckpt;
+    alternate = policy && !rev.get().is('0');
+    saved = uwu_stream_plan(0);
+  }
+  ~StreamPlan() { uwu_stream_plan(saved); }
+  StreamPlan(const StreamPlan&) = delete;
+  StreamPlan& operator=(const StreamPlan&) = delete;
+  void next() {
+    uwu_stream_plan(policy ? UWU_SP_POLICY | (dir ? UWU_SP_REVERSE : 0) : 0);
+    if (alternate) dir ^= 1;
+  }
+  void off() { uwu_stream_plan(0); }
+};
+#define RUN_SP(plan, expr) \
+  do {                     \
+    (plan).next();         \
+    int rc_ = (expr);      \
+    (plan).off();          \
+    if (rc_ != UWU_OK) return rc_; \
+  } while (0)
+
 int lin_fwd(const void* X, const void* W, const float* bias, void* Y, void* Y2, int M, int N, int K, int dt, int cdt,
             int epi, void* st) {
   return uwu_gemm(X, W, Y, Y2, bias, nullptr, M, N, K, K, K, N, 0, 0, 0, dt, cdt, epi, 1, st);
@@ -391,7 +418,8 @@
 }
 
 
-int block_forward(const uwu_dit_desc& d, const Layout& L, const Ptrs& P, const F8& f8, int l, bool recompute, void* st) {
+int block_forward(const uwu_dit_desc& d, const Layout& L, const Ptrs& P, const F8& f8, int l, bool recompute, StreamPlan& sp,
+                  void* st) {
   const int dt = d.dtype, B = d.B, T = d.T, D = d.D, M = (int)L.M, D3 = (int)L.D3, D4 = (int)L.D4;
   const size_t es = L.es;
   const float* w32 = d.w32;
@@ -414,16 +442,16 @@
     if (h1q < 0) return h1q;
   } else
   if (l == 0 || recompute) {
-    RUN(uwu_add_ln_modulate_fwd(x0, nullptr, nullptr, m + 0, m + D, ML, x0, P.lay(l, L.o_h1),
-                                P.lay<float>(l, L.o_m1), P.lay<float>(l, L.o_r1), B, T, D, d.ln_eps, 0, dt, st));
+    RUN_SP(sp, uwu_add_ln_modulate_fwd(x0, nullptr, nullptr, m + 0, m + D, ML, x0, P.lay(l, L.o_h1),
+                                       P.lay<float>(l, L.o_m1), P.lay<float>(l, L.o_r1), B, T, D, d.ln_eps, 0, dt, st));
   } else {
     const float* mp = mod + (int64_t)(l - 1) * 6 * D;
-    RUN(uwu_add_ln_modulate_fwd(P.lay(l - 1, L.o_x1), P.lay(l - 1, L.o_y2), mp + 5 * D, m + 0, m + D, ML, x0,
-                                P.lay(l, L.o_h1), P.lay<float>(l, L.o_m1), P.lay<float>(l, L.o_r1), B, T, D,
-                                d.ln_eps, 0, dt, st));
+    RUN_SP(sp, uwu_add_ln_modulate_fwd(P.lay(l - 1, L.o_x1), P.lay(l - 1, L.o_y2), mp + 5 * D, m + 0, m + D, ML, x0,
+                                       P.lay(l, L.o_h1), P.lay<float>(l, L.o_m1), P.lay<float>(l, L.o_r1), B, T, D,
+                                       d.ln_eps, 0, dt, st));
   }
   if (d.fp8) RUN(f8_fwd(f8, h1q ? nullptr : P.lay(l, L.o_h1), P.lay(l, L.o_h1t), f8.w(l, 0, false), w.qkv_b, P.lay(l, L.o_qkv), nullptr, M, D3, D, f8.role(l, 0), f8.role(l, 8), UWU_EPI_BIAS));
-  else RUN(lin_fwd(P.lay(l, L.o_h1), w.qkv_w, w.qkv_b, P.lay(l, L.o_qkv), nullptr, M, D3, D, dt, dt, UWU_EPI_BIAS, st));
+  else RUN_SP(sp, lin_fwd(P.lay(l, L.o_h1), w.qkv_w, w.qkv_b, P.lay(l, L.o_qkv), nullptr, M, D3, D, dt, dt, UWU_EPI_BIAS, st));
   char* qkv = P.lay<char>(l, L.o_qkv);
   if (d.rope) {
     const int64_t fo = (int64_t)l * d.H * (D / d.H / 4);
@@ -432,18 +460,18 @@
     RUN(uwu_attention_rope_fwd(qkv, qkv + (size_t)D * es, qkv + (size_t)2 * D * es, P.lay<float>(l, L.o_rope), P.lay(l, L.o_ao),
                                P.lay<float>(l, L.o_lse), B, T, d.H, D / d.H, D3, D3, D3, D, D, scale, dt, st));
   } else
-  RUN(uwu_attention_fwd(qkv, qkv + (size_t)D * es, qkv + (size_t)2 * D * es, P.lay(l, L.o_ao), P.lay<float>(l, L.o_lse),
-                        B, T, T, d.H, D / d.H, D3, D3, D3, D, scale, dt, st));
+  RUN_SP(sp, uwu_attention_fwd(qkv, qkv + (size_t)D * es, qkv + (size_t)2 * D * es, P.lay(l, L.o_ao), P.lay<float>(l, L.o_lse),
+                               B, T, T, d.H, D / d.H, D3, D3, D3, D, scale, dt, st));
   if (d.fp8) RUN(f8_fwd(f8, P.lay(l, L.o_ao), P.lay(l, L.o_aot), f8.w(l, 1, false), w.o_b, P.lay(l, L.o_y1), nullptr, M, D, D, f8.role(l, 1), f8.role(l, 9), UWU_EPI_BIAS));
-  else RUN(lin_fwd(P.lay(l, L.o_ao), w.o_w, w.o_b, P.lay(l, L.o_y1), nullptr, M, D, D, dt, dt, UWU_EPI_BIAS, st));
+  else RUN_SP(sp, lin_fwd(P.lay(l, L.o_ao), w.o_w, w.o_b, P.lay(l, L.o_y1), nullptr, M, D, D, dt, dt, UWU_EPI_BIAS, st));
   if (d.fp8) {
     h2q = ln_fwd_f8(d, f8, x0, P.lay(l, L.o_y1), m + 2 * D, m + 3 * D, m + 4 * D, ML, P.lay(l, L.o_x1), P.lay(l, L.o_h2),
                     P.lay(l, L.o_h2t), f8.role(l, 2), P.lay<float>(l, L.o_m2), P.lay<float>(l, L.o_r2), st);
     if (h2q < 0) return h2q;
   } else
-  RUN(uwu_add_ln_modulate_fwd(x0, P.lay(l, L.o_y1), m + 2 * D, m + 3 * D, m + 4 * D, ML, P.lay(l, L.o_x1),
-                              P.lay(l, L.o_h2), P.lay<float>(l, L.o_m2), P.lay<float>(l, L.o_r2), B, T, D, d.ln_eps,
-                              0, dt, st));
+  RUN_SP(sp, uwu_add_ln_modulate_fwd(x0, P.lay(l, L.o_y1), m + 2 * D, m + 3 * D, m + 4 * D, ML, P.lay(l, L.o_x1),
+                                     P.lay(l, L.o_h2), P.lay<float>(l, L.o_m2), P.lay<float>(l, L.o_r2), B, T, D, d.ln_eps,
+                                     0, dt, st));
   if (d.fp8) {
     if (f8_emit(d)) {
       const int r2 = f8.role(l, 2), r3 = f8.role(l, 3);
@@ -458,9 +486,9 @@
     RUN(f8_fwd(f8, h2q ? nullptr : P.lay(l, L.o_h2), P.lay(l, L.o_h2t), f8.w(l, 2, false), w.fc1_b, P.lay(l, L.o_u), P.lay(l, L.o_f), M, D4, D, f8.role(l, 2), f8.role(l, 10), UWU_EPI_BIAS_GELU));
     RUN(f8_fwd(f8, P.lay(l, L.o_f), P.lay(l, L.o_ft), f8.w(l, 3, false), w.fc2_b, P.lay(l, L.o_y2), nullptr, M, D, D4, f8.role(l, 3), f8.role(l, 11), UWU_EPI_BIAS));
   } else {
-    RUN(lin_fwd(P.lay(l, L.o_h2), w.fc1_w, w.fc1_b, P.lay(l, L.o_u), P.lay(l, L.o_f), M, D4, D, dt, dt,
-                UWU_EPI_BIAS_GELU, st));
-    RUN(lin_fwd(P.lay(l, L.o_f), w.fc2_w, w.fc2_b, P.lay(l, L.o_y2), nullptr, M, D, D4, dt, dt, UWU_EPI_BIAS, st));
+    RUN_SP(sp, lin_fwd(P.lay(l, L.o_h2), w.fc1_w, w.fc1_b, P.lay(l, L.o_u), P.lay(l, L.o_f), M, D4, D, dt, dt,
+                       UWU_EPI_BIAS_GELU, st));
+    RUN_SP(sp, lin_fwd(P.lay(l, L.o_f), w.fc2_w, w.fc2_b, P.lay(l, L.o_y2), nullptr, M, D, D4, dt, dt, UWU_EPI_BIAS, st));
   }
   return UWU_OK;
 }
@@ -537,13 +565,14 @@
               dt, UWU_EPI_BIAS, st));
   RUN(uwu_add_pos(P.lay(0, L.o_x0), d.pos, B, T, D, dt, st));
 
-  for (int l = 0; l < d.L; ++l) RUN(block_forward(d, L, P, f8, l, false, st));
+  StreamPlan sp(d, L.M, L.ckpt);
+  for (int l = 0; l < d.L; ++l) RUN(block_forward(d, L, P, f8, l, false, sp, st));
   {
     const int l = d.L - 1;
     const float* mp = mod + (int64_t)l * 6 * D;
     const float* mf = mod + (int64_t)d.L * 6 * D;
-    RUN(uwu_add_ln_modulate_fwd(P.lay(l, L.o_x1), P.lay(l, L.o_y2), mp + 5 * D, mf + 0, mf + D, ML, P.at(L.xF),
-                                P.at(L.hF), P.at<float>(L.mF), P.at<float>(L.rF), B, T, D, d.ln_eps, 0, dt, st));
+    RUN_SP(sp, uwu_add_ln_modulate_fwd(P.lay(l, L.o_x1), P.lay(l, L.o_y2), mp + 5 * D, mf + 0, mf + D, ML, P.at(L.xF),
+                                       P.at(L.hF), P.at<float>(L.mF), P.at<float>(L.rF), B, T, D, d.ln_eps, 0, dt, st));
     RUN(lin_fwd(P.at(L.hF), wb + d.off_final_w * es, w32 + d.off_final_b, P.at(L.otok), nullptr, M, (int)L.Ko, D, dt, dt,
                 UWU_EPI_BIAS, st));
     RUN(uwu_unpatchify(P.at(L.otok), dt, out, B, d.out_ch, d.img, d.img, d.patch, st));
@@ -581,6 +610,7 @@
   const bool pairs = !fk.on && !d.fp8 && dt == UWU_BF16 && M > 16384 && !L.ckpt;
   const bool pair_fc = pairs && wgrad_pair_ok(M, D4, D, D, D4, L.wsc_bytes);
   const bool pair_attn = pairs && wgrad_pair_ok(M, D3, D, D, D, L.wsc_bytes);
+  StreamPlan sp(d, L.M, L.ckpt);
 
   RUN(uwu_patchify(dout, P.at(L.dotok), B, d.out_ch, d.img, d.img, d.patch, dt, st));
   RUN(lin_wgrad(P.at(L.dotok), P.at(L.hF), g + d.off_final_w, M, (int)L.Ko, D, dt, st));
@@ -592,9 +622,9 @@
     const float* mf = mod + (int64_t)d.L * 6 * D;
     float* dmp = dmod + (int64_t)l * 6 * D;
     float* dmf = dmod + (int64_t)d.L * 6 * D;
-    RUN(uwu_add_ln_modulate_bwd(P.at(L.dh), P.at(L.xF), P.at<float>(L.mF), P.at<float>(L.rF), mf + D, nullptr,
-                                P.lay(l, L.o_y2), mp + 5 * D, ML, P.at(L.dx), P.at(L.dy), dmf + 0, dmf + D, dmp + 5 * D,
-                                B, T, D, 0, dt, st));
+    RUN_SP(sp, uwu_add_ln_modulate_bwd(P.at(L.dh), P.at(L.xF), P.at<float>(L.mF), P.at<float>(L.rF), mf + D, nullptr,
+                                       P.lay(l, L.o_y2), mp + 5 * D, ML, P.at(L.dx), P.at(L.dy), dmf + 0, dmf + D, dmp + 5 * D,
+                                       B, T, D, 0, dt, st));
   }
   for (int l = d.L - 1; l >= 0; --l) {
     const LayerW w = layer_weights(d, l);
@@ -622,10 +652,10 @@
     if (side_used[1]) RUN(join_side(fk, 1));
     if (dt == UWU_BF16 && D == 384 && M % 256 == 0 && M >= 256 * 256 && D4 % 64 == 0 && D4 >= 1024 && D4 <= 2048) {
       RUN(uwu_transpose_bf16(w.fc2_w, P.at(L.w2t), D, D4, D4, D, st));
-      RUN(uwu_gemm(P.at(L.dy), P.at(L.w2t), P.at(L.du), nullptr, nullptr, P.lay(l, L.o_u), M, D4, D, D, D, D4, D4, 0, 0, dt, dt,
-                   UWU_EPI_DGELU, 1, st));
+      RUN_SP(sp, uwu_gemm(P.at(L.dy), P.at(L.w2t), P.at(L.du), nullptr, nullptr, P.lay(l, L.o_u), M, D4, D, D, D, D4, D4, 0, 0, dt, dt,
+                          UWU_EPI_DGELU, 1, st));
     } else {
-      RUN(lin_dgrad(P.at(L.dy), w.fc2_w, P.at(L.du), P.lay(l, L.o_u), M, D, D4, dt, st, nullptr));
+      RUN_SP(sp, lin_dgrad(P.at(L.dy), w.fc2_w, P.at(L.du), P.lay(l, L.o_u), M, D, D4, dt, st, nullptr));
     }
     if (pair_fc) {
       RUN(lin_wgrad_pair(P.at(L.du), P.lay(l, L.o_h2), g + w.off_fc1_w, g + w.off_fc1_b, D4, D, P.at(L.dy), P.lay(l, L.o_f),
@@ -636,12 +666,12 @@
     }));
     side_used[1] = true;
     }
-    RUN(lin_dgrad(P.at(L.du), w.fc1_w, P.at(L.dh), nullptr, M, D4, D, dt, st));
+    RUN_SP(sp, lin_dgrad(P.at(L.du), w.fc1_w, P.at(L.dh), nullptr, M, D4, D, dt, st));
     RUN(join_side(fk, 0));
     }
-    RUN(uwu_add_ln_modulate_bwd(P.at(L.dh), P.lay(l, L.o_x1), P.lay<float>(l, L.o_m2), P.lay<float>(l, L.o_r2), m + 4 * D,
-                                P.at(L.dx), P.lay(l, L.o_y1), m + 2 * D, ML, P.at(L.dx), P.at(L.dy), dm + 3 * D,
-                                dm + 4 * D, dm + 2 * D, B, T, D, 0, dt, st));
+    RUN_SP(sp, uwu_add_ln_modulate_bwd(P.at(L.dh), P.lay(l, L.o_x1), P.lay<float>(l, L.o_m2), P.lay<float>(l, L.o_r2), m + 4 * D,
+                                       P.at(L.dx), P.lay(l, L.o_y1), m + 2 * D, ML, P.at(L.dx), P.at(L.dy), dm + 3 * D,
+                                       dm + 4 * D, dm + 2 * D, B, T, D, 0, dt, st));
     if (d.fp8) {
       RUN(f8_bwd(f8, P.at(L.dy), P.lay(l, L.o_aot), f8.w(l, 1, true), g + w.off_o_w, g + w.off_o_b, P.at(L.dao), nullptr, nullptr, M, D, D,
                  f8.role(l, 5), f8.role(l, 1), f8.role(l, 9)));
@@ -652,7 +682,7 @@
     }));
     side_used[2] = true;
     }
-    RUN(lin_dgrad(P.at(L.dy), w.o_w, P.at(L.dao), nullptr, M, D, D, dt, st));
+    RUN_SP(sp, lin_dgrad(P.at(L.dy), w.o_w, P.at(L.dao), nullptr, M, D, D, dt, st));
     if (side_used[3]) RUN(join_side(fk, 3));
     }
     char* qkv = P.lay<char>(l, L.o_qkv);
@@ -667,9 +697,9 @@
                                       w32 + d.off_rope_h + fo, w32 + d.off_rope_w + fo, dqkv + (size_t)qk * D * es,
                                       g + d.off_rope_h + fo, g + d.off_rope_w + fo, (int64_t)M, d.H, D / d.H, D3, dt, st));
     } else
-    RUN(uwu_attention_bwd(qkv, qkv + (size_t)D * es, qkv + (size_t)2 * D * es, P.lay(l, L.o_ao), P.at(L.dao),
-                          P.lay<float>(l, L.o_lse), P.at<float>(L.delta), dqkv, dqkv + (size_t)D * es,
-                          dqkv + (size_t)2 * D * es, B, T, T, d.H, D / d.H, D3, D3, D3, D, scale, dt, st));
+    RUN_SP(sp, uwu_attention_bwd(qkv, qkv + (size_t)D * es, qkv + (size_t)2 * D * es, P.lay(l, L.o_ao), P.at(L.dao),
+                                 P.lay<float>(l, L.o_lse), P.at<float>(L.delta), dqkv, dqkv + (size_t)D * es,
+                                 dqkv + (size_t)2 * D * es, B, T, T, d.H, D / d.H, D3, D3, D3, D, scale, dt, st));
     if (d.fp8) {
       RUN(f8_bwd(f8, dqkv, P.lay(l, L.o_h1t), f8.w(l, 0, true), g + w.off_qkv_w, g + w.off_qkv_b, P.at(L.dh), nullptr, nullptr, M, D3, D,
                  f8.role(l, 4), f8.role(l, 0), f8.role(l, 8)));
@@ -693,18 +723,18 @@
       uwu_set_error("dit_backward: hipEventRecord(layer_done[%d]) failed", l);
       return UWU_ELAUNCH;
     }
-    if (!d.fp8) RUN(lin_dgrad(dqkv, w.qkv_w, P.at(L.dh), nullptr, M, D3, D, dt, st));
+    if (!d.fp8) RUN_SP(sp, lin_dgrad(dqkv, w.qkv_w, P.at(L.dh), nullptr, M, D3, D, dt, st));
     if (!d.fp8) RUN(join_side(fk, 2));
-    if (L.ckpt && l > 0) RUN(block_forward(d, L, P, f8, l - 1, true, st));
+    if (L.ckpt && l > 0) RUN(block_forward(d, L, P, f8, l - 1, true, sp, st));
     if (l > 0) {
       const float* mp = mod + (int64_t)(l - 1) * 6 * D;
       float* dmp = dmod + (int64_t)(l - 1) * 6 * D;
-      RUN(uwu_add_ln_modulate_bwd(P.at(L.dh), P.lay(l, L.o_x0), P.lay<float>(l, L.o_m1), P.lay<float>(l, L.o_r1), m + D,
-                                  P.at(L.dx), P.lay(l - 1, L.o_y2), mp + 5 * D, ML, P.at(L.dx), P.at(L.dy), dm + 0,
-                                  dm + D, dmp + 5 * D, B, T, D, 0, dt, st));
+      RUN_SP(sp, uwu_add_ln_modulate_bwd(P.at(L.dh), P.lay(l, L.o_x0), P.lay<float>(l, L.o_m1), P.lay<float>(l, L.o_r1), m + D,
+                                         P.at(L.dx), P.lay(l - 1, L.o_y2), mp + 5 * D, ML, P.at(L.dx), P.at(L.dy), dm + 0,
+                                         dm + D, dmp + 5 * D, B, T, D, 0, dt, st));
     } else {
-      RUN(uwu_add_ln_modulate_bwd(P.at(L.dh), P.lay(l, L.o_x0), P.lay<float>(l, L.o_m1), P.lay<float>(l, L.o_r1), m + D,
-                                  P.at(L.dx), nullptr, nullptr, ML, P.at(L.dx), nullptr, dm + 0, dm + D, nullptr, B, T, D, 0, dt, st));
+      RUN_SP(sp, uwu_add_ln_modulate_bwd(P.at(L.dh), P.lay(l, L.o_x0), P.lay<float>(l, L.o_m1), P.lay<float>(l, L.o_r1), m + D,
+                                         P.at(L.dx), nullptr, nullptr, ML, P.at(L.dx), nullptr, dm + 0, dm + D, nullptr, B, T, D, 0, dt, st));
     }
   }
   if (fk.on)
diff --git a/uwudiff_amd/csrc/gemm.hip b/uwudiff_amd/csrc/gemm.hip
--- a/uwudiff_amd/csrc/gemm.hip
+++ b/uwudiff_amd/csrc/gemm.hip
@@ -440,6 +440,7 @@
     const int bid = blockIdx.x, xcd = bid & 7, loc = bid >> 3;
     const int q = nblk >> 3, rm = nblk & 7;
     tile = (xcd < rm ? xcd * (q + 1) : rm * (q + 1) + (xcd - rm) * q) + loc;
+    tile = uwu_walk_index(tile, nblk, g.sp & UWU_SP_REVERSE);
   }
   const int tm = tile / g.tiles_n, tn = tile - tm * g.tiles_n;
   const int m0 = tm * BMR, n0 = tn * BNC;
@@ -980,6 +981,7 @@
   g.M = M; g.N = N; g.K = K; g.lda = lda; g.ldb = ldb; g.ldc = ldc; g.ldaux = ldaux; g.epi = epilogue;
   g.tiles_m = (M + BM - 1) / BM;
   g.tiles_n = (N + BN - 1) / BN;
+  g.sp = uwu_stream_flags();
   g.wide = (!acc && c_dtype == UWU_BF16 && N % 8 == 0 && ldc % 8 == 0 && ((uintptr_t)C & 15) == 0 &&
             (C2 == nullptr || epilogue == UWU_EPI_DGELU || ((uintptr_t)C2 & 15) == 0)) ? 1 : 0;
   g.aux16 = (epilogue == UWU_EPI_DGELU && dtype == UWU_BF16 && N % 8 == 0 && ldaux % 8 == 0 && ((uintptr_t)aux & 15) == 0) ? 1 : 0;
diff --git a/uwudiff_amd/csrc/gemm_as.hip b/uwudiff_amd/csrc/gemm_as.hip
--- a/uwudiff_amd/csrc/gemm_as.hip
+++ b/uwudiff_amd/csrc/gemm_as.hip
@@ -5,7 +5,7 @@
 constexpr int AS_K = 384, AS_BN = 64, AS_STAGE = AS_BN * AS_K * 2;
 constexpr int AS_NST = 3;
 constexpr int AS_LDS = AS_NST * AS_STAGE + 8192;
-template <typename TC, int EPI>
+template <typename TC, int EPI, bool FAR_AUX = false>
 __global__ void __launch_bounds__(512, 2) gemm_as_kernel(const GemmArgs g) {
   extern __shared__ __attribute__((aligned(16))) char smem[];
   typedef bf16_t T;
@@ -13,7 +13,7 @@
   const int tid = threadIdx.x, lane = tid & 63;
   const int wave = __builtin_amdgcn_readfirstlane(tid >> 6);
   const int fr = lane & 15, fq = lane >> 4;
-  const int m0 = blockIdx.x * 256 + wave * 32;
+  const int m0 = uwu_walk_index((int)blockIdx.x, (int)gridDim.x, g.sp & UWU_SP_REVERSE) * 256 + wave * 32;
   const T* A = static_cast<const T*>(g.A);
   const T* B = static_cast<const T*>(g.B);
   float* bias_lds = reinterpret_cast<float*>(smem + AS_NST * AS_STAGE);
@@ -52,7 +52,10 @@
   auto aux_load = [&](int n0, int u) {
     const int i = u >> 1, jp = u & 1;
     const int m = m0 + 16 * i + fr, n = n0 + 32 * jp + (odd ? 16 + 4 * (fq - 1) : 4 * fq);
-    auxr[u] = *reinterpret_cast<const uint4*>(auxp + (int64_t)m * g.ldaux + n);
+    typedef unsigned au32x4 __attribute__((ext_vector_type(4)));
+    const au32x4* src = reinterpret_cast<const au32x4*>(auxp + (int64_t)m * g.ldaux + n);
+    const au32x4 v = FAR_AUX ? __builtin_nontemporal_load(src) : *src;
+    auxr[u] = uint4{v[0], v[1], v[2], v[3]};
   };
   auto epi_unit = [&](const f32x4 (&pa)[FI][FJ], int n0, int i, int jp) {
     f32x4 v0 = pa[i][2 * jp], v1 = pa[i][2 * jp + 1];
@@ -159,6 +162,9 @@
 template <typename TC, int EPI>
 int uwu_launch_gemm_as(GemmArgs g, hipStream_t st) {
   g.wide = 1;
+  if constexpr (EPI == UWU_EPI_DGELU)
+    if (g.sp & UWU_SP_POLICY)
+      return gemm_launch<gemm_as_kernel<TC, EPI, true>>("gemm_as", AS_LDS, dim3(g.M / 256), 512, st, gemm_prof(g, false, sizeof(TC)), g);
   return gemm_launch<gemm_as_kernel<TC, EPI>>("gemm_as", AS_LDS, dim3(g.M / 256), 512, st, gemm_prof(g, false, sizeof(TC)), g);
 }
 
diff --git a/uwudiff_amd/csrc/gemm_p8n.hip b/uwudiff_amd/csrc/gemm_p8n.hip
--- a/uwudiff_amd/csrc/gemm_p8n.hip
+++ b/uwudiff_amd/csrc/gemm_p8n.hip
@@ -24,7 +24,7 @@
   auto tile_of = [&](int L) __attribute__((always_inline)) {
     const int xcd = L & 7, loc = L >> 3;
     const int q = nblk >> 3, rm = nblk & 7;
-    return (xcd < rm ? xcd * (q + 1) : rm * (q + 1) + (xcd - rm) * q) + loc;
+    return uwu_walk_index((xcd < rm ? xcd * (q + 1) : rm * (q + 1) + (xcd - rm) * q) + loc, nblk, g.sp & UWU_SP_REVERSE);
   };
 
   constexpr int NOA = FI == 6 ? 1 : G::APIECES;
diff --git a/uwudiff_amd/csrc/gemm_shared.h b/uwudiff_amd/csrc/gemm_shared.h
--- a/uwudiff_amd/csrc/gemm_shared.h
+++ b/uwudiff_amd/csrc/gemm_shared.h
@@ -31,6 +31,7 @@
   const float* q_scale;
   float* q_amax;
   int ldq, ldqt;
+  int sp;
 };
 
 namespace {
diff --git a/uwudiff_amd/csrc/norm.hip b/uwudiff_amd/csrc/norm.hip
--- a/uwudiff_amd/csrc/norm.hip
+++ b/uwudiff_amd/csrc/norm.hip
@@ -48,10 +48,12 @@
                                                              const float* __restrict__ scale, int mod_ld,
                                                              T* __restrict__ x_out, T* __restrict__ h,
                                                              float* __restrict__ mean_o, float* __restrict__ rstd_o,
-                                                             int M, int T_tok, int D, float eps, int affine) {
+                                                             int M, int T_tok, int D, float eps, int affine, int sp) {
   const int lane = threadIdx.x & 63, wave = threadIdx.x >> 6;
   const int nit = (D + 511) >> 9;
-  for (int row = blockIdx.x * 4 + wave; row < M; row += gridDim.x * 4) {
+  const int rev = sp & UWU_SP_REVERSE;
+  for (int u = blockIdx.x * 4 + wave; u < M; u += gridDim.x * 4) {
+    const int row = uwu_walk_index(u, M, rev);
     const int b = row / T_tok;
     const int64_t off = (int64_t)row * D;
     f32x8 v[MAX_IT];
@@ -120,11 +122,14 @@
                                                                const float* __restrict__ scale, int mod_ld,
                                                                T* __restrict__ x_out, T* __restrict__ h,
                                                                float* __restrict__ mean_o, float* __restrict__ rstd_o,
-                                                               int M, int T_tok, float eps, int affine) {
+                                                               int M, int T_tok, float eps, int affine, int sp) {
   constexpr int D = 128 * NCH;
   const int lane = threadIdx.x & 63, wave = threadIdx.x >> 6;
   const int sub = lane >> 4, l16 = lane & 15;
-  for (int row0 = (blockIdx.x * 4 + wave) * 4; row0 < M; row0 += gridDim.x * 16) {
+  const int rev = sp & UWU_SP_REVERSE;
+  const int n4 = (M + 3) >> 2;
+  for (int u = blockIdx.x * 4 + wave; u < n4; u += gridDim.x * 4) {
+    const int row0 = 4 * uwu_walk_index(u, n4, rev);
     const int row = row0 + sub;
     const bool ok = row < M;
     const int rc = ok ? row : M - 1;
@@ -317,11 +322,11 @@
     const float* __restrict__ rstd_i, const float* __restrict__ scale, const T* __restrict__ dx_in,
     const T* __restrict__ y, const float* __restrict__ gate, int mod_ld, T* __restrict__ dx_out, T* __restrict__ dy,
     float* __restrict__ dshift, float* __restrict__ dscale, float* __restrict__ dgate, int M, int T_tok, int D,
-    int rows_per_block, int affine) {
+    int rows_per_block, int affine, int sp) {
   extern __shared__ __attribute__((aligned(16))) float red[];
   const int lane = threadIdx.x & 63, wave = threadIdx.x >> 6;
   const int nit = (D + 511) >> 9;
-  const int row0 = blockIdx.x * rows_per_block;
+  const int row0 = uwu_walk_index((int)blockIdx.x, (int)gridDim.x, sp & UWU_SP_REVERSE) * rows_per_block;
   const int b = row0 / T_tok;
   f32x8 a_sh[MAX_IT], a_sc[MAX_IT], a_g[MAX_IT];
 #pragma unroll
@@ -631,6 +636,7 @@
   if (grid > 8192) grid = 8192;
   hipStream_t st = (hipStream_t)stream;
   UWU_CHECK_ARG(dtype == UWU_F32 || dtype == UWU_BF16, "add_ln_modulate_fwd: bad dtype");
+  const int sp = uwu_stream_flags();
   UwuProfScope prof(stream);
   static UwuEnv r16("UWU_LN_ROW16");
   const bool al16 = (((uintptr_t)x_in | (uintptr_t)h | (uintptr_t)y | (uintptr_t)x_out) & 15) == 0 && (mod_ld % 4 == 0);
@@ -641,11 +647,11 @@
   case NCH:                                                                                                                    \
     if (dtype == UWU_F32)                                                                                                      \
       hipLaunchKernelGGL((add_ln_mod_fwd16_kernel<float, NCH>), dim3(g16), dim3(256), 0, st, (const float*)x_in, (const float*)y, \
-                         gate, shift, scale, mod_ld, (float*)x_out, (float*)h, mean, rstd, M, T, eps, affine);                   \
+                         gate, shift, scale, mod_ld, (float*)x_out, (float*)h, mean, rstd, M, T, eps, affine, sp);               \
     else                                                                                                                       \
       hipLaunchKernelGGL((add_ln_mod_fwd16_kernel<bf16_t, NCH>), dim3(g16), dim3(256), 0, st, (const bf16_t*)x_in,            \
                          (const bf16_t*)y, gate, shift, scale, mod_ld, (bf16_t*)x_out, (bf16_t*)h, mean, rstd, M, T, eps,       \
-                         affine);                                                                                               \
+                         affine, sp);                                                                                           \
     break;
     switch (D / 128) {
       F16_CASE(1) F16_CASE(2) F16_CASE(3) F16_CASE(4) F16_CASE(5) F16_CASE(6) F16_CASE(7) F16_CASE(8) F16_CASE(9) F16_CASE(10)
@@ -662,11 +668,11 @@
     if (dtype == UWU_F32)                                                                                          \
       hipLaunchKernelGGL((add_ln_mod_fwd_kernel<float, NIT>), dim3(grid), dim3(256), 0, st, (const float*)x_in,    \
                          (const float*)y, gate, shift, scale, mod_ld, (float*)x_out, (float*)h, mean, rstd, M, T, D, \
-                         eps, affine);                                                                                     \
+                         eps, affine, sp);                                                                                 \
     else                                                                                                           \
       hipLaunchKernelGGL((add_ln_mod_fwd_kernel<bf16_t, NIT>), dim3(grid), dim3(256), 0, st, (const bf16_t*)x_in,  \
                          (const bf16_t*)y, gate, shift, scale, mod_ld, (bf16_t*)x_out, (bf16_t*)h, mean, rstd, M,  \
-                         T, D, eps, affine);                                                                               \
+                         T, D, eps, affine, sp);                                                                           \
     break;
   switch ((D + 511) / 512) {
     FWD_CASE(1) FWD_CASE(2) FWD_CASE(3) FWD_CASE(4) FWD_CASE(5) FWD_CASE(6) FWD_CASE(7) FWD_CASE(8)
@@ -692,6 +698,7 @@
   const int M = B * T;
   hipStream_t st = (hipStream_t)stream;
   UWU_CHECK_ARG(dtype == UWU_F32 || dtype == UWU_BF16, "add_ln_modulate_bwd: bad dtype");
+  const int sp = uwu_stream_flags();
   if (affine && mod_ld == 0 && scale && !y && dshift && dscale && D <= 2048 && (dx_in == nullptr || ((uintptr_t)dx_in & 15) == 0)) {
     const int rpb = M >= 16384 ? 64 : (M >= 4096 ? 32 : 16);
     const int grid = (M + rpb - 1) / rpb;
@@ -745,7 +752,7 @@
   case NIT:                                                                                                            \
     hipLaunchKernelGGL((add_ln_mod_bwd_kernel<bf16_t, NIT, 8>), dim3(M / rows), dim3(512), lds, st, (const bf16_t*)dh, \
                        (const bf16_t*)x, mean, rstd, scale, (const bf16_t*)dx_in, (const bf16_t*)y, gate, mod_ld,      \
-                       (bf16_t*)dx_out, (bf16_t*)dy, dshift, dscale, dgate, M, T, D, rows, affine);                    \
+                       (bf16_t*)dx_out, (bf16_t*)dy, dshift, dscale, dgate, M, T, D, rows, affine, sp);                    \
     break;
     if (dtype == UWU_BF16) {
       switch ((D + 511) / 512) { SMALL_CASE(1) SMALL_CASE(2) }
@@ -772,12 +779,12 @@
     if (dtype == UWU_F32)                                                                                           \
       hipLaunchKernelGGL((add_ln_mod_bwd_kernel<float, NIT>), dim3(M / rows), dim3(256), lds, st, (const float*)dh, \
                          (const float*)x, mean, rstd, scale, (const float*)dx_in, (const float*)y, gate, mod_ld,    \
-                         (float*)dx_out, (float*)dy, dshift, dscale, dgate, M, T, D, rows, affine);                         \
+                         (float*)dx_out, (float*)dy, dshift, dscale, dgate, M, T, D, rows, affine, sp);                         \
     else                                                                                                            \
       hipLaunchKernelGGL((add_ln_mod_bwd_kernel<bf16_t, NIT>), dim3(M / rows), dim3(256), lds, st,                  \
                          (const bf16_t*)dh, (const bf16_t*)x, mean, rstd, scale, (const bf16_t*)dx_in,              \
                          (const bf16_t*)y, gate, mod_ld, (bf16_t*)dx_out, (bf16_t*)dy, dshift, dscale, dgate, M, T,   \
-                         D, rows, affine);                                                                                  \
+                         D, rows, affine, sp);                                                                              \
     break;
   switch ((D + 511) / 512) {
     BWD_CASE(1) BWD_CASE(2) BWD_CASE(3) BWD_CASE(4) BWD_CASE(5) BWD_CASE(6)
diff --git a/uwudiff_amd/csrc/stream.h b/uwudiff_amd/csrc/stream.h
--- /dev/null
+++ b/uwudiff_amd/csrc/stream.h
@@ -0,0 +1,5 @@
+#pragma once
+#include <hip/hip_runtime.h>
+
+int uwu_stream_flags();
+__host__ __device__ __forceinline__ int uwu_walk_index(int i, int n, int reverse) { return reverse ? n - 1 - i : i; }
diff --git a/uwudiff_amd/lib.py b/uwudiff_amd/lib.py
--- a/uwudiff_amd/lib.py
+++ b/uwudiff_amd/lib.py
@@ -10,6 +10,7 @@
 F32, BF16, I64 = 0, 1, 2
 PT = {"epsilon": 0, "v_prediction": 1, "sample": 2, "rectified_flow": 3}
 EPI_NONE, EPI_BIAS, EPI_BIAS_GELU, EPI_DGELU, EPI_BIAS_SILU, EPI_ACCUM = 0, 1, 2, 3, 4, 5
+SP_POLICY, SP_REVERSE = 1, 2
 ACT = {"quick_gelu": 0, "gelu": 1}
 GATE = {"gated-gelu": 0}
 FILTER = {"bilinear": 0, "bicubic": 1, "lanczos": 2}
@@ -41,6 +42,8 @@
     "uwu_last_error": (c_char_p, []),
     "uwu_version": (c_int, []),
     "uwu_env_refresh": (c_int, []),
+    "uwu_stream_plan": (c_int, [c_int]),
+    "uwu_stream_walk_index": (c_int, [c_int, c_int, c_int]),
     "uwu_memset_zero": (c_int, [P, ctypes.c_uint64, P]),
     "uwu_schedule_gather": (c_int, [P, P, P, P, c_int, c_int, c_int, c_float, c_int, P, P]),
     "uwu_rf_time_to_sigma": (c_int, [P, c_float, P, c_int, c_int, P, P, P]),
diff --git a/uwudiff_amd/ops.py b/uwudiff_amd/ops.py
--- a/uwudiff_amd/ops.py
+++ b/uwudiff_amd/ops.py
@@ -1,8 +1,18 @@
+import contextlib
 import ctypes
 
 import torch
 
 from . import lib as L
+
+
+@contextlib.contextmanager
+def stream_plan(flags):
+    prev = L.load().uwu_stream_plan(int(flags))
+    try:
+        yield
+    finally:
+        L.load().uwu_stream_plan(prev)
 
 
 def gemm(a, b, *, trans_a=False, trans_b=False, bias=None, aux=None, epilogue=L.EPI_NONE, out=None, out2=None,
```

New measurement: 17830 images/s, median of 6. About the same (+0.5%).
